# DerryHub/BEVFormer_tensorrt

Hardware: AMD Instinct MI355X
Metric: frames/sec BEVFormer-base bs=1 fp16 end-to-end on MI355X (re-hosted model, random weights, synthetic 6-camera frames) (higher is better)
Workload: dtype f16

## Files before the change

### bevformer_tensorrt_amd/bevformer.py

```python
import math
import os
import time

import torch
import torch.nn as nn
import torch.nn.functional as F

from . import functions as _hip_ops
from . import geometry as G
from .functions.dispatch import OWN_KERNELS, own_kernel_choice, using as _dispatch_using
from .functions.linear import tsgemm_weight_stationary
from .utils import lib as _lib

CONFIGS = {
    "tiny": dict(depth=50, dcn=(False, False, False, False), fpn_in=[2048], out_indices=(3,), levels=1,
                 image=(480, 800), bev=(50, 50), enc_layers=3, style="pytorch"),
    "small": dict(depth=101, dcn=(False, False, True, True), fpn_in=[2048], out_indices=(3,), levels=1,
                  image=(736, 1280), bev=(150, 150), enc_layers=3, style="caffe"),
    "base": dict(depth=101, dcn=(False, False, True, True), fpn_in=[512, 1024, 2048], out_indices=(1, 2, 3),
                 levels=4, image=(928, 1600), bev=(200, 200), enc_layers=6, style="caffe"),
}
PC_RANGE = [-51.2, -51.2, -5.0, 51.2, 51.2, 3.0]
POST_CENTER_RANGE = [-61.2, -61.2, -10.0, 61.2, 61.2, 10.0]
MAX_DETECTIONS = 300
EMBED, HEADS, NUM_QUERY, NUM_CAMS = 256, 8, 900, 6


inverse_sigmoid = G.inverse_sigmoid


_CAM_IDX = {}


def _take_cams(t, cams):
    cams = tuple(cams)
    if cams == tuple(range(t.shape[0])):
        return t
    key = (cams, str(t.device))
    idx = _CAM_IDX.get(key)
    if idx is None:
        idx = _CAM_IDX[key] = torch.tensor(cams, dtype=torch.long, device=t.device)
    return t.index_select(0, idx)


def _rows(x):
    return x.permute(0, 2, 3, 1).reshape(-1, x.shape[1])


def _from_rows(y, n, h, w):
    return y.view(n, h, w, y.shape[-1]).permute(0, 3, 1, 2)


_FUSED_LINEAR = {"enabled": os.environ.get("BEVOPS_FUSED_LINEAR", "1") != "0"}
_R3 = {"enabled": os.environ.get("BEVOPS_R3_FUSIONS", "1") != "0"}
_TSA_LOCAL = {"enabled": os.environ.get("BEVOPS_TSA_LOCAL", "1") == "1"}
_TSA_GLUE = {"enabled": os.environ.get("BEVOPS_TSA_GLUE", "1") == "1"}


def _or_none(fn, *args, **kwargs):
    try:
        return fn(*args, **kwargs)
    except _lib.BevopsError as exc:
        if exc.status != _lib.NOT_SUPPORTED:
            raise
        return None


def _fused_linear(ops, x, weight, bias, residual, relu):
    fn = getattr(ops, "linear_bias_act", None)
    if fn is None or not _FUSED_LINEAR["enabled"] or x.dtype != torch.float16 or not x.is_cuda:
        return None
    auto = getattr(ops, "dense_auto", None)
    if auto is not None and _R3["enabled"]:
        return _or_none(auto, x, weight, bias, residual, relu)
    return _or_none(fn, x, weight, bias, residual, relu)


def _gemm_entry(ops):
    return getattr(ops, "dense_auto", None) or getattr(ops, "linear_bias_act", None)


def _dense(ops, lin, x, residual=None, relu=False):
    if hasattr(lin, "fake_quant_reference"):
        return lin(x, residual, relu)
    y = _fused_linear(ops, x, lin.weight, lin.bias, residual, relu)
    if y is not None:
        return y
    y = lin(x)
    if residual is not None:
        y = y + residual
    return F.relu(y, inplace=True) if relu else y


def _mlp(ops, seq, x):
    mods = list(seq)
    if not _R3["enabled"] or not all(isinstance(m, (nn.Linear, nn.ReLU)) for m in mods):
        return seq(x)
    i = 0
    while i < len(mods):
        if isinstance(mods[i], nn.ReLU):
            x = F.relu(x)
            i += 1
            continue
        relu = i + 1 < len(mods) and isinstance(mods[i + 1], nn.ReLU)
        x = _dense(ops, mods[i], x, None, relu)
        i += 2 if relu else 1
    return x


def _layer_norm(ops, norm, x):
    fn = getattr(ops, "layer_norm", None)
    if fn is None or not _FUSED_LINEAR["enabled"] or x.dtype != torch.float16 or not x.is_cuda or \
            x.shape[-1] not in (64, 128, 256, 512):
        return norm(x)
    return fn(x, norm.weight, norm.bias, norm.eps)


_FUSED_REFINE = {"enabled": os.environ.get("BEVOPS_FUSED_REFINE", "1") == "1"}
_OWN_ATTN = {"enabled": os.environ.get("BEVOPS_OWN_ATTN", "1") == "1"}
_LN_FUSED = {"enabled": os.environ.get("BEVOPS_LN_FUSED", "1") == "1"}
_INT8_LN_FUSED = {"enabled": os.environ.get("BEVOPS_INT8_LN_FUSED", "0") == "1"}
_OWN_ENCODER = {"enabled": os.environ.get("BEVOPS_OWN_ENCODER", "1") == "1"}
_SHARDED_TABLE_BACKBONE = {"enabled": _OWN_ENCODER["enabled"] and os.environ.get("BEVOPS_SHARDED_RULE_DISPATCH", "0") != "1"}


def _dense_norm(ops, lin, x, residual, norm):
    fn = getattr(ops, "tsgemm_ln", None)
    if fn is not None and _LN_FUSED["enabled"] and _R3["enabled"] and _FUSED_LINEAR["enabled"] and type(lin) is nn.Linear \
            and x.dtype == torch.float16 and x.is_cuda and lin.out_features == EMBED and lin.in_features % 64 == 0 \
            and isinstance(norm, nn.LayerNorm) and norm.elementwise_affine and norm.normalized_shape == (EMBED,) \
            and x.numel() // x.shape[-1] >= 32:
        out = _or_none(fn, x, lin.weight, lin.bias, residual, norm.weight, norm.bias, norm.eps)
        if out is not None:
            return out
    if _int8_ln_on(ops) and _int8_norm_ok(lin, x, norm):
        return lin.forward_norm_from_q(_hip_ops.quantize_rows(x, lin.scale_in), residual, norm)
    return _layer_norm(ops, norm, _dense(ops, lin, x, residual, False))


def _int8_ln_on(ops):
    on = getattr(ops, "int8_ln_fused", None)
    return _INT8_LN_FUSED["enabled"] if on is None else on


def _int8_norm_ok(lin, x, norm):
    return hasattr(lin, "fake_quant_reference") and lin.mode == "int8" \
        and lin.in_features % 128 == 0 and lin.out_features == EMBED and x.dtype == torch.float16 and x.is_cuda \
        and isinstance(norm, nn.LayerNorm) and norm.elementwise_affine and norm.normalized_shape == (EMBED,)


def _int8_ffn_chain_ok(fc1, fc2, x, norm):
    return hasattr(fc1, "fake_quant_reference") and fc1.mode == "int8" and fc1.in_features % 16 == 0 \
        and _int8_norm_ok(fc2, x, norm)


def _conv1x1_nhwc(ops, x, conv, relu, residual=None):
    s = conv.stride[0]
    if s > 1:
        strided = getattr(ops, "conv_nhwc", None)
        if strided is not None and _R3["enabled"] and _FUSED_LINEAR["enabled"] and x.dtype == torch.float16 and x.is_cuda \
                and not hasattr(conv, "lin") and conv.in_channels % 32 == 0 and x.is_contiguous(memory_format=torch.channels_last):
            return strided(x, conv.weight, conv.bias, relu, residual, s)
        lin = getattr(conv, "lin", None)
        int8_conv = getattr(ops, "conv_int8_nhwc", None)
        if lin is not None and getattr(lin, "mode", None) == "int8" and int8_conv is not None and _R3["enabled"] \
                and x.dtype == torch.float16 and x.is_cuda and conv.in_channels % 64 == 0 \
                and x.is_contiguous(memory_format=torch.channels_last):
            return int8_conv(x, lin.scale_in, lin.weight_q.view(conv.out_channels, 1, 1, conv.in_channels), lin.scale_w,
                             lin.bias_f32, relu, residual, s)
        x = x[:, :, ::s, ::s].contiguous(memory_format=torch.channels_last)
    n, c, h, w = x.shape
    if hasattr(conv, "lin"):
        y = conv.lin(_rows(x), None if residual is None else _rows(residual), relu)
        return _from_rows(y, n, h, w)
    wt = conv.weight.view(conv.out_channels, c).t()
    if residual is not None:
        y = _fused_linear(ops, _rows(x), conv.weight.view(conv.out_channels, c), conv.bias, _rows(residual), relu)
        if y is None:
            y = torch.mm(_rows(x), wt)
            ops.bias_act_nhwc_(y, conv.bias, _rows(residual), relu)
    else:
        y = _fused_linear(ops, _rows(x), conv.weight.view(conv.out_channels, c), conv.bias, None, relu) \
            if _R3["enabled"] else None
        if y is None:
            y = torch._addmm_activation(conv.bias, _rows(x), wt) if relu else torch.addmm(conv.bias, _rows(x), wt)
    return _from_rows(y, n, h, w)


def _conv_nhwc(ops, x, conv, relu, residual=None):
    qmode = getattr(conv, "qmode", None)
    if qmode == "calibrate":
        conv.collect(x)
    elif qmode == "int8" and x.is_contiguous(memory_format=torch.channels_last):
        return conv.int8_nhwc(x, residual, relu)
    auto = getattr(ops, "conv3x3_auto", None)
    if auto is not None and _R3["enabled"] and _FUSED_LINEAR["enabled"] and x.dtype == torch.float16 and x.is_cuda \
            and conv.kernel_size == (3, 3) and conv.stride[0] == conv.stride[1] and conv.padding == (1, 1) \
            and conv.groups == 1 and conv.dilation == (1, 1) and conv.in_channels % 32 == 0 \
            and x.is_contiguous(memory_format=torch.channels_last):
        return auto(x, conv.weight, conv.bias, relu, residual, conv.stride[0])
    y = F.conv2d(x, conv.weight, None, conv.stride, conv.padding)
    if not y.is_contiguous(memory_format=torch.channels_last):
        y = y.contiguous(memory_format=torch.channels_last)
    return ops.bias_act_nhwc_(y, conv.bias, residual, relu)


class DCNv2Pack(nn.Module):

    def __init__(self, cin, cout, ops, stride=1):
        super().__init__()
        self.ops, self.stride = ops, stride
        self._c32_ok = True
        self.weight = nn.Parameter(torch.randn(cout, cin, 3, 3) / math.sqrt(cin * 9))
        self.bias = nn.Parameter(torch.zeros(cout))
        self.conv_offset = nn.Conv2d(cin, 27, 3, stride, 1)
        nn.init.normal_(self.conv_offset.weight, std=0.01)
        nn.init.zeros_(self.conv_offset.bias)

    def forward(self, x):
        out = self.conv_offset(x)
        o1, o2, mask = torch.chunk(out, 3, dim=1)
        offset = torch.cat((o1, o2), dim=1)
        return self.ops.modulated_deformable_conv2d(x, offset, torch.sigmoid(mask), self.weight,
                                                    self.bias, self.stride, 1, 1, 1, 1)

    def _chain_collect(self, om):
        cal = getattr(self, "chain_cal", None)
        if cal is not None:
            cal.collect(self.chain_site + ".offset", om[:, :18])
            cal.collect(self.chain_site + ".mask", torch.sigmoid(om[:, 18:27]))

    def forward_nhwc(self, x, relu):
        fn = getattr(self.ops, "conv_offset_nhwc", None)
        if fn is not None and self.stride == 1 and _FUSED_LINEAR["enabled"] and self._c32_ok:
            try:
                out = fn(x, self.conv_offset.weight, self.conv_offset.bias)
                self._chain_collect(out)
                return self.ops.modulated_deformable_conv2d_nhwc(x, None, None, self.weight, self.bias, self.stride,
                                                                 1, 1, 1, 1, relu=relu, offset_mask_nhwc=out)
            except _lib.BevopsError as exc:
                if exc.status != _lib.NOT_SUPPORTED:
                    raise
                self._c32_ok = False
        w = self.conv_offset.weight
        if getattr(self, "_w32", None) is None or self._w32[2] != (w._version, w.dtype, w.device):
            w32 = torch.zeros(32, *w.shape[1:], dtype=w.dtype, device=w.device)
            w32[:27] = w.detach()
            b32 = torch.zeros(32, dtype=w.dtype, device=w.device)
            b32[:27] = self.conv_offset.bias.detach()
            self._w32 = (w32.contiguous(memory_format=torch.channels_last), b32, (w._version, w.dtype, w.device))
        out = F.conv2d(x, self._w32[0], None, self.stride, 1)
        if not out.is_contiguous(memory_format=torch.channels_last):
            out = out.contiguous(memory_format=torch.channels_last)
        out = self.ops.bias_act_nhwc_(out, self._w32[1], None, False)
        self._chain_collect(out)
        return self.ops.modulated_deformable_conv2d_nhwc(x, None, None, self.weight, self.bias, self.stride, 1, 1,
                                                         1, 1, relu=relu, offset_mask_nhwc=out)


_FUSED_DOWNSAMPLE = {"enabled": os.environ.get("BEVOPS_FUSED_DOWNSAMPLE", "1") != "0"}
_FUSED_DOWNSAMPLE_SHAPES = {(64, 64, 1), (128, 256, 2), (256, 512, 2), (512, 1024, 2)}


def _two_source_ok(ops, blk, x):
    ds, c3 = blk.downsample, blk.conv3
    if ds is None or not (_FUSED_DOWNSAMPLE["enabled"] and _R3["enabled"] and _FUSED_LINEAR["enabled"]) \
            or getattr(ops, "gemm2", None) is None or getattr(blk, "chain_cal", None) is not None:
        return False
    if type(ds) is not nn.Conv2d or type(c3) is not nn.Conv2d or hasattr(ds, "lin") or hasattr(c3, "lin") \
            or ds.bias is None or c3.bias is None or ds.weight.dtype != torch.float16 or c3.weight.dtype != torch.float16 \
            or ds.kernel_size != (1, 1) or c3.kernel_size != (1, 1) or c3.stride != (1, 1) or ds.stride[0] != ds.stride[1]:
        return False
    if x.dtype != torch.float16 or not x.is_cuda or x.dim() != 4 or not x.is_contiguous(memory_format=torch.channels_last):
        return False
    return (c3.in_channels, ds.in_channels, ds.stride[0]) in _FUSED_DOWNSAMPLE_SHAPES


def _stacked_pair(blk):
    ds, c3 = blk.downsample, blk.conv3
    key = _versions(c3.weight, ds.weight, c3.bias, ds.bias)
    hit = getattr(blk, "_w3d", None)
    if hit is None or hit[0] != key:
        n = c3.out_channels
        w = torch.cat([c3.weight.detach().reshape(n, -1), ds.weight.detach().reshape(n, -1)], dim=1).contiguous()
        b = (c3.bias.detach().float() + ds.bias.detach().float()).to(c3.bias.dtype).contiguous()
        hit = (key, w, b)
        blk._w3d = hit
    return hit[1], hit[2]


class Bottleneck(nn.Module):

    def __init__(self, cin, planes, stride, dcn, ops, downsample, style="caffe"):
        super().__init__()
        s1, s2 = (stride, 1) if style == "caffe" else (1, stride)
        self.conv1 = nn.Conv2d(cin, planes, 1, s1)
        self.conv2 = DCNv2Pack(planes, planes, ops, s2) if dcn else nn.Conv2d(planes, planes, 3, s2, 1)
        self.conv3 = nn.Conv2d(planes, planes * 4, 1)
        self.downsample = nn.Conv2d(cin, planes * 4, 1, stride) if downsample else None

    def forward(self, x):
        idt = x if self.downsample is None else self.downsample(x)
        out = F.relu(self.conv1(x), inplace=True)
        out = F.relu(self.conv2(out), inplace=True)
        return F.relu(self.conv3(out) + idt, inplace=True)

    def _hidden_nhwc(self, x, ops):
        out = _conv1x1_nhwc(ops, x, self.conv1, True)
        if isinstance(self.conv2, DCNv2Pack):
            return self.conv2.forward_nhwc(out, True)
        return _conv_nhwc(ops, out, self.conv2, True)

    def forward_nhwc(self, x, ops):
        if _two_source_ok(ops, self, x):
            h = self._hidden_nhwc(x, ops)
            w, b = _stacked_pair(self)
            n, _, ho, wo = h.shape
            y = _or_none(ops.gemm2, _rows(h), x, w, b, self.downsample.stride[0], True)
            if y is not None:
                return _from_rows(y, n, ho, wo)
            return _conv1x1_nhwc(ops, h, self.conv3, True, residual=_conv1x1_nhwc(ops, x, self.downsample, False))
        idt = x if self.downsample is None else _conv1x1_nhwc(ops, x, self.downsample, False)
        out = _conv1x1_nhwc(ops, x, self.conv1, True)
        cal = getattr(self, "chain_cal", None)
        if cal is not None:
            cal.collect(self.chain_site + ".t1", out)
            if self.downsample is not None:
                cal.collect(self.chain_site + ".idt", idt)
        if isinstance(self.conv2, DCNv2Pack):
            out = self.conv2.forward_nhwc(out, True)
        else:
            out = _conv_nhwc(ops, out, self.conv2, True)
        return _conv1x1_nhwc(ops, out, self.conv3, True, residual=idt)


class ResNet(nn.Module):
    def __init__(self, depth, dcn, out_indices, ops, style="caffe"):
        super().__init__()
        blocks = {50: (3, 4, 6, 3), 101: (3, 4, 23, 3)}[depth]
        self.out_indices = out_indices
        self.stem = nn.Conv2d(3, 64, 7, 2, 3)
        cin, stages = 64, []
        for i, n in enumerate(blocks):
            planes, layers = 64 * 2 ** i, []
            for j in range(n):
                layers.append(Bottleneck(cin, planes, (2 if i > 0 else 1) if j == 0 else 1, dcn[i], ops, j == 0, style))
                cin = planes * 4
            stages.append(nn.Sequential(*layers))
        self.stages = nn.ModuleList(stages)

    def forward(self, x):
        x = F.max_pool2d(F.relu(self.stem(x), inplace=True), 3, 2, 1)
        outs = []
        for i, st in enumerate(self.stages):
            x = st(x)
            if i in self.out_indices:
                outs.append(x)
        return outs

    def _stem_fused(self, x, ops):
        fused = getattr(ops, "stem_conv_pool", None)
        if fused is None or not (_R3["enabled"] and _FUSED_LINEAR["enabled"]):
            return None
        from .functions.conv import STEM_FUSED
        st = self.stem
        ok = (STEM_FUSED["enabled"] and x.is_cuda and x.dtype == torch.float16 and x.is_contiguous() and x.shape[-1] % 2 == 0
              and tuple(st.weight.shape) == (64, 3, 7, 7) and st.stride == (2, 2) and st.padding == (3, 3))
        return fused(x, st.weight, st.bias) if ok else None

    def forward_nhwc(self, x, ops):
        y = self._stem_fused(x, ops)
        if y is not None:
            return self._stages_nhwc(y, ops)
        x = x.contiguous(memory_format=torch.channels_last)
        pool = getattr(ops, "bias_relu_maxpool_nhwc", None)
        if pool is not None and _R3["enabled"] and _FUSED_LINEAR["enabled"] and x.dtype == torch.float16 and x.is_cuda:
            y = F.conv2d(x, self.stem.weight, None, self.stem.stride, self.stem.padding)
            if not y.is_contiguous(memory_format=torch.channels_last):
                y = y.contiguous(memory_format=torch.channels_last)
            x = pool(y, self.stem.bias)
        else:
            x = F.max_pool2d(_conv_nhwc(ops, x, self.stem, True), 3, 2, 1)
        return self._stages_nhwc(x, ops)

    def _stages_nhwc(self, x, ops):
        outs = []
        for i, st in enumerate(self.stages):
            for blk in st:
                x = blk.forward_nhwc(x, ops)
            if i in self.out_indices:
                outs.append(x)
        return outs


class FPN(nn.Module):

    def __init__(self, cins, cout, num_outs):
        super().__init__()
        self.lateral = nn.ModuleList(nn.Conv2d(c, cout, 1) for c in cins)
        self.fpn = nn.ModuleList(nn.Conv2d(cout, cout, 3, 1, 1) for _ in cins)
        self.extra = nn.ModuleList(nn.Conv2d(cout, cout, 3, 2, 1) for _ in range(num_outs - len(cins)))

    def forward(self, feats):
        lat = [l(f) for l, f in zip(self.lateral, feats)]
        for i in range(len(lat) - 1, 0, -1):
            lat[i - 1] = lat[i - 1] + F.interpolate(lat[i], size=lat[i - 1].shape[2:], mode="nearest")
        outs = [c(x) for c, x in zip(self.fpn, lat)]
        for e in self.extra:
            outs.append(e(F.relu(outs[-1])))
        return outs

    def forward_nhwc(self, feats, ops):
        return self.topdown_nhwc([_conv1x1_nhwc(ops, f, l, False) for l, f in zip(self.lateral, feats)], ops)

    def topdown_nhwc(self, lat, ops):
        up_add = getattr(ops, "upsample_add_nhwc_", None)
        for i in range(len(lat) - 1, 0, -1):
            a, b = lat[i - 1], lat[i]
            if up_add is not None and _FUSED_LINEAR["enabled"] and _R3["enabled"] and a.dtype == torch.float16 and a.is_cuda \
                    and a.is_contiguous(memory_format=torch.channels_last) and b.is_contiguous(memory_format=torch.channels_last):
                up_add(a, b)
            else:
                lat[i - 1] = a + F.interpolate(b, size=a.shape[2:], mode="nearest")
        outs = [_conv_nhwc(ops, x.contiguous(memory_format=torch.channels_last), c, False) for c, x in zip(self.fpn, lat)]
        for e in self.extra:
            outs.append(_conv_nhwc(ops, F.relu(outs[-1]), e, False))
        return outs


class FFN(nn.Module):
    def __init__(self, dim=EMBED, hidden=2 * EMBED):
        super().__init__()
        self.fc1, self.fc2 = nn.Linear(dim, hidden), nn.Linear(hidden, dim)

    def forward(self, x, ops=None, norm=None):
        if norm is not None and _int8_ln_on(ops) and _int8_ffn_chain_ok(self.fc1, self.fc2, x, norm):
            h_q = self.fc1.forward_q(x, self.fc2.scale_in, relu=True)
            return self.fc2.forward_norm_from_q(h_q, x, norm)
        h = _dense(ops, self.fc1, x, None, True)
        return _dense(ops, self.fc2, h, x, False) if norm is None else _dense_norm(ops, self.fc2, h, x, norm)


class TemporalSelfAttention(nn.Module):

    def __init__(self, ops, points=4):
        super().__init__()
        self.ops, self.points = ops, points
        self.sampling_offsets = nn.Linear(EMBED * 2, 2 * HEADS * points * 2)
        self.attention_weights = nn.Linear(EMBED * 2, 2 * HEADS * points)
        self.value_proj, self.output_proj = nn.Linear(EMBED, EMBED), nn.Linear(EMBED, EMBED)
        self._split = self._pos_term = None

    def _split_projection(self, query, prev0, bev_pos, prev_term=None):
        def both_terms():
            terms = self._split_terms(query, bev_pos)
            if terms is None:
                return None
            fn, wa, wb, pos_term = terms
            t = prev_term if prev_term is not None else fn(prev0.reshape(-1, EMBED), wa, None, pos_term, False)
            return fn(query.reshape(-1, EMBED), wb, None, t, False)
        return _or_none(both_terms)

    def _split_terms(self, query, bev_pos):
        fn = _gemm_entry(self.ops)
        so, aw = self.sampling_offsets, self.attention_weights
        if fn is None or not (_R3["enabled"] and _FUSED_LINEAR["enabled"]) or query.dtype != torch.float16 \
                or not query.is_cuda or type(so) is not nn.Linear or type(aw) is not nn.Linear:
            return None
        key = (so.weight._version, aw.weight._version, so.bias._version, aw.bias._version, so.weight.data_ptr())
        if self._split is None or self._split[0] != key:
            w = torch.cat([so.weight, aw.weight]).detach()
            self._split = (key, w[:, :EMBED].contiguous(), w[:, EMBED:].contiguous(),
                           torch.cat([so.bias, aw.bias]).detach().contiguous())
            self._pos_term = None
        _, wa, wb, b = self._split
        pkey = (bev_pos.data_ptr(), bev_pos._version, tuple(bev_pos.shape), bev_pos.dtype)
        if self._pos_term is None or self._pos_term[0] != pkey:
            self._pos_term = (pkey, fn(bev_pos.reshape(-1, EMBED), wb, b, None, False))
        return fn, wa, wb, self._pos_term[1]

    def forward(self, query, value, bev_pos, ref_2d, spatial_shapes, rows=None, norm=None, prev_term=None):
        identity = query
        nq, nk = query.shape[1], value.shape[1]
        mine = value if rows is None else value[:, rows[0]:rows[1]]
        both = self._split_projection(query, mine[0], bev_pos, prev_term if rows is None else None)
        split = getattr(self.ops, "tsa_split", None) if _TSA_GLUE["enabled"] else None
        pre = None
        if both is not None and split is not None and self.points == 4:
            pre = split(both, HEADS, self.points)
        elif both is not None:
            n_off = 2 * HEADS * self.points * 2
            off = both[:, :n_off].view(1, nq, HEADS, 2, 1, self.points, 2)
            w = both[:, n_off:].view(1, nq, HEADS, 2, 1, self.points)
        else:
            query = torch.cat([mine[:1], query + bev_pos], -1)
            off = self.sampling_offsets(query).view(1, nq, HEADS, 2, 1, self.points, 2)
            w = self.attention_weights(query).view(1, nq, HEADS, 2, 1, self.points)
        value = _dense(self.ops, self.value_proj, value).view(2, nk, HEADS, EMBED // HEADS)
        if pre is not None:
            off, w = pre
        else:
            w = w.permute(0, 3, 1, 2, 4, 5).contiguous().view(2, nq, HEADS, -1)
            off = off.permute(0, 3, 1, 2, 4, 5, 6).contiguous().view(2, nq, HEADS, -1)
        msda = (getattr(self.ops, "multi_scale_deformable_attn_local", None) if _TSA_LOCAL["enabled"] else None) \
            or self.ops.multi_scale_deformable_attn
        out = msda(value, spatial_shapes, ref_2d, off, w).flatten(2)
        mean2 = getattr(self.ops, "queue_mean2", None) if _TSA_GLUE["enabled"] else None
        if mean2 is not None and out.is_cuda and out.dtype == torch.float16 and out.numel() % 16 == 0 and _R3["enabled"]:
            out = mean2(out)
        else:
            out = torch.mean(out, keepdim=True, dim=0)
        if norm is not None:
            return _dense_norm(self.ops, self.output_proj, out, identity, norm)
        return _dense(self.ops, self.output_proj, out, identity, False)


class SpatialCrossAttention(nn.Module):

    def __init__(self, ops, levels, points=8):
        super().__init__()
        self.ops = ops
        self._proj_ok = True
        self.sampling_offsets = nn.Linear(EMBED, HEADS * levels * points * 2)
        self.attention_weights = nn.Linear(EMBED, HEADS * levels * points)
        self.value_proj, self.output_proj = nn.Linear(EMBED, EMBED), nn.Linear(EMBED, EMBED)

    def _offsets_weights(self, query, nq, merged):
        pair = _merged_pair(self.ops, self, "_so_aw", self.sampling_offsets, self.attention_weights, query) if merged else None
        if pair is None:
            pair = (_dense(self.ops, self.sampling_offsets, query), _dense(self.ops, self.attention_weights, query))
        return pair[0].view(1, nq, HEADS, -1), pair[1].view(1, nq, HEADS, -1)

    def forward(self, query, value, reference_points_cam, bev_mask, spatial_shapes, cams=None, gather=None, plan=None,
                residual=None, norm=None, merged=False):
        inp_residual = query if residual is None else residual
        ncam, nk, nq = value.shape[0], value.shape[1], query.shape[1]
        mode = getattr(gather, "mode", None)
        if cams is None and gather is not None and hasattr(gather, "cams"):
            cams = gather.cams
        ref = reference_points_cam.reshape(reference_points_cam.shape[0], nq, 1, -1)
        ref_l, mask_l = (ref, bev_mask) if cams is None else (_take_cams(ref, cams), _take_cams(bev_mask, cams))
        local_sum = gather is None or mode in ("reduce", "scatter")
        projected = getattr(self.ops, "spatial_cross_attention_projected", None)
        fused = getattr(self.ops, "spatial_cross_attention_sample", None)
        fp16_gpu = value.dtype == torch.float16 and value.is_cuda
        slots = None
        if local_sum and ncam == 0:
            slots = torch.zeros((1, nq, EMBED), dtype=value.dtype, device=value.device)
        elif projected is not None and local_sum and _R3["enabled"] and self._proj_ok and fp16_gpu \
                and not hasattr(self.value_proj, "fake_quant_reference"):
            off, w = self._offsets_weights(query, nq, merged)
            try:
                slots = projected(value.reshape(ncam, nk, EMBED), self.value_proj.weight, self.value_proj.bias,
                                  spatial_shapes, ref_l.contiguous(), off, w, mask_l.contiguous(), HEADS,
                                  **({"plan": plan} if plan is not None else {}))
            except _lib.BevopsError as exc:
                if exc.status != _lib.NOT_SUPPORTED:
                    raise
                self._proj_ok = False
        if slots is None:
            value = _dense(self.ops, self.value_proj, value.reshape(ncam, nk, EMBED)).view(ncam, nk, HEADS, EMBED // HEADS)
            off, w = (t.expand(ncam, -1, -1, -1) for t in self._offsets_weights(query, nq, merged))
            msda = self.ops.multi_scale_deformable_attn
            if mode == "gather":
                ref_c = ref_l.contiguous()
                queries = gather.gather(
                    lambda i: msda(value[i:i + 1], spatial_shapes, ref_c[i:i + 1], off[:1], w[:1]).flatten(2),
                    (nq, EMBED), value.dtype, value.device)
                slots = (queries * bev_mask).sum(0, keepdim=True)
            elif local_sum and fused is not None and (fp16_gpu or getattr(fused, "any_device", False)):
                slots = fused(value, spatial_shapes, ref_l, off[:1], w[:1], mask_l)
            elif local_sum:
                queries = msda(value, spatial_shapes, ref_l.contiguous(), off, w).flatten(2)
                slots = (queries * mask_l).sum(0, keepdim=True)
            else:
                queries = gather(msda(value, spatial_shapes, ref_l.contiguous(), off, w).flatten(2))
                slots = (queries * bev_mask).sum(0, keepdim=True)
        if mode == "reduce":
            slots = gather.reduce(slots)
        elif mode == "scatter":
            slots = gather.reduce_scatter_queries(slots, nq)
        if norm is not None:
            return _dense_norm(self.ops, self.output_proj, slots, inp_residual, norm)
        return _dense(self.ops, self.output_proj, slots, inp_residual, False)


class BEVFormerLayer(nn.Module):
    def __init__(self, ops, levels):
        super().__init__()
        self.tsa, self.sca, self.ffn = TemporalSelfAttention(ops), SpatialCrossAttention(ops, levels), FFN()
        self.norms = nn.ModuleList(nn.LayerNorm(EMBED) for _ in range(3))

    def forward(self, query, value, bev_pos, ref_2d, ref_cam, bev_mask, spatial_shapes, bev_shapes, prev_bev,
                use_prev_bev, cams, gather, plan=None, rows=None, tsa_prev_term=None, merged=False):
        ops = self.tsa.ops
        if rows is not None:
            lo, hi = rows
            nq = bev_pos.shape[1]
            if torch.is_tensor(use_prev_bev) or not use_prev_bev:
                full = gather.all_gather_queries(query, nq)
                prev = torch.where(use_prev_bev.to(torch.bool), prev_bev, full.expand(2, -1, -1)) \
                    if torch.is_tensor(use_prev_bev) else full.repeat(2, 1, 1)
            else:
                prev = prev_bev
            query = self.tsa(query, prev, bev_pos[:, lo:hi], ref_2d[:, lo:hi].contiguous(), bev_shapes, rows=rows,
                             norm=self.norms[0])
            full = gather.all_gather_queries(query, nq)
            query = self.sca(full, value, ref_cam, bev_mask, spatial_shapes, cams, gather, plan, residual=query,
                             norm=self.norms[1])
            return self.ffn(query, ops, norm=self.norms[2])
        if torch.is_tensor(use_prev_bev):
            prev = torch.where(use_prev_bev.to(torch.bool), prev_bev, query.expand(2, -1, -1))
        else:
            prev = prev_bev if use_prev_bev else query.repeat(2, 1, 1)
        if prev is not prev_bev:
            tsa_prev_term = None
        query = self.tsa(query, prev, bev_pos, ref_2d, bev_shapes, norm=self.norms[0], prev_term=tsa_prev_term)
        query = self.sca(query, value, ref_cam, bev_mask, spatial_shapes, cams, gather, plan, norm=self.norms[1],
                         merged=merged)
        return self.ffn(query, ops, norm=self.norms[2])


def _static_term(cache, owner, key, pos, fn, weight, bias):
    hit = getattr(owner, cache, None)
    if hit is None or hit[0] != key or hit[1] is not pos:
        hit = (key, pos, fn(pos.reshape(-1, pos.shape[-1]), weight, bias, None, False))
        setattr(owner, cache, hit)
    return hit[2]


def _fast_dense_ok(ops, x, *linears):
    return getattr(ops, "linear_bias_act", None) is not None and _R3["enabled"] and _FUSED_LINEAR["enabled"] \
        and x.dtype == torch.float16 and x.is_cuda \
        and all(isinstance(l, nn.Linear) and not hasattr(l, "fake_quant_reference") for l in linears)


def _versions(*tensors):
    return tuple(t._version for t in tensors) + tuple(t.data_ptr() for t in tensors)


_MERGED_PROJ = {"enabled": os.environ.get("BEVOPS_MERGED_PROJ", "1") != "0"}


def _merge_ok(ops, x, linears, has_res):
    if not (_MERGED_PROJ["enabled"] and _R3["enabled"] and _FUSED_LINEAR["enabled"]) \
            or getattr(ops, "dense_auto", None) is None or x.dtype != torch.float16 or not x.is_cuda \
            or not all(type(l) is nn.Linear and l.bias is not None and l.weight.dtype == torch.float16 for l in linears):
        return False
    if not OWN_KERNELS["enabled"]:
        return False
    K = x.shape[-1]
    return _per_layer_kernels(x.device, x.numel() // K, [l.weight.shape[0] for l in linears], K, not has_res, has_res) == "tiled"


def _per_layer_kernels(device, M, widths, K, has_bias, has_res):
    if M <= 0:
        return None
    names = {own_kernel_choice(device, M, n, K, False, has_bias, has_res) for n in widths}
    if names == {"small"}:
        return "small"
    if names <= {"tile", "tsgemm"} and ("tsgemm" not in names or tsgemm_weight_stationary(K)):
        return "tiled"
    return None


def _merged_pair(ops, owner, cache, lin_a, lin_b, x):
    fn = getattr(ops, "tile_gemm_dst", None)
    widths = [lin_a.weight.shape[0], lin_b.weight.shape[0]]
    if fn is None or not _merge_ok(ops, x, (lin_a, lin_b), False) or any(n % 64 for n in widths):
        return None
    key = _versions(lin_a.weight, lin_b.weight, lin_a.bias, lin_b.bias)
    hit = getattr(owner, cache, None)
    if hit is None or hit[0] != key:
        hit = (key, torch.cat([lin_a.weight, lin_b.weight]).detach().contiguous(),
               torch.cat([lin_a.bias, lin_b.bias]).detach().contiguous())
        setattr(owner, cache, hit)
    return _or_none(fn, x.reshape(-1, x.shape[-1]), hit[1], hit[2], widths)


def _merged_prev_terms(ops, owner, cache, tsas, query, prev0, bev_pos):
    fn = getattr(ops, "tile_gemm_dst", None)
    if fn is None or not (_MERGED_PROJ["enabled"] and _R3["enabled"] and _FUSED_LINEAR["enabled"]) \
            or prev0.dtype != torch.float16 or not prev0.is_cuda:
        return None
    if not OWN_KERNELS["enabled"]:
        return None

    def all_layers():
        terms = [t._split_terms(query, bev_pos) for t in tsas]
        if any(t is None for t in terms):
            return None
        widths = [t[1].shape[0] for t in terms]
        M = prev0.numel() // EMBED
# ... 566 lines not shown
```

### bevformer_tensorrt_amd/csrc/capi.hip

```cpp
#include <string.h>

#include "common.h"

extern "C" const char *bevops_version(void) { return "bevops-hip 0.1 (gfx950)"; }

extern "C" const char *bevops_status_string(int status) {
  switch (status) {
    case BEVOPS_SUCCESS: return "success";
    case BEVOPS_FAILURE: return "failure (kernel launch error)";
    case BEVOPS_BAD_PARAM: return "bad parameter";
    case BEVOPS_NOT_SUPPORTED: return "dtype/shape combination not supported";
    case BEVOPS_NOT_INITIALIZED: return "not initialized";
    default: return "unknown status";
  }
}

namespace {
struct Entry {
  const char *name;
  void *fn;
};
const Entry kTable[] = {
    {"bevops_msda_forward", (void *)&bevops_msda_forward},
    {"bevops_msda_forward_ws", (void *)&bevops_msda_forward_ws},
    {"bevops_msda_workspace_size", (void *)&bevops_msda_workspace_size},
    {"MultiScaleDeformableAttnTRT", (void *)&bevops_msda_forward},
    {"MultiScaleDeformableAttnTRT2", (void *)&bevops_msda_forward},
    {"bevops_rotate_forward", (void *)&bevops_rotate_forward},
    {"RotateTRT", (void *)&bevops_rotate_forward},
    {"RotateTRT2", (void *)&bevops_rotate_forward},
    {"bevops_grid_sampler_2d_forward", (void *)&bevops_grid_sampler_2d_forward},
    {"GridSampler2DTRT", (void *)&bevops_grid_sampler_2d_forward},
    {"GridSampler2DTRT2", (void *)&bevops_grid_sampler_2d_forward},
    {"bevops_grid_sampler_3d_forward", (void *)&bevops_grid_sampler_3d_forward},
    {"GridSampler3DTRT", (void *)&bevops_grid_sampler_3d_forward},
    {"GridSampler3DTRT2", (void *)&bevops_grid_sampler_3d_forward},
    {"bevops_bev_pool_v2_forward", (void *)&bevops_bev_pool_v2_forward},
    {"BEVPoolV2TRT", (void *)&bevops_bev_pool_v2_forward},
    {"BEVPoolV2TRT2", (void *)&bevops_bev_pool_v2_forward},
    {"bevops_mdconv_forward", (void *)&bevops_mdconv_forward},
    {"bevops_mdconv_workspace_size", (void *)&bevops_mdconv_workspace_size},
    {"bevops_mdconv_forward_int8", (void *)&bevops_mdconv_forward_int8},
    {"bevops_mdconv_forward_int8_packed", (void *)&bevops_mdconv_forward_int8_packed},
    {"ModulatedDeformableConv2dTRT", (void *)&bevops_mdconv_forward},
    {"ModulatedDeformableConv2dTRT2", (void *)&bevops_mdconv_forward},
    {"bevops_qkv_forward", (void *)&bevops_qkv_forward},
    {"bevops_qkv_workspace_size", (void *)&bevops_qkv_workspace_size},
    {"QKVTRT", (void *)&bevops_qkv_forward},
    {"QKVTRT2", (void *)&bevops_qkv_forward},
    {"bevops_inverse_forward", (void *)&bevops_inverse_forward},
    {"InverseTRT", (void *)&bevops_inverse_forward},
    {"bevops_nms_free_decode", (void *)&bevops_nms_free_decode},
    {"bevops_centerpoint_decode", (void *)&bevops_centerpoint_decode},
    {"bevops_centerpoint_decode_ex", (void *)&bevops_centerpoint_decode_ex},
    {"bevops_centerpoint_decode_workspace_size", (void *)&bevops_centerpoint_decode_workspace_size},
    {"bevops_bev_nms", (void *)&bevops_bev_nms},
    {"bevops_bev_nms_workspace_size", (void *)&bevops_bev_nms_workspace_size},
    {"bevops_bev_iou", (void *)&bevops_bev_iou},
    {"bevops_centernet_decode", (void *)&bevops_centernet_decode},
    {"bevops_centernet_decode_workspace_size", (void *)&bevops_centernet_decode_workspace_size},
    {"bevops_yolox_decode", (void *)&bevops_yolox_decode},
    {"bevops_box_nms", (void *)&bevops_box_nms},
    {"bevops_box_nms_workspace_size", (void *)&bevops_box_nms_workspace_size},
    {"bevops_lss_voxel_prepare", (void *)&bevops_lss_voxel_prepare},
    {"bevops_lss_voxel_prepare_workspace_size", (void *)&bevops_lss_voxel_prepare_workspace_size},
    {"bevops_lss_voxel_prepare_batched", (void *)&bevops_lss_voxel_prepare_batched},
    {"bevops_lss_voxel_prepare_batched_workspace_size", (void *)&bevops_lss_voxel_prepare_batched_workspace_size},
    {"bevops_bev_pool_v2_forward_indirect", (void *)&bevops_bev_pool_v2_forward_indirect},
    {"bevops_grid_sampler_2d_forward_ws", (void *)&bevops_grid_sampler_2d_forward_ws},
    {"bevops_grid_sampler_2d_workspace_size", (void *)&bevops_grid_sampler_2d_workspace_size},
    {"bevops_rotate_forward_hwc", (void *)&bevops_rotate_forward_hwc},
    {"bevops_sca_forward", (void *)&bevops_sca_forward},
    {"bevops_mdconv_forward_nhwc", (void *)&bevops_mdconv_forward_nhwc},
    {"bevops_conv3x3_c32_forward_nhwc", (void *)&bevops_conv3x3_c32_forward_nhwc},
    {"bevops_bias_act_nhwc", (void *)&bevops_bias_act_nhwc},
    {"bevops_bias_relu_maxpool_nhwc", (void *)&bevops_bias_relu_maxpool_nhwc},
    {"bevops_stem_packed_size", (void *)&bevops_stem_packed_size},
    {"bevops_stem_pack", (void *)&bevops_stem_pack},
    {"bevops_stem_conv_pool", (void *)&bevops_stem_conv_pool},
    {"bevops_stem_set_variant", (void *)&bevops_stem_set_variant},
    {"bevops_upsample_add_nhwc", (void *)&bevops_upsample_add_nhwc},
    {"bevops_lss_depth_split", (void *)&bevops_lss_depth_split},
    {"bevops_upsample_bilinear_concat_nhwc", (void *)&bevops_upsample_bilinear_concat_nhwc},
    {"bevops_lss_depth_split_s8", (void *)&bevops_lss_depth_split_s8},
    {"bevops_upsample_bilinear_s8", (void *)&bevops_upsample_bilinear_s8},
    {"bevops_tsa_split", (void *)&bevops_tsa_split},
    {"bevops_queue_mean2", (void *)&bevops_queue_mean2},
    {"bevops_tsgemm_f16", (void *)&bevops_tsgemm_f16},
    {"bevops_tsgemm_s8", (void *)&bevops_tsgemm_s8},
    {"bevops_tsgemm_s8_ln", (void *)&bevops_tsgemm_s8_ln},
    {"bevops_tsgemm_tile_rows", (void *)&bevops_tsgemm_tile_rows},
    {"bevops_tsgemm_f16_ln", (void *)&bevops_tsgemm_f16_ln},
    {"bevops_tsgemm_f16_grouped", (void *)&bevops_tsgemm_f16_grouped},
    {"bevops_mha_selfattn_f16", (void *)&bevops_mha_selfattn_f16},
    {"bevops_mha_selfattn_max_queries", (void *)&bevops_mha_selfattn_max_queries},
    {"bevops_value_proj_packed_size", (void *)&bevops_value_proj_packed_size},
    {"bevops_value_proj_packed", (void *)&bevops_value_proj_packed},
    {"bevops_value_pack_planes", (void *)&bevops_value_pack_planes},
    {"bevops_sca_prepacked_workspace_size", (void *)&bevops_sca_prepacked_workspace_size},
    {"bevops_sca_forward_prepacked", (void *)&bevops_sca_forward_prepacked},
    {"bevops_sca_plan_size", (void *)&bevops_sca_plan_size},
    {"bevops_sca_plan_build", (void *)&bevops_sca_plan_build},
    {"bevops_sca_forward_planned", (void *)&bevops_sca_forward_planned},
    {"bevops_point_sampling", (void *)&bevops_point_sampling},
    {"bevops_feat_embed_nhwc", (void *)&bevops_feat_embed_nhwc},
    {"bevops_linear_bias_act", (void *)&bevops_linear_bias_act},
    {"bevops_linear_tune", (void *)&bevops_linear_tune},
    {"bevops_quantize_rows", (void *)&bevops_quantize_rows},
    {"bevops_dequantize_rows", (void *)&bevops_dequantize_rows},
    {"bevops_linear_int8", (void *)&bevops_linear_int8},
    {"bevops_linear_int8_fused", (void *)&bevops_linear_int8_fused},
    {"bevops_tile_gemm_f16", (void *)&bevops_tile_gemm_f16},
    {"bevops_tile_gemm_f16_dst", (void *)&bevops_tile_gemm_f16_dst},
    {"bevops_gemm2_f16", (void *)&bevops_gemm2_f16},
    {"bevops_small_gemm_f16_dst", (void *)&bevops_small_gemm_f16_dst},
    {"bevops_small_gemm_f16", (void *)&bevops_small_gemm_f16},
    {"bevops_conv_tile_f16", (void *)&bevops_conv_tile_f16},
    {"bevops_conv3x3_c64_f16", (void *)&bevops_conv3x3_c64_f16},
    {"bevops_deconv4x4s2_packed_weight_size", (void *)&bevops_deconv4x4s2_packed_weight_size},
    {"bevops_deconv4x4s2_pack_weight", (void *)&bevops_deconv4x4s2_pack_weight},
    {"bevops_deconv4x4s2_f16", (void *)&bevops_deconv4x4s2_f16},
    {"bevops_conv_slice_f16", (void *)&bevops_conv_slice_f16},
    {"bevops_conv_slice_f16_ex", (void *)&bevops_conv_slice_f16_ex},
    {"bevops_lss_camera_gate_packed_size", (void *)&bevops_lss_camera_gate_packed_size},
    {"bevops_lss_camera_gate", (void *)&bevops_lss_camera_gate},
    {"bevops_se_gate2_nhwc", (void *)&bevops_se_gate2_nhwc},
    {"bevops_global_avgpool_nhwc", (void *)&bevops_global_avgpool_nhwc},
    {"bevops_focus_nhwc", (void *)&bevops_focus_nhwc},
    {"bevops_spp_maxpool_nhwc", (void *)&bevops_spp_maxpool_nhwc},
    {"bevops_upsample_nearest2x_nhwc", (void *)&bevops_upsample_nearest2x_nhwc},
    {"bevops_conv_slice_s8", (void *)&bevops_conv_slice_s8},
    {"bevops_conv_slice_s8_ex", (void *)&bevops_conv_slice_s8_ex},
    {"bevops_conv_slice_s8_ex2", (void *)&bevops_conv_slice_s8_ex2},
    {"bevops_se_gate2_nhwc_s8", (void *)&bevops_se_gate2_nhwc_s8},
    {"bevops_global_avgpool_nhwc_s8", (void *)&bevops_global_avgpool_nhwc_s8},
    {"bevops_deconv4x4s2_s8", (void *)&bevops_deconv4x4s2_s8},
    {"bevops_focus_nhwc_q", (void *)&bevops_focus_nhwc_q},
    {"bevops_spp_maxpool_nhwc_s8", (void *)&bevops_spp_maxpool_nhwc_s8},
    {"bevops_upsample_nearest2x_nhwc_s8", (void *)&bevops_upsample_nearest2x_nhwc_s8},
    {"bevops_refine_reference_points", (void *)&bevops_refine_reference_points},
    {"bevops_decode_boxes", (void *)&bevops_decode_boxes},
    {"bevops_conv_tile_int8_fused", (void *)&bevops_conv_tile_int8_fused},
    {"bevops_linear_int8_chain", (void *)&bevops_linear_int8_chain},
    {"bevops_conv_tile_int8", (void *)&bevops_conv_tile_int8},
    {"bevops_bias_relu_maxpool_nhwc_int8", (void *)&bevops_bias_relu_maxpool_nhwc_int8},
    {"bevops_mdconv_int8_nhwc_workspace_size", (void *)&bevops_mdconv_int8_nhwc_workspace_size},
    {"bevops_mdconv_forward_int8_nhwc", (void *)&bevops_mdconv_forward_int8_nhwc},
    {"bevops_image_normalize_pad", (void *)&bevops_image_normalize_pad},
    {"bevops_image_normalize_resize_pad", (void *)&bevops_image_normalize_resize_pad},
    {"bevops_image_letterbox", (void *)&bevops_image_letterbox},
    {"bevops_image_resize_plan_size", (void *)&bevops_image_resize_plan_size},
    {"bevops_image_resize_plan_build", (void *)&bevops_image_resize_plan_build},
    {"bevops_image_resize_crop_normalize", (void *)&bevops_image_resize_crop_normalize},
    {"bevops_msda_packed_size", (void *)&bevops_msda_packed_size},
    {"bevops_msda_pack_value", (void *)&bevops_msda_pack_value},
    {"bevops_msda_forward_prepacked", (void *)&bevops_msda_forward_prepacked},
    {"bevops_linear_workspace_size", (void *)&bevops_linear_workspace_size},
    {"bevops_msda_workspace_size_shapes", (void *)&bevops_msda_workspace_size_shapes},
    {"bevops_sca_workspace_size", (void *)&bevops_sca_workspace_size},
    {"bevops_mdconv_forward_packed", (void *)&bevops_mdconv_forward_packed},
    {"bevops_mdconv_pack_weight", (void *)&bevops_mdconv_pack_weight},
    {"bevops_mdconv_packed_weight_size", (void *)&bevops_mdconv_packed_weight_size},
    {"bevops_conv3x3_c32_pack_weight", (void *)&bevops_conv3x3_c32_pack_weight},
    {"bevops_conv3x3_c32_packed_weight_size", (void *)&bevops_conv3x3_c32_packed_weight_size},
    {"bevops_layer_norm", (void *)&bevops_layer_norm},
    {"bevops_calib_state_size", (void *)&bevops_calib_state_size},
    {"bevops_calib_collect", (void *)&bevops_calib_collect},
    {"bevops_calib_threshold_workspace_size", (void *)&bevops_calib_threshold_workspace_size},
    {"bevops_calib_threshold", (void *)&bevops_calib_threshold},
    {"bevops_deform_conv3x3_nhwc_f16", (void *)&bevops_deform_conv3x3_nhwc_f16},
};
}

extern "C" void *bevops_query(const char *name) {
  if (!name) return nullptr;
  for (const Entry &e : kTable)
    if (strcmp(e.name, name) == 0) return e.fn;
  return nullptr;
}
```

### bevformer_tensorrt_amd/csrc/tsgemm.hip

```cpp
#include <stdlib.h>

#include <type_traits>

#include "gemm_host.h"
#include "mdconv.h"
#include "msda_pad.h"

namespace bevops {
namespace {

constexpr int kTsBN = 256;
constexpr int kTsG = 5;
constexpr int kTsThreads = 512;
constexpr int kTsW = kTsBN * 128;
constexpr int kTsX = kTsG * 32 * 128;
constexpr int kTsStage = kTsW + kTsX;
constexpr int kTsEpiStride = 128 * 4 + 16;
constexpr int kTsStages = 3;
constexpr int kTsLds = kTsStages * kTsStage;
constexpr int kTsS8LnLds = kTsLds + 2 * kTsBN * 2;

struct TsPacked {
  char *gset, *sset;
  Hm3Tab t;
// ... 161 lines not shown
    w_off[j] = (unsigned)(((size_t)(n0 + row) * K) * 2) + ((pchunk ^ swz8(row)) << 4);
  }
  const unsigned hi = (unsigned)(lane >> 5);
  const unsigned fa = (unsigned)(wave * 32 + (lane & 31));
  const int nk = K / 64;

  float bcol[16];
#pragma unroll
  for (int rq = 0; rq < 4; ++rq)
#pragma unroll
    for (int e = 0; e < 4; ++e)
      bcol[4 * rq + e] = bias ? __half2float(bias[n0 + wave * 32 + 8 * rq + 4 * (int)hi + e]) : 0.f;

  for (int u0 = u_begin; u0 < u_end; u0 += kTsG) {
    const int G = min(kTsG, u_end - u0);
    const int r0 = u0 * 32;
    const int pieces_x = G * 4;
    unsigned x_off[3];
#pragma unroll
    for (int j = 0; j < 3; ++j) {
      const unsigned row = (unsigned)((wave + 8 * j) * 8) + prow;
      x_off[j] = (unsigned)(((size_t)(r0 + row) * K) * 2) + ((pchunk ^ swz8(row)) << 4);
    }
    const int k_rot = bi % nk;
    auto dma = [&](int step, int buf) {
      char *wd = smem + buf * kTsStage + wave * 4096;
      int kstep = step + k_rot;
      if (kstep >= nk) kstep -= nk;
      const int soff = kstep * 128;
#pragma unroll
      for (int j = 0; j < 4; ++j)
        __builtin_amdgcn_raw_ptr_buffer_load_lds(rs_w, (lds_void_t *)(wd + j * 1024), 16, (int)w_off[j], soff, 0, 0);
      char *xd = smem + buf * kTsStage + kTsW;
#pragma unroll
      for (int j = 0; j < 3; ++j)
        if (wave + 8 * j < pieces_x)
          __builtin_amdgcn_raw_ptr_buffer_load_lds(rs_x, (lds_void_t *)(xd + (wave + 8 * j) * 1024), 16,
                                                   (int)x_off[j], soff, 0, 0);
    };
    f32x16 acc[kTsG];
#pragma unroll
    for (int g = 0; g < kTsG; ++g)
#pragma unroll
      for (int r = 0; r < 16; ++r) acc[g][r] = 0.f;

    const int my_dma = 4 + (wave < pieces_x ? 1 : 0) + (wave + 8 < pieces_x ? 1 : 0) + (wave + 16 < pieces_x ? 1 : 0);
    auto wait_keep_one_step = [&]() {
      switch (my_dma) {
        case 4: asm volatile("s_waitcnt vmcnt(4)" ::: "memory"); break;
        case 5: asm volatile("s_waitcnt vmcnt(5)" ::: "memory"); break;
        case 6: asm volatile("s_waitcnt vmcnt(6)" ::: "memory"); break;
        default: asm volatile("s_waitcnt vmcnt(7)" ::: "memory"); break;
      }
    };
    auto kloop = [&](auto gc) __attribute__((always_inline)) {
      constexpr int GG = decltype(gc)::value;
      dma(0, 0);
      if (nk > 1) dma(1, 1);
      for (int s = 0; s < nk; ++s) {
        const int buf = s % kTsStages;
        if (s + 1 < nk) wait_keep_one_step();
        else asm volatile("s_waitcnt vmcnt(0)" ::: "memory");
        __builtin_amdgcn_s_barrier();
        if (s + 2 < nk) dma(s + 2, (s + 2) % kTsStages);
        const char *Wb = smem + buf * kTsStage;
        const char *Xb = Wb + kTsW;
#pragma unroll
        for (int ks = 0; ks < 4; ++ks) {
          const unsigned c = 2u * ks + hi;
          const f16x8 a = *reinterpret_cast<const f16x8 *>(Wb + fa * 128 + ((c ^ swz8(fa)) << 4));
          f16x8 b[GG];
#pragma unroll
          for (int g = 0; g < GG; ++g) {
            const unsigned xr = (unsigned)(g * 32 + (lane & 31));
            b[g] = *reinterpret_cast<const f16x8 *>(Xb + xr * 128 + ((c ^ swz8(xr)) << 4));
          }
#pragma unroll
          for (int g = 0; g < GG; ++g) acc[g] = __builtin_amdgcn_mfma_f32_32x32x16_f16(a, b[g], acc[g], 0, 0, 0);
        }
      }
    };
    switch (G) {
      case 1: kloop(std::integral_constant<int, 1>{}); break;
      case 2: kloop(std::integral_constant<int, 2>{}); break;
      case 3: kloop(std::integral_constant<int, 3>{}); break;
      case 4: kloop(std::integral_constant<int, 4>{}); break;
      default: kloop(std::integral_constant<int, 5>{}); break;
    }
    __builtin_amdgcn_s_barrier();
    const int rows = min(G * 32, M - r0);
    uint4 keep[2][kTsG];
    float rsum[kTsG];
    if constexpr (EPI == 2) {
#pragma unroll
      for (int i = 0; i < kTsG; ++i) rsum[i] = 0.f;
    }
#pragma unroll
    for (int half = 0; half < 2; ++half) {
      if ((wave >> 2) == half) {
        const int cw = (wave & 3) * 32;
#pragma unroll
        for (int g = 0; g < kTsG; ++g) {
          if (g < G) {
            char *rowp = smem + (g * 32 + (lane & 31)) * kTsEpiStride;
#pragma unroll
            for (int rq = 0; rq < 4; ++rq) {
              float4 v = make_float4(acc[g][4 * rq] + bcol[4 * rq], acc[g][4 * rq + 1] + bcol[4 * rq + 1],
                                     acc[g][4 * rq + 2] + bcol[4 * rq + 2], acc[g][4 * rq + 3] + bcol[4 * rq + 3]);
              *reinterpret_cast<float4 *>(rowp + (cw + 8 * rq + 4 * (int)hi) * 4) = v;
            }
          }
        }
      }
      __builtin_amdgcn_s_barrier();
      auto row_pass = [&](int r, auto itc) __attribute__((always_inline)) {
        constexpr int it = decltype(itc)::value;
        (void)it;
        const int c8 = tid & 15;
        const float4 lo = *reinterpret_cast<const float4 *>(smem + r * kTsEpiStride + c8 * 32);
        const float4 hi4 = *reinterpret_cast<const float4 *>(smem + r * kTsEpiStride + c8 * 32 + 16);
        float v[8] = {lo.x, lo.y, lo.z, lo.w, hi4.x, hi4.y, hi4.z, hi4.w};
        const int col = n0 + half * 128 + c8 * 8;
        const size_t m = (size_t)(r0 + r);
        if constexpr (EPI == 2) {
          if (res) {
            const uint4 q = *reinterpret_cast<const uint4 *>(res + m * N + col);
            v[0] += h2f_lo(q.x); v[1] += h2f_hi(q.x); v[2] += h2f_lo(q.y); v[3] += h2f_hi(q.y);
            v[4] += h2f_lo(q.z); v[5] += h2f_hi(q.z); v[6] += h2f_lo(q.w); v[7] += h2f_hi(q.w);
          }
          uint4 o;
          o.x = pack_h2(v[0], v[1]); o.y = pack_h2(v[2], v[3]); o.z = pack_h2(v[4], v[5]); o.w = pack_h2(v[6], v[7]);
          keep[half][it] = o;
          rsum[it] += (h2f_lo(o.x) + h2f_hi(o.x)) + (h2f_lo(o.y) + h2f_hi(o.y)) + (h2f_lo(o.z) + h2f_hi(o.z)) +
                      (h2f_lo(o.w) + h2f_hi(o.w));
        } else if constexpr (EPI == 0) {
          if (res) {
            const uint4 q = *reinterpret_cast<const uint4 *>(res + m * N + col);
            v[0] += h2f_lo(q.x); v[1] += h2f_hi(q.x); v[2] += h2f_lo(q.y); v[3] += h2f_hi(q.y);
            v[4] += h2f_lo(q.z); v[5] += h2f_hi(q.z); v[6] += h2f_lo(q.w); v[7] += h2f_hi(q.w);
          }
          if (relu) {
#pragma unroll
            for (int k = 0; k < 8; ++k) v[k] = fmaxf(v[k], 0.f);
          }
          uint4 o;
          o.x = pack_h2(v[0], v[1]); o.y = pack_h2(v[2], v[3]); o.z = pack_h2(v[4], v[5]); o.w = pack_h2(v[6], v[7]);
          *reinterpret_cast<uint4 *>(out + m * N + col) = o;
        } else {
          const int cam = (int)(m / (size_t)pk.nk), s = (int)(m - (size_t)cam * pk.nk);
          const int head = col >> 5, q8 = (col & 31) >> 3;
          int l = 0;
#pragma unroll
          for (int k = 1; k < kHm3MaxLevels; ++k)
            if (k < pk.t.L && s >= pk.t.src0[k]) l = k;
          const int rel = s - pk.t.src0[l];
          const int y = rel / pk.t.W[l], xx = rel - y * pk.t.W[l];
          const int wp = pk.t.W[l] + 1;
          const int f = pk.t.ent0[l] + (y + 1) * wp + xx;
          const size_t plane = (size_t)cam * pk.heads + head;
          const unsigned h0 = pack_h2(v[0], v[1]), h1 = pack_h2(v[2], v[3]), h2 = pack_h2(v[4], v[5]), h3 = pack_h2(v[6], v[7]);
          if (l >= pk.t.ls) {
            *reinterpret_cast<uint4 *>(pk.sset + (plane * pk.t.s_entries + f) * kLdsPixBytes + q8 * 16) =
                make_uint4(h0, h1, h2, h3);
          } else {
            float nb[8];
            const bool has_r = xx + 1 < pk.t.W[l] && r + 1 < rows;
            const bool own_r = xx + 1 < pk.t.W[l];
            if (has_r) {
              const float4 a4 = *reinterpret_cast<const float4 *>(smem + (r + 1) * kTsEpiStride + c8 * 32);
              const float4 b4 = *reinterpret_cast<const float4 *>(smem + (r + 1) * kTsEpiStride + c8 * 32 + 16);
              nb[0] = a4.x; nb[1] = a4.y; nb[2] = a4.z; nb[3] = a4.w; nb[4] = b4.x; nb[5] = b4.y; nb[6] = b4.z; nb[7] = b4.w;
            } else {
#pragma unroll
              for (int k = 0; k < 8; ++k) nb[k] = 0.f;
            }
            char *e = pk.gset + (plane * pk.t.g_entries + f) * kEntBytes + q8 * 32;
            if (has_r || !own_r) {
              uint4 o0, o1;
              o0.x = pack_h2(v[0], nb[0]); o0.y = pack_h2(v[1], nb[1]); o0.z = pack_h2(v[2], nb[2]); o0.w = pack_h2(v[3], nb[3]);
              o1.x = pack_h2(v[4], nb[4]); o1.y = pack_h2(v[5], nb[5]); o1.z = pack_h2(v[6], nb[6]); o1.w = pack_h2(v[7], nb[7]);
              *reinterpret_cast<uint4 *>(e) = o0;
              *reinterpret_cast<uint4 *>(e + 16) = o1;
            } else {
              unsigned short *e16 = reinterpret_cast<unsigned short *>(e);
              const unsigned hv[4] = {h0, h1, h2, h3};
#pragma unroll
              for (int k = 0; k < 4; ++k) { e16[4 * k] = (unsigned short)(hv[k] & 0xffffu); e16[4 * k + 2] = (unsigned short)(hv[k] >> 16); }
            }
            if (xx == 0) {
              uint4 o0, o1;
              o0.x = h0 << 16; o0.y = h0 & 0xffff0000u; o0.z = h1 << 16; o0.w = h1 & 0xffff0000u;
              o1.x = h2 << 16; o1.y = h2 & 0xffff0000u; o1.z = h3 << 16; o1.w = h3 & 0xffff0000u;
              *reinterpret_cast<uint4 *>(e - kEntBytes) = o0;
              *reinterpret_cast<uint4 *>(e - kEntBytes + 16) = o1;
            } else if (r == 0) {
              unsigned short *e16 = reinterpret_cast<unsigned short *>(e - kEntBytes);
              const unsigned hv[4] = {h0, h1, h2, h3};
#pragma unroll
              for (int k = 0; k < 4; ++k) { e16[4 * k + 1] = (unsigned short)(hv[k] & 0xffffu); e16[4 * k + 3] = (unsigned short)(hv[k] >> 16); }
            }
          }
        }
      };
      if constexpr (EPI == 2) {
        const int rb = tid >> 4;
        if (rb < rows) row_pass(rb, std::integral_constant<int, 0>{});
        if (rb + 32 < rows) row_pass(rb + 32, std::integral_constant<int, 1>{});
        if (rb + 64 < rows) row_pass(rb + 64, std::integral_constant<int, 2>{});
        if (rb + 96 < rows) row_pass(rb + 96, std::integral_constant<int, 3>{});
        if (rb + 128 < rows) row_pass(rb + 128, std::integral_constant<int, 4>{});
      } else {
        for (int r = tid >> 4; r < rows; r += kTsThreads / 16) row_pass(r, std::integral_constant<int, 0>{});
      }
      __builtin_amdgcn_s_barrier();
    }
    if constexpr (EPI == 2) {
      const int c8 = tid & 15;
      const __half *gam = reinterpret_cast<const __half *>(pk.gset), *bet = reinterpret_cast<const __half *>(pk.sset);
      int it = 0;
#pragma unroll
      for (int r = tid >> 4; r < kTsG * 32; r += kTsThreads / 16, ++it) {
        if (r >= rows) break;
        const float mean = row16_sum(rsum[it]) * (1.f / 256.f);
        float f[16];
#pragma unroll
        for (int h = 0; h < 2; ++h) {
          const uint4 o = keep[h][it];
          f[8 * h + 0] = h2f_lo(o.x) - mean; f[8 * h + 1] = h2f_hi(o.x) - mean;
          f[8 * h + 2] = h2f_lo(o.y) - mean; f[8 * h + 3] = h2f_hi(o.y) - mean;
          f[8 * h + 4] = h2f_lo(o.z) - mean; f[8 * h + 5] = h2f_hi(o.z) - mean;
          f[8 * h + 6] = h2f_lo(o.w) - mean; f[8 * h + 7] = h2f_hi(o.w) - mean;
        }
        float sq = 0.f;
#pragma unroll
        for (int k = 0; k < 16; ++k) sq = fmaf(f[k], f[k], sq);
        const float rstd = rsqrtf(row16_sum(sq) * (1.f / 256.f) + pk.eps);
        const size_t m = (size_t)(r0 + r);
#pragma unroll
        for (int h = 0; h < 2; ++h) {
          const int col = h * 128 + c8 * 8;
          const uint4 g4 = *reinterpret_cast<const uint4 *>(gam + col), b4 = *reinterpret_cast<const uint4 *>(bet + col);
          const float gg[8] = {h2f_lo(g4.x), h2f_hi(g4.x), h2f_lo(g4.y), h2f_hi(g4.y),
                               h2f_lo(g4.z), h2f_hi(g4.z), h2f_lo(g4.w), h2f_hi(g4.w)};
          const float bb[8] = {h2f_lo(b4.x), h2f_hi(b4.x), h2f_lo(b4.y), h2f_hi(b4.y),
                               h2f_lo(b4.z), h2f_hi(b4.z), h2f_lo(b4.w), h2f_hi(b4.w)};
          float y[8];
#pragma unroll
          for (int k = 0; k < 8; ++k) y[k] = fmaf(f[8 * h + k] * rstd, gg[k], bb[k]);
          uint4 o;
          o.x = pack_h2(y[0], y[1]); o.y = pack_h2(y[2], y[3]); o.z = pack_h2(y[4], y[5]); o.w = pack_h2(y[6], y[7]);
          *reinterpret_cast<uint4 *>(out + m * N + col) = o;
        }
      }
    }
  }
}

__global__ __launch_bounds__(256) void tsgemm_pad_zero_kernel(TsPacked pk, int planes) {
  const Hm3Tab &t = pk.t;
  const int plane = blockIdx.y;
  if (plane >= planes) return;
  for (int l = 0; l < t.L; ++l) {
    const bool staged = l >= t.ls;
    const int wp = t.W[l] + 1, H = t.H[l];
    const int ebytes = staged ? kLdsPixBytes : kEntBytes;
    const int chunks = ebytes / 16;
    char *base = (staged ? pk.sset + (size_t)plane * t.s_entries * kLdsPixBytes
                         : pk.gset + (size_t)plane * t.g_entries * kEntBytes);
    const int total = 2 * wp + H;
    for (int i = blockIdx.x * 256 + threadIdx.x; i < total * chunks; i += gridDim.x * 256) {
      const int e = i / chunks, c = i - e * chunks;
      int yp, xx;
      if (e < wp) { yp = 0; xx = e; }
      else if (e < 2 * wp) { yp = H + 1; xx = e - wp; }
      else { yp = e - 2 * wp + 1; xx = t.W[l]; }
      if (!staged && xx == t.W[l] && yp < H) continue;
      *reinterpret_cast<uint4 *>(base + (size_t)(t.ent0[l] + yp * wp + xx) * ebytes + c * 16) = make_uint4(0, 0, 0, 0);
    }
  }
  if (blockIdx.x == 0 && threadIdx.x < 16) {
    const int c = threadIdx.x & 7, which = threadIdx.x >> 3;
    char *g = pk.gset + (size_t)plane * t.g_entries * kEntBytes;
    *reinterpret_cast<uint4 *>(g + (which ? (size_t)(t.g_entries - 1) * kEntBytes : 0) + c * 16) = make_uint4(0, 0, 0, 0);
    if (t.s_entries && c < 4) {
      char *s = pk.sset + (size_t)plane * t.s_entries * kLdsPixBytes;
      *reinterpret_cast<uint4 *>(s + (which ? (size_t)(t.s_entries - 1) * kLdsPixBytes : 0) + c * 16) = make_uint4(0, 0, 0, 0);
    }
  }
}

constexpr int kWsG = 2;
constexpr int kWsRows = kWsG * 32;
constexpr int kWsBufs = 3;
constexpr int kWsStep = kWsRows * 128;
constexpr int kWsEpi = kWsRows * kTsEpiStride;
constexpr int ws_lds(int ks) { return kWsEpi + kWsBufs * ks * kWsStep; }

struct TsSrc2 {
  const __half *x2;
  unsigned bytes;
  int hin, win, hout, wout, stride;
};

template <int EPI, int KS, bool GRP, int KS2 = 0>
__device__ __forceinline__ void tsgemm_ws_body(const __half *__restrict__ x, const __half *__restrict__ w,
                                               const __half *__restrict__ bias, const __half *__restrict__ res,
                                               __half *__restrict__ out, int M, int N, int relu, int units_total, int parts,
                                               int chunks, const TsPacked &pk, const TsSrc2 &src2 = TsSrc2{}) {
  extern __shared__ __attribute__((aligned(16))) char smem[];
  constexpr int K = KS * 64;
  constexpr int KS1 = KS - KS2, K1 = KS1 * 64, K2 = KS2 * 64;
  const int tid = threadIdx.x, lane = tid & 63, wave = tid >> 6;
  int part, chunk;
  if (gridDim.x % (8u * (unsigned)chunks) == 0) {
    const int i = (int)(blockIdx.x >> 3);
    chunk = i % chunks;
    part = (i / chunks) * 8 + (int)(blockIdx.x & 7);
  } else {
    chunk = (int)blockIdx.x % chunks;
    part = (int)blockIdx.x / chunks;
  }
  const int n0 = chunk * kTsBN;
  const int per = units_total / parts, extra = units_total % parts;
  const int u_begin = part * per + min(part, extra);
  const int u_end = u_begin + per + (part < extra ? 1 : 0);
  if (u_begin >= u_end) return;
  const int ntiles = (u_end - u_begin + kWsG - 1) / kWsG;

  const __amdgpu_buffer_rsrc_t rs_x =
      __builtin_amdgcn_make_buffer_rsrc(const_cast<__half *>(x), 0, (unsigned)((size_t)M * K1 * 2), 0x00020000);
  const __amdgpu_buffer_rsrc_t rs_x2 =
      __builtin_amdgcn_make_buffer_rsrc(const_cast<__half *>(src2.x2), 0, KS2 > 0 ? src2.bytes : 0u, 0x00020000);
  const unsigned hi = (unsigned)(lane >> 5);
  const unsigned fa = (unsigned)(wave * 32 + (lane & 31));
  f16x8 wr[KS * 4];
  {
    const __half *wrow = w + (size_t)(n0 + (int)fa) * K + hi * 8;
#pragma unroll
    for (int kk = 0; kk < KS * 4; ++kk) wr[kk] = *reinterpret_cast<const f16x8 *>(wrow + kk * 16);
  }
  float bcol[16];
  if (bias) {
    uint2 bq[4];
#pragma unroll
    for (int rq = 0; rq < 4; ++rq)
      bq[rq] = *reinterpret_cast<const uint2 *>(bias + n0 + wave * 32 + 8 * rq + 4 * (int)hi);
#pragma unroll
    for (int rq = 0; rq < 4; ++rq) {
      bcol[4 * rq] = h2f_lo(bq[rq].x); bcol[4 * rq + 1] = h2f_hi(bq[rq].x);
      bcol[4 * rq + 2] = h2f_lo(bq[rq].y); bcol[4 * rq + 3] = h2f_hi(bq[rq].y);
    }
  } else {
#pragma unroll
    for (int i = 0; i < 16; ++i) bcol[i] = 0.f;
  }

  const unsigned trow = (unsigned)(wave * 8 + (lane >> 3));
  const unsigned tchunk = (((unsigned)(lane & 7)) ^ swz8(trow)) << 4;
  auto dma = [&](int t, int buf) {
    const int row = (u_begin + t * kWsG) * 32 + (int)trow;
    const bool valid = t < ntiles && u_begin + t * kWsG + (wave >> 2) < u_end && row < M;
    const unsigned voff = valid ? (unsigned)((size_t)row * K1 * 2) + tchunk : 0xFFFFFF00u;
    char *d = smem + kWsEpi + buf * (KS * kWsStep) + wave * 1024;
#pragma unroll
    for (int ks = 0; ks < KS1; ++ks)
      __builtin_amdgcn_raw_ptr_buffer_load_lds(rs_x, (lds_void_t *)(d + ks * kWsStep), 16, (int)voff, ks * 128, 0, 0);
    if constexpr (KS2 > 0) {
      unsigned voff2 = 0xFFFFFF00u;
      if (valid) {
        size_t pix = (size_t)row;
        if (src2.stride != 1) {
          const int per = src2.hout * src2.wout;
          const int b = row / per, q = row - b * per;
          const int yo = q / src2.wout, xo = q - yo * src2.wout;
          pix = ((size_t)b * src2.hin + (size_t)(yo * src2.stride)) * src2.win + (size_t)(xo * src2.stride);
        }
        voff2 = (unsigned)(pix * K2 * 2) + tchunk;
      }
#pragma unroll
      for (int ks = 0; ks < KS2; ++ks)
        __builtin_amdgcn_raw_ptr_buffer_load_lds(rs_x2, (lds_void_t *)(d + (KS1 + ks) * kWsStep), 16, (int)voff2, ks * 128,
                                                 0, 0);
    }
  };
  auto wait_keep_one_tile = [&]() { asm volatile("s_waitcnt vmcnt(%0)" ::"n"(KS) : "memory"); };
  auto wait_for_next_tile = [&](int younger) {
    switch (younger) {
      case 0: asm volatile("s_waitcnt vmcnt(%0)" ::"n"(KS) : "memory"); break;
      case 2: asm volatile("s_waitcnt vmcnt(%0)" ::"n"(KS + 2) : "memory"); break;
      case 4: asm volatile("s_waitcnt vmcnt(%0)" ::"n"(KS + 4) : "memory"); break;
      case 6: asm volatile("s_waitcnt vmcnt(%0)" ::"n"(KS + 6) : "memory"); break;
      default: asm volatile("s_waitcnt vmcnt(%0)" ::"n"(KS + 8) : "memory"); break;
    }
  };
  const int rb = tid >> 4, c8 = tid & 15;
  uint4 rq[2][kWsG];
  auto load_res = [&](int t, uint4(&q)[2][kWsG]) {
#pragma unroll
    for (int half = 0; half < 2; ++half)
#pragma unroll
      for (int i = 0; i < kWsG; ++i) {
        const size_t m = (size_t)min((u_begin + t * kWsG) * 32 + rb + 32 * i, M - 1);
        q[half][i] = *reinterpret_cast<const uint4 *>(res + m * N + n0 + half * 128 + c8 * 8);
      }
  };
  uint4 gb[4];
  if constexpr (EPI == 2) ts_ln_params(pk, c8, gb);
  if constexpr (EPI != 1) {
    if (res) load_res(0, rq);
  }

  dma(0, 0);
  dma(1, 1);
#pragma unroll
  for (int kk = 0; kk < KS * 4; ++kk) asm volatile("" ::"v"(wr[kk]));
  wait_keep_one_tile();
  __builtin_amdgcn_s_barrier();

  int buf = 0;
  int stores_prev = 0;
  for (int t = 0; t < ntiles; ++t) {
    const int u0 = u_begin + t * kWsG;
    const int r0 = u0 * 32;
    const int rows = min(min(kWsRows, (u_end - u0) * 32), M - r0);
    uint4 rqn[2][kWsG];
    if constexpr (EPI != 1) {
      if (res) load_res(t + 1, rqn);
    }
    {
      int b2 = buf + 2;
      if (b2 >= kWsBufs) b2 -= kWsBufs;
      dma(t + 2, b2);
    }
    f32x16 acc[kWsG];
#pragma unroll
    for (int g = 0; g < kWsG; ++g)
#pragma unroll
      for (int r = 0; r < 16; ++r) acc[g][r] = 0.f;
    const char *Xt = smem + kWsEpi + buf * (KS * kWsStep);
#pragma unroll
    for (int kk = 0; kk < KS * 4; ++kk) {
      const unsigned c = 2u * (kk & 3) + hi;
      f16x8 b[kWsG];
#pragma unroll
      for (int g = 0; g < kWsG; ++g) {
        const unsigned xr = (unsigned)(g * 32 + (lane & 31));
        b[g] = *reinterpret_cast<const f16x8 *>(Xt + (kk >> 2) * kWsStep + xr * 128 + ((c ^ swz8(xr)) << 4));
      }
#pragma unroll
      for (int g = 0; g < kWsG; ++g) acc[g] = __builtin_amdgcn_mfma_f32_32x32x16_f16(wr[kk], b[g], acc[g], 0, 0, 0);
    }
    uint4 keep[2][kWsG];
    float rsum[kWsG];
    if constexpr (EPI == 2) {
#pragma unroll
      for (int i = 0; i < kWsG; ++i) rsum[i] = 0.f;
    }
#pragma unroll
    for (int half = 0; half < 2; ++half) {
      if ((wave >> 2) == half) {
        const int cw = (wave & 3) * 32;
#pragma unroll
        for (int g = 0; g < kWsG; ++g) {
          const unsigned rowa = lds_addr(smem + (lane & 31) * kTsEpiStride + (cw + 4 * (int)hi) * 4);
          auto put = [&](auto qc) __attribute__((always_inline)) {
            constexpr int q = decltype(qc)::value;
            const f32x4 v = {acc[g][4 * q] + bcol[4 * q], acc[g][4 * q + 1] + bcol[4 * q + 1],
                             acc[g][4 * q + 2] + bcol[4 * q + 2], acc[g][4 * q + 3] + bcol[4 * q + 3]};
            if (g == 0) lds_write16<q * 32>(rowa, v);
            else lds_write16<32 * kTsEpiStride + q * 32>(rowa, v);
          };
          put(std::integral_constant<int, 0>{}); put(std::integral_constant<int, 1>{});
          put(std::integral_constant<int, 2>{}); put(std::integral_constant<int, 3>{});
        }
        asm volatile("s_waitcnt lgkmcnt(0)" ::: "memory");
      }
      __builtin_amdgcn_s_barrier();
      if (half == 0) wait_for_next_tile(stores_prev + ((EPI != 1 && res) ? 4 : 0));
#pragma unroll
      for (int i = 0; i < kWsG; ++i) {
        const int r = rb + 32 * i;
        if (r < rows) {
          float v[8];
          lds_read32(lds_addr(smem + r * kTsEpiStride + c8 * 32), v);
          const int col = n0 + half * 128 + c8 * 8;
          const size_t m = (size_t)(r0 + r);
          if constexpr (EPI == 1) {
            ts_store_planes(v, pk, m, col, r, rows, c8, smem);
          } else {
            if (res) ts_add_res(v, rq[half][i]);
            if constexpr (EPI == 2) {
              const uint4 o = ts_pack8(v);
              keep[half][i] = o;
              rsum[i] += ts_sum8(o);
            } else {
              if (relu) {
#pragma unroll
                for (int k = 0; k < 8; ++k) v[k] = fmaxf(v[k], 0.f);
              }
              if constexpr (GRP)
                *reinterpret_cast<uint4 *>(out + (size_t)chunk * (size_t)pk.gstride + m * kTsBN + (col - n0)) = ts_pack8(v);
              else
                *reinterpret_cast<uint4 *>(out + m * N + col) = ts_pack8(v);
            }
          }
        }
      }
      __builtin_amdgcn_s_barrier();
    }
    if constexpr (EPI == 2) {
#pragma unroll
      for (int i = 0; i < kWsG; ++i) {
        const int r = rb + 32 * i;
        if (r < rows) ts_ln_row(keep[0][i], keep[1][i], rsum[i], pk.eps, gb, out + (size_t)(r0 + r) * N, c8);
      }
    }
    if constexpr (EPI != 1) {
      if (res) {
#pragma unroll
        for (int half = 0; half < 2; ++half)
#pragma unroll
          for (int i = 0; i < kWsG; ++i) rq[half][i] = rqn[half][i];
      }
    }
    stores_prev = __builtin_amdgcn_readfirstlane(2 * ((wave * 4 < rows ? 1 : 0) + (wave * 4 + 32 < rows ? 1 : 0)));
    if (++buf == kWsBufs) buf = 0;
  }
}

template <int EPI, int KS>
__global__ __launch_bounds__(kTsThreads) void tsgemm_ws_kernel(const __half *__restrict__ x, const __half *__restrict__ w,
                                                               const __half *__restrict__ bias,
                                                               const __half *__restrict__ res, __half *__restrict__ out,
                                                               int M, int N, int relu, int units_total, int parts,
                                                               int chunks, TsPacked pk) {
  tsgemm_ws_body<EPI, KS, false>(x, w, bias, res, out, M, N, relu, units_total, parts, chunks, pk);
}

template <int KS>
__global__ __launch_bounds__(kTsThreads) void tsgemm_ws_grouped_kernel(const __half *__restrict__ x, const __half *__restrict__ w,
                                                                       const __half *__restrict__ bias, __half *__restrict__ out,
                                                                       int M, int N, int units_total, int parts, int chunks,
                                                                       TsPacked pk) {
  tsgemm_ws_body<0, KS, true>(x, w, bias, nullptr, out, M, N, 0, units_total, parts, chunks, pk);
}

template <int KS, int KS2>
__global__ __launch_bounds__(kTsThreads) void tsgemm_ws2_kernel(const __half *__restrict__ x, const __half *__restrict__ w,
                                                                const __half *__restrict__ bias, __half *__restrict__ out,
                                                                int M, int N, int relu, int units_total, int parts, int chunks,
                                                                TsSrc2 src2) {
  tsgemm_ws_body<0, KS, false, KS2>(x, w, bias, nullptr, out, M, N, relu, units_total, parts, chunks, TsPacked{}, src2);
}

typedef int i32x4v __attribute__((ext_vector_type(4)));
typedef int i32x16v __attribute__((ext_vector_type(16)));

struct TsS8Args {
  const int8_t *a, *w;
  const float *bias, *wscale;
  const void *res;
  void *out;
  float s_aw, s_res, inv_s_out;
  int M, N, K, relu, units_total, res_i8, out_i8;
};

struct TsS8LnArgs : TsS8Args {
  TsPacked pk;
};

template <int EPI>
__global__ __launch_bounds__(kTsThreads) void tsgemm_s8_kernel(
    const std::conditional_t<EPI == 2, TsS8LnArgs, TsS8Args> p) {
  extern __shared__ __attribute__((aligned(16))) char smem[];
  const int tid = threadIdx.x, lane = tid & 63, wave = tid >> 6;
  const int M = p.M, N = p.N, K = p.K;
  const int n0 = blockIdx.y * kTsBN;
  const int nb = gridDim.x, bi = blockIdx.x;
  const int per = p.units_total / nb, extra = p.units_total % nb;
  const int u_begin = bi * per + min(bi, extra);
  const int u_end = u_begin + per + (bi < extra ? 1 : 0);
  if (u_begin >= u_end) return;
  const __amdgpu_buffer_rsrc_t rs_x =
      __builtin_amdgcn_make_buffer_rsrc(const_cast<int8_t *>(p.a), 0, (unsigned)((size_t)M * K), 0x00020000);
  const __amdgpu_buffer_rsrc_t rs_w =
      __builtin_amdgcn_make_buffer_rsrc(const_cast<int8_t *>(p.w), 0, (unsigned)((size_t)N * K), 0x00020000);
  const unsigned prow = (unsigned)(lane >> 3), pchunk = (unsigned)(lane & 7);
  unsigned w_off[4];
#pragma unroll
  for (int j = 0; j < 4; ++j) {
    const unsigned row = (unsigned)((wave * 4 + j) * 8) + prow;
    w_off[j] = (unsigned)((size_t)(n0 + row) * K) + ((pchunk ^ swz8(row)) << 4);
  }
  const unsigned hi = (unsigned)(lane >> 5);
  const unsigned fa = (unsigned)(wave * 32 + (lane & 31));
  const int nk = K / 128;
  float scol[16], bcol[16];
#pragma unroll
  for (int rq = 0; rq < 4; ++rq)
#pragma unroll
    for (int e = 0; e < 4; ++e) {
      const int col = n0 + wave * 32 + 8 * rq + 4 * (int)hi + e;
      scol[4 * rq + e] = p.wscale ? p.s_aw * p.wscale[col] : p.s_aw;
      bcol[4 * rq + e] = p.bias ? p.bias[col] : 0.f;
    }
  TsPacked ln_lds;
  if constexpr (EPI == 2) {
    ln_lds.gset = smem + kTsLds;
    ln_lds.sset = smem + kTsLds + kTsBN * 2;
    if (tid < 64) {
      const char *src = (tid < 32 ? p.pk.gset : p.pk.sset) + (tid & 31) * 16;
      *reinterpret_cast<uint4 *>(smem + kTsLds + tid * 16) = *reinterpret_cast<const uint4 *>(src);
      asm volatile("s_waitcnt lgkmcnt(0)" ::: "memory");
    }
  }
  for (int u0 = u_begin; u0 < u_end; u0 += kTsG) {
    const int G = min(kTsG, u_end - u0);
    const int r0 = u0 * 32;
    const int pieces_x = G * 4;
    unsigned x_off[3];
#pragma unroll
    for (int j = 0; j < 3; ++j) {
      const unsigned row = (unsigned)((wave + 8 * j) * 8) + prow;
      x_off[j] = (unsigned)((size_t)(r0 + row) * K) + ((pchunk ^ swz8(row)) << 4);
    }
    const int k_rot = bi % nk;
    auto dma = [&](int step, int buf) {
      char *wd = smem + buf * kTsStage + wave * 4096;
      int kstep = step + k_rot;
      if (kstep >= nk) kstep -= nk;
      const int soff = kstep * 128;
#pragma unroll
      for (int j = 0; j < 4; ++j)
        __builtin_amdgcn_raw_ptr_buffer_load_lds(rs_w, (lds_void_t *)(wd + j * 1024), 16, (int)w_off[j], soff, 0, 0);
      char *xd = smem + buf * kTsStage + kTsW;
#pragma unroll
      for (int j = 0; j < 3; ++j)
        if (wave + 8 * j < pieces_x)
          __builtin_amdgcn_raw_ptr_buffer_load_lds(rs_x, (lds_void_t *)(xd + (wave + 8 * j) * 1024), 16,
                                                   (int)x_off[j], soff, 0, 0);
    };
    i32x16v acc[kTsG];
#pragma unroll
    for (int g = 0; g < kTsG; ++g)
#pragma unroll
      for (int r = 0; r < 16; ++r) acc[g][r] = 0;
    const int my_dma = 4 + (wave < pieces_x ? 1 : 0) + (wave + 8 < pieces_x ? 1 : 0) + (wave + 16 < pieces_x ? 1 : 0);
    auto wait_keep_one_step = [&]() {
      switch (my_dma) {
        case 4: asm volatile("s_waitcnt vmcnt(4)" ::: "memory"); break;
        case 5: asm volatile("s_waitcnt vmcnt(5)" ::: "memory"); break;
        case 6: asm volatile("s_waitcnt vmcnt(6)" ::: "memory"); break;
        default: asm volatile("s_waitcnt vmcnt(7)" ::: "memory"); break;
      }
    };
    auto kloop = [&](auto gc) __attribute__((always_inline)) {
      constexpr int GG = decltype(gc)::value;
      dma(0, 0);
      if (nk > 1) dma(1, 1);
      for (int s = 0; s < nk; ++s) {
        const int buf = s % kTsStages;
        if (s + 1 < nk) wait_keep_one_step();
        else asm volatile("s_waitcnt vmcnt(0)" ::: "memory");
        __builtin_amdgcn_s_barrier();
        if (s + 2 < nk) dma(s + 2, (s + 2) % kTsStages);
        const char *Wb = smem + buf * kTsStage;
        const char *Xb = Wb + kTsW;
#pragma unroll
        for (int ks = 0; ks < 4; ++ks) {
          const unsigned c = 2u * ks + hi;
          const i32x4v a = *reinterpret_cast<const i32x4v *>(Wb + fa * 128 + ((c ^ swz8(fa)) << 4));
          i32x4v b[GG];
#pragma unroll
          for (int g = 0; g < GG; ++g) {
            const unsigned xr = (unsigned)(g * 32 + (lane & 31));
            b[g] = *reinterpret_cast<const i32x4v *>(Xb + xr * 128 + ((c ^ swz8(xr)) << 4));
          }
#pragma unroll
          for (int g = 0; g < GG; ++g) acc[g] = __builtin_amdgcn_mfma_i32_32x32x32_i8(a, b[g], acc[g], 0, 0, 0);
        }
      }
    };
    switch (G) {
      case 1: kloop(std::integral_constant<int, 1>{}); break;
      case 2: kloop(std::integral_constant<int, 2>{}); break;
      case 3: kloop(std::integral_constant<int, 3>{}); break;
      case 4: kloop(std::integral_constant<int, 4>{}); break;
      default: kloop(std::integral_constant<int, 5>{}); break;
    }
    __builtin_amdgcn_s_barrier();
    const int rows = min(G * 32, M - r0);
    uint4 keep[kTsG];
#pragma unroll
    for (int half = 0; half < 2; ++half) {
      if ((wave >> 2) == half) {
        const int cw = (wave & 3) * 32;
#pragma unroll
        for (int g = 0; g < kTsG; ++g) {
          if (g < G) {
            char *rowp = smem + (g * 32 + (lane & 31)) * kTsEpiStride;
#pragma unroll
            for (int rq = 0; rq < 4; ++rq) {
              float4 v = make_float4((float)acc[g][4 * rq] * scol[4 * rq] + bcol[4 * rq],
                                     (float)acc[g][4 * rq + 1] * scol[4 * rq + 1] + bcol[4 * rq + 1],
                                     (float)acc[g][4 * rq + 2] * scol[4 * rq + 2] + bcol[4 * rq + 2],
                                     (float)acc[g][4 * rq + 3] * scol[4 * rq + 3] + bcol[4 * rq + 3]);
              *reinterpret_cast<float4 *>(rowp + (cw + 8 * rq + 4 * (int)hi) * 4) = v;
            }
          }
        }
      }
      __builtin_amdgcn_s_barrier();
      if constexpr (EPI == 2) {
        auto ln_pass = [&](auto itc) __attribute__((always_inline)) {
          constexpr int it = decltype(itc)::value;
          const int r = (tid >> 4) + 32 * it;
          if (r >= rows) return;
          const int c8 = tid & 15;
          const float4 lo = *reinterpret_cast<const float4 *>(smem + r * kTsEpiStride + c8 * 32);
          const float4 hi4 = *reinterpret_cast<const float4 *>(smem + r * kTsEpiStride + c8 * 32 + 16);
          float v[8] = {lo.x, lo.y, lo.z, lo.w, hi4.x, hi4.y, hi4.z, hi4.w};
          const int col = half * 128 + c8 * 8;
          const size_t m = (size_t)(r0 + r);
          if (p.res) {
            if (p.res_i8) {
              const uint2 q = *reinterpret_cast<const uint2 *>(static_cast<const int8_t *>(p.res) + m * kTsBN + col);
#pragma unroll
              for (int c = 0; c < 4; ++c) {
                v[c] += (float)(int)(signed char)((q.x >> (8 * c)) & 0xffu) * p.s_res;
                v[4 + c] += (float)(int)(signed char)((q.y >> (8 * c)) & 0xffu) * p.s_res;
              }
            } else {
              ts_add_res(v, *reinterpret_cast<const uint4 *>(static_cast<const __half *>(p.res) + m * kTsBN + col));
            }
          }
          const uint4 o = ts_pack8(v);
          if (half == 0) {
            keep[it] = o;
          } else {
            uint4 gb[4];
            ts_ln_params(ln_lds, c8, gb);
            ts_ln_row(keep[it], o, ts_sum8(keep[it]) + ts_sum8(o), p.pk.eps, gb, static_cast<__half *>(p.out) + m * kTsBN, c8);
          }
        };
        ln_pass(std::integral_constant<int, 0>{}); ln_pass(std::integral_constant<int, 1>{});
        ln_pass(std::integral_constant<int, 2>{}); ln_pass(std::integral_constant<int, 3>{});
        ln_pass(std::integral_constant<int, 4>{});
        __builtin_amdgcn_s_barrier();
        continue;
      }
      for (int r = tid >> 4; r < rows; r += kTsThreads / 16) {
        const int c8 = tid & 15;
        const float4 lo = *reinterpret_cast<const float4 *>(smem + r * kTsEpiStride + c8 * 32);
        const float4 hi4 = *reinterpret_cast<const float4 *>(smem + r * kTsEpiStride + c8 * 32 + 16);
        float v[8] = {lo.x, lo.y, lo.z, lo.w, hi4.x, hi4.y, hi4.z, hi4.w};
        const int col = n0 + half * 128 + c8 * 8;
        const size_t m = (size_t)(r0 + r);
        if (p.res) {
          if (p.res_i8) {
            const uint2 q = *reinterpret_cast<const uint2 *>(static_cast<const int8_t *>(p.res) + m * N + col);
#pragma unroll
            for (int c = 0; c < 4; ++c) {
              v[c] += (float)(int)(signed char)((q.x >> (8 * c)) & 0xffu) * p.s_res;
              v[4 + c] += (float)(int)(signed char)((q.y >> (8 * c)) & 0xffu) * p.s_res;
            }
          } else {
            const uint4 q = *reinterpret_cast<const uint4 *>(static_cast<const __half *>(p.res) + m * N + col);
            v[0] += h2f_lo(q.x); v[1] += h2f_hi(q.x); v[2] += h2f_lo(q.y); v[3] += h2f_hi(q.y);
            v[4] += h2f_lo(q.z); v[5] += h2f_hi(q.z); v[6] += h2f_lo(q.w); v[7] += h2f_hi(q.w);
          }
        }
        if (p.relu) {
#pragma unroll
          for (int k = 0; k < 8; ++k) v[k] = fmaxf(v[k], 0.f);
        }
        if (p.out_i8) {
          unsigned pk[2] = {0, 0};
#pragma unroll
          for (int c = 0; c < 8; ++c)
            pk[c >> 2] |= ((unsigned)(int)fminf(fmaxf(rintf(v[c] * p.inv_s_out), -127.f), 127.f) & 0xffu) << (8 * (c & 3));
          *reinterpret_cast<uint2 *>(static_cast<int8_t *>(p.out) + m * N + col) = make_uint2(pk[0], pk[1]);
        } else {
          uint4 o;
          o.x = pack_h2(v[0], v[1]); o.y = pack_h2(v[2], v[3]); o.z = pack_h2(v[4], v[5]); o.w = pack_h2(v[6], v[7]);
          *reinterpret_cast<uint4 *>(static_cast<__half *>(p.out) + m * N + col) = o;
        }
      }
      __builtin_amdgcn_s_barrier();
    }
  }
}

inline int ts_grid_x(int units, int chunks_n) {
  int dev = 0, cus = 256;
  if (hipGetDevice(&dev) == hipSuccess) {
    hipDeviceProp_t p;
    static int cached[16] = {0};
    if (cached[dev & 15] == 0 && hipGetDeviceProperties(&p, dev) == hipSuccess) cached[dev & 15] = p.multiProcessorCount;
    if (cached[dev & 15] > 0) cus = cached[dev & 15];
  }
  (void)chunks_n;
  return units < cus ? units : cus;
}

thread_local int g_ts_variant = 0;
const bool g_ts_env_old = [] {
  const char *e = getenv("BEVOPS_TSGEMM_WS");
  return e && e[0] == '0' && e[1] == 0;
}();

inline bool ts_use_ws(int k) { return k <= 256 && g_ts_variant != 1 && !g_ts_env_old; }

template <int EPI, int KS, bool GRP = false>
int ws_launch_ks(const GemmCall &c, const TsPacked &pk) {
  if constexpr (GRP) {
    if (!ensure_dynamic_lds<tsgemm_ws_grouped_kernel<KS>>(ws_lds(KS))) return BEVOPS_FAILURE;
  } else {
    if (!ensure_dynamic_lds<tsgemm_ws_kernel<EPI, KS>>(ws_lds(KS))) return BEVOPS_FAILURE;
  }
  const int units = (int)((c.m + 31) / 32), chunks = c.n / kTsBN;
  const int cus = ts_grid_x(1 << 30, chunks);
  int parts = cus / chunks;
  if (parts < 1) parts = 1;
  if (GRP && parts >= 8) parts -= parts % 8;
  if (parts > units) parts = units;
  if constexpr (GRP)
    hipLaunchKernelGGL((tsgemm_ws_grouped_kernel<KS>), dim3((unsigned)(parts * chunks)), dim3(kTsThreads), ws_lds(KS), c.st,
                       (const __half *)c.x, (const __half *)c.w, (const __half *)c.bias, (__half *)c.out, (int)c.m, c.n,
                       units, parts, chunks, pk);
  else
    hipLaunchKernelGGL((tsgemm_ws_kernel<EPI, KS>), dim3((unsigned)(parts * chunks)), dim3(kTsThreads), ws_lds(KS), c.st,
                       (const __half *)c.x, (const __half *)c.w, (const __half *)c.bias, (const __half *)c.res,
                       (__half *)c.out, (int)c.m, c.n, c.relu, units, parts, chunks, pk);
  return launch_status();
}

template <int EPI>
int ts_launch_f16(const GemmCall &c, const TsPacked &pk) {
  if (ts_use_ws(c.k)) {
    if constexpr (EPI == 1) return ws_launch_ks<1, 4>(c, pk);
    else return gemm_k64<4>(c.k / 64, [&](auto ks) { return ws_launch_ks<EPI, decltype(ks)::value>(c, pk); });
  }
  if (!ensure_dynamic_lds<tsgemm_f16_kernel<EPI>>(kTsLds)) return BEVOPS_FAILURE;
  const int units = (int)((c.m + 31) / 32);
  const dim3 grid((unsigned)ts_grid_x(units, c.n / kTsBN), (unsigned)(c.n / kTsBN));
  hipLaunchKernelGGL(tsgemm_f16_kernel<EPI>, grid, dim3(kTsThreads), kTsLds, c.st, (const __half *)c.x, (const __half *)c.w,
                     (const __half *)c.bias, (const __half *)c.res, (__half *)c.out, (int)c.m, c.n, c.k, c.relu, units, pk);
  return launch_status();
}

int ts_f16_check(const GemmCall &c, bool w_limit) {
  if (c.m > 0x7fffffff || gemm_over_limit(c.m, c.k, 2) || (w_limit && gemm_over_limit(c.n, c.k, 2))) return BEVOPS_NOT_SUPPORTED;
  if (misaligned(c.x, 15u) || misaligned(c.w, 15u) || misaligned(c.out, 15u) || (c.bias && misaligned(c.bias, 15u)) ||
      (c.res && misaligned(c.res, 15u)))
    return BEVOPS_BAD_PARAM;
  return BEVOPS_SUCCESS;
}

int ts_s8_check(const GemmCallS8 &c, bool one_chunk) {
  const bool res8 = c.res && c.res_dtype == BEVOPS_I8, out8 = c.out_dtype == BEVOPS_I8;
  if (!(c.scale_a > 0.f) || (!c.w_scales && !(c.scale_w > 0.f))) return BEVOPS_BAD_PARAM;
  if (c.k % 128 != 0 || (one_chunk ? c.n != kTsBN : c.n % kTsBN != 0)) return BEVOPS_NOT_SUPPORTED;
  if (!out8 && c.out_dtype != BEVOPS_F16) return BEVOPS_NOT_SUPPORTED;
  if (c.res && !res8 && c.res_dtype != BEVOPS_F16) return BEVOPS_NOT_SUPPORTED;
  if (out8 && !(c.scale_out > 0.f)) return BEVOPS_BAD_PARAM;
  if (res8 && !(c.scale_res > 0.f)) return BEVOPS_BAD_PARAM;
  if (c.m > 0x7fffffff || gemm_over_limit(c.m, c.k, 1) || (!one_chunk && gemm_over_limit(c.n, c.k, 1))) return BEVOPS_NOT_SUPPORTED;
  if (misaligned(c.x, 15u) || misaligned(c.w, 15u) || misaligned(c.out, out8 ? 7u : 15u) ||
      (c.res && misaligned(c.res, res8 ? 7u : 15u)) || (c.bias && misaligned(c.bias, 3u)) ||
      (c.w_scales && misaligned(c.w_scales, 3u)))
    return BEVOPS_BAD_PARAM;
  return BEVOPS_SUCCESS;
}

void ts_s8_fill(TsS8Args &p, const GemmCallS8 &c) {
  p.a = static_cast<const int8_t *>(c.x); p.w = static_cast<const int8_t *>(c.w);
  p.bias = static_cast<const float *>(c.bias); p.wscale = c.w_scales; p.res = c.res; p.out = c.out;
  p.s_aw = c.w_scales ? c.scale_a : c.scale_a * c.scale_w;
  p.s_res = c.scale_res;
  p.inv_s_out = c.out_dtype == BEVOPS_I8 ? 1.0f / c.scale_out : 0.f;
  p.M = (int)c.m; p.N = c.n; p.K = c.k; p.relu = c.relu; p.units_total = (int)((c.m + 31) / 32);
  p.res_i8 = c.res && c.res_dtype == BEVOPS_I8 ? 1 : 0;
  p.out_i8 = c.out_dtype == BEVOPS_I8 ? 1 : 0;
}

TsPacked ts_ln_params(const void *ln_weight, const void *ln_bias, float eps) {
  TsPacked pk{};
  pk.gset = const_cast<char *>(static_cast<const char *>(ln_weight));
  pk.sset = const_cast<char *>(static_cast<const char *>(ln_bias));
  pk.eps = eps;
  return pk;
}

template <int KS, int KS2>
int ws2_launch_ks(const Gemm2Call &g) {
  if (!ensure_dynamic_lds<tsgemm_ws2_kernel<KS, KS2>>(ws_lds(KS))) return BEVOPS_FAILURE;
  const int units = (int)((g.m + 31) / 32), chunks = g.n / kTsBN;
  int parts = ts_grid_x(1 << 30, chunks) / chunks;
  if (parts < 1) parts = 1;
  if (parts > units) parts = units;
  const TsSrc2 src2{(const __half *)g.a2, (unsigned)((unsigned long long)g.B * g.H * g.W * g.k2 * 2), g.H, g.W, g.ho, g.wo,
                    g.stride};
  hipLaunchKernelGGL((tsgemm_ws2_kernel<KS, KS2>), dim3((unsigned)(parts * chunks)), dim3(kTsThreads), ws_lds(KS), g.st,
                     (const __half *)g.a1, (const __half *)g.w, (const __half *)g.bias, (__half *)g.out, (int)g.m, g.n, g.relu,
                     units, parts, chunks, src2);
  return launch_status();
}

}

bool tsgemm_ws2_in_domain(const Gemm2Call &g) { return g.n % kTsBN == 0 && g.k1 + g.k2 <= 256 && ts_use_ws(g.k1 + g.k2); }

int tsgemm_ws2_launch(const Gemm2Call &g) {
  return gemm_k64<4>((g.k1 + g.k2) / 64, [&](auto ks) {
    constexpr int KS = decltype(ks)::value;
    return gemm_k64<KS - 1>(g.k2 / 64, [&](auto ks2) { return ws2_launch_ks<KS, decltype(ks2)::value>(g); });
  });
}

}

using namespace bevops;

extern "C" int bevops_tsgemm_set_variant(int variant) {
  const int prev = g_ts_variant;
  g_ts_variant = variant;
  return prev;
}

extern "C" int bevops_tsgemm_tile_rows(int k) {
  if (k <= 0 || k % 64 != 0) return 0;
  return ts_use_ws(k) ? kWsRows : kTsG * 32;
}

extern "C" int bevops_tsgemm_f16(const void *x, const void *weight, const void *bias, const void *residual,
                                 void *out, long long m, int n, int k, int relu, void *stream) {
  const GemmCall c{x, weight, bias, residual, out, m, n, k, relu, static_cast<hipStream_t>(stream)};
  if (!x || !weight || !out || m <= 0 || n <= 0 || k <= 0) return BEVOPS_BAD_PARAM;
  if (k % 64 != 0 || n % kTsBN != 0) return BEVOPS_NOT_SUPPORTED;
  const int rc = ts_f16_check(c, true);
  return rc != BEVOPS_SUCCESS ? rc : ts_launch_f16<0>(c, TsPacked{});
}

extern "C" int bevops_tsgemm_f16_grouped(const void *x, const void *weight, const void *bias, void *out,
                                         long long group_stride, long long m, int groups, int k, void *stream) {
  if (!x || !weight || !out || m <= 0 || groups <= 0 || k <= 0) return BEVOPS_BAD_PARAM;
  if (k % 64 != 0 || k > 256 || groups > 64) return BEVOPS_NOT_SUPPORTED;
  const GemmCall c{x, weight, bias, nullptr, out, m, groups * kTsBN, k, 0, static_cast<hipStream_t>(stream)};
  const int rc = ts_f16_check(c, false);
  if (rc != BEVOPS_SUCCESS) return rc;
  if (group_stride < m * kTsBN || group_stride % 8 != 0) return BEVOPS_BAD_PARAM;
  if (!ts_use_ws(k)) {
    for (int g = 0; g < groups; ++g) {
      const int rc_g = bevops_tsgemm_f16(x, static_cast<const __half *>(weight) + (size_t)g * kTsBN * k,
                                         bias ? static_cast<const __half *>(bias) + (size_t)g * kTsBN : nullptr, nullptr,
                                         static_cast<__half *>(out) + (size_t)g * (size_t)group_stride, m, kTsBN, k, 0, stream);
      if (rc_g != BEVOPS_SUCCESS) return rc_g;
    }
    return BEVOPS_SUCCESS;
  }
  TsPacked pk{};
  pk.gstride = group_stride;
  return gemm_k64<4>(k / 64, [&](auto ks) { return ws_launch_ks<0, decltype(ks)::value, true>(c, pk); });
}

extern "C" int bevops_tsgemm_f16_ln(const void *x, const void *weight, const void *bias, const void *residual,
                                    const void *ln_weight, const void *ln_bias, float eps, void *out, long long m, int n,
                                    int k, void *stream) {
  const GemmCall c{x, weight, bias, residual, out, m, n, k, 0, static_cast<hipStream_t>(stream)};
  if (!x || !weight || !out || !ln_weight || !ln_bias || m <= 0 || n <= 0 || k <= 0 || !(eps >= 0.f)) return BEVOPS_BAD_PARAM;
  if (k % 64 != 0 || n != kTsBN) return BEVOPS_NOT_SUPPORTED;
  const int rc = ts_f16_check(c, false);
  if (rc != BEVOPS_SUCCESS) return rc;
  if (misaligned(ln_weight, 15u) || misaligned(ln_bias, 15u)) return BEVOPS_BAD_PARAM;
  return ts_launch_f16<2>(c, ts_ln_params(ln_weight, ln_bias, eps));
}

extern "C" int bevops_tsgemm_s8(const void *a_q, float scale_a, const void *w_q, const float *w_scales, float scale_w,
                                const float *bias, const void *residual, int res_dtype, float scale_res, int out_dtype,
                                void *out, float scale_out, long long m, int n, int k, int relu, void *stream) {
  const GemmCallS8 c{{a_q, w_q, bias, residual, out, m, n, k, relu, static_cast<hipStream_t>(stream)},
                     w_scales, scale_a, scale_w, scale_res, scale_out, res_dtype, out_dtype};
  if (!a_q || !w_q || !out || m <= 0 || n <= 0 || k <= 0) return BEVOPS_BAD_PARAM;
  const int rc = ts_s8_check(c, false);
  if (rc != BEVOPS_SUCCESS) return rc;
  if (!ensure_dynamic_lds<tsgemm_s8_kernel<0>>(kTsLds)) return BEVOPS_FAILURE;
  TsS8Args p;
  ts_s8_fill(p, c);
  const dim3 grid((unsigned)ts_grid_x(p.units_total, n / kTsBN), (unsigned)(n / kTsBN));
  hipLaunchKernelGGL(tsgemm_s8_kernel<0>, grid, dim3(kTsThreads), kTsLds, c.st, p);
  return launch_status();
}

extern "C" int bevops_tsgemm_s8_ln(const void *a_q, float scale_a, const void *w_q, const float *w_scales, float scale_w,
                                   const float *bias, const void *residual, int res_dtype, float scale_res,
                                   const void *ln_weight, const void *ln_bias, float eps, void *out, long long m, int n,
                                   int k, void *stream) {
  const GemmCallS8 c{{a_q, w_q, bias, residual, out, m, n, k, 0, static_cast<hipStream_t>(stream)},
                     w_scales, scale_a, scale_w, scale_res, 1.f, res_dtype, BEVOPS_F16};
  if (!a_q || !w_q || !out || !ln_weight || !ln_bias || m <= 0 || n <= 0 || k <= 0 || !(eps >= 0.f)) return BEVOPS_BAD_PARAM;
  const int rc = ts_s8_check(c, true);
  if (rc != BEVOPS_SUCCESS) return rc;
  if (misaligned(ln_weight, 15u) || misaligned(ln_bias, 15u)) return BEVOPS_BAD_PARAM;
  if (!ensure_dynamic_lds<tsgemm_s8_kernel<2>>(kTsS8LnLds)) return BEVOPS_FAILURE;
  TsS8LnArgs p{};
  ts_s8_fill(p, c);
  p.pk = ts_ln_params(ln_weight, ln_bias, eps);
  hipLaunchKernelGGL(tsgemm_s8_kernel<2>, dim3((unsigned)ts_grid_x(p.units_total, 1)), dim3(kTsThreads), kTsS8LnLds, c.st, p);
  return launch_status();
}

extern "C" size_t bevops_value_proj_packed_size(const int32_t *spatial_shapes_host, int num_cams, int nk, int heads,
                                                int channels, int num_levels, int num_query, int num_point) {
  if (!spatial_shapes_host || num_cams <= 0 || nk <= 0) return 0;
  if (heads <= 0 || channels != 32 || (heads * channels) % kTsBN != 0) return 0;
  const MsdaDims d{num_cams, nk, heads, channels, num_levels, num_query, num_point, 4, 1};
  Hm3Tab tab;
  size_t g_room = 0, s_bytes = 0;
  if (!msda_hm5_layout(d, spatial_shapes_host, &tab, &g_room, &s_bytes)) return 0;
  if (gemm_over_limit((unsigned long long)num_cams * nk, heads * channels, 2)) return 0;
  return msda_hm5_workspace_bytes(d, spatial_shapes_host);
}

extern "C" int bevops_value_proj_packed(const void *x, const void *weight, const void *bias,
                                        const int32_t *spatial_shapes_host, void *packed, size_t packed_bytes,
                                        int num_cams, int nk, int heads, int channels, int num_levels,
                                        int num_query, int num_point, void *stream) {
  if (!x || !weight || !spatial_shapes_host || !packed) return BEVOPS_BAD_PARAM;
  if (num_cams <= 0 || nk <= 0 || heads <= 0 || channels != 32 || (heads * channels) % kTsBN != 0) return BEVOPS_NOT_SUPPORTED;
  long total = 0;
  for (int l = 0; l < num_levels; ++l) total += (long)spatial_shapes_host[2 * l] * spatial_shapes_host[2 * l + 1];
  if (total != nk) return BEVOPS_BAD_PARAM;
  TsPacked pk{};
  size_t g_room = 0, s_bytes = 0;
  const MsdaDims d{num_cams, nk, heads, channels, num_levels, num_query, num_point, 4, 1};
  if (!msda_hm5_layout(d, spatial_shapes_host, &pk.t, &g_room, &s_bytes))
    return BEVOPS_NOT_SUPPORTED;
  if (packed_bytes < g_room + s_bytes || misaligned(packed, 127u)) return BEVOPS_BAD_PARAM;
  const int n = heads * channels;
  const GemmCall c{x, weight, bias, nullptr, nullptr, (long long)num_cams * nk, n, n, 0, static_cast<hipStream_t>(stream)};
  const int rc = ts_f16_check(c, false);
  if (rc != BEVOPS_SUCCESS) return rc;
  pk.gset = static_cast<char *>(packed);
  pk.sset = pk.gset + g_room;
  pk.nk = nk;
  pk.heads = heads;
  hipLaunchKernelGGL(tsgemm_pad_zero_kernel, dim3(4, (unsigned)(num_cams * heads)), dim3(256), 0, c.st, pk, num_cams * heads);
  return ts_launch_f16<1>(c, pk);
}

extern "C" int bevops_value_pack_planes(const void *value, const int32_t *spatial_shapes_host, void *packed,
                                        size_t packed_bytes, int num_cams, int nk, int heads, int channels,
                                        int num_levels, int num_query, int num_point, void *stream) {
  if (!value || !spatial_shapes_host || !packed) return BEVOPS_BAD_PARAM;
  TsPacked pk{};
  size_t g_room = 0, s_bytes = 0;
  const MsdaDims d{num_cams, nk, heads, channels, num_levels, num_query, num_point, 4, 1};
  if (!msda_hm5_layout(d, spatial_shapes_host, &pk.t, &g_room, &s_bytes))
    return BEVOPS_NOT_SUPPORTED;
  if (packed_bytes < g_room + s_bytes || misaligned(packed, 127u)) return BEVOPS_BAD_PARAM;
  msda_hm3_repack_launch(value, static_cast<char *>(packed), static_cast<char *>(packed) + g_room, pk.t, num_cams, nk,
                         heads, static_cast<hipStream_t>(stream));
  return launch_status();
}
```

### bevformer_tensorrt_amd/functions/__init__.py

```python
from .multi_scale_deformable_attn import (
    multi_scale_deformable_attn,
    multi_scale_deformable_attn2,
    multi_scale_deformable_attn_int8,
    multi_scale_deformable_attn_local,
    msda_pack_value,
    multi_scale_deformable_attn_prepacked,
)
from .rotate import rotate, rotate2, rotate_int8, rotate_hwc
from .grid_sampler import grid_sampler, grid_sampler2, grid_sampler_int8
from .bev_pool_v2 import bev_pool_v2, bev_pool_v2_2, bev_pool_v2_int8
from .modulated_deformable_conv2d import (modulated_deformable_conv2d, modulated_deformable_conv2d2,
                                          modulated_deformable_conv2d_int8, modulated_deformable_conv2d_nhwc,
                                          bias_act_nhwc_, bias_relu_maxpool_nhwc, conv_offset_nhwc, upsample_add_nhwc_,
                                          feat_embed_nhwc)
from .spatial_cross_attention import (spatial_cross_attention_sample, spatial_cross_attention_projected,
                                      spatial_cross_attention_plan)
from .linear import (linear_bias_act, layer_norm, quantize_rows, dequantize_rows, linear_int8, tsgemm, tsgemm_ln, tsgemm_grouped, tile_gemm, tile_gemm_dst, gemm2, small_gemm, small_gemm_dst,
                     dense_auto, tsa_split, queue_mean2)
from .int8_chain import linear_int8_chain, linear_int8_ln, conv_int8_chain_nhwc, modulated_deformable_conv2d_int8_nhwc
from .conv import conv_nhwc, conv3x3_nhwc, conv3x3_auto, conv3x3_c64, conv_int8_nhwc, stem_conv_pool
from .image import (image_normalize_pad, padded_size, bevdet_test_augmentation, bevdet_post_transform, image_resize_plan,
                    image_resize_crop_normalize, BEVFORMER_IMAGE_PIPELINES, scaled_size, scale_lidar2img,
                    image_normalize_resize_pad, DETECT2D_IMAGE_PIPELINES, keep_ratio_size, yolox_test_geometry,
                    centernet_test_geometry, image_letterbox)
from .point_sampling import point_sampling
from .attention import self_attention_qkv
from .refine import refine_reference_points, decode_boxes
from .multi_head_attn import qkv, qkv2
from .inverse import inverse
from .decode import nms_free_decode, centerpoint_decode
from .nms import bev_nms, nms_bev, circle_nms, bev_iou
from .decode2d import centernet_decode, yolox_decode, box_nms
from .lss_prepare import (lss_voxel_prepare, lss_lidar_coor, bev_pool_v2_indirect, lss_voxel_prepare_batched,
                          lss_lidar_coor_batched)
from .calibrate import calib_state_size, calib_collect, calib_threshold
from .bev_half import lss_depth_split, upsample_bilinear_concat_nhwc, lss_depth_split_q, upsample_bilinear_nhwc_q
from .deconv import conv_transpose2d_nhwc, pack_deconv4x4s2, deconv_packed_weight, conv_transpose2d_q_nhwc, quantize_deconv_weight
from .yolox_ops import (conv_slice_nhwc, conv_slice_taps, conv_slice_packed_weight, focus_nhwc, spp_maxpool_nhwc,
                        upsample_nearest2x_nhwc, pad_channels, unpad_channels, conv_slice_q_taps, focus_nhwc_q,
                        quantize_weight_taps)
from .lss_depthnet import (lss_camera_gate, se_gate2_nhwc, global_avgpool_nhwc, pack_camera_gate, camera_gate_packed,
                           se_gate2_nhwc_q, global_avgpool_nhwc_q)
from .deform_conv import deform_conv2d, deform_conv2d_nhwc, deform_conv_packed_weight
from ..utils.register import TRT_FUNCTIONS

TRT_FUNCTIONS.register_module(module=multi_scale_deformable_attn)
TRT_FUNCTIONS.register_module(module=multi_scale_deformable_attn2)
TRT_FUNCTIONS.register_module(module=multi_scale_deformable_attn_int8)
for _f in (rotate, rotate2, rotate_int8, grid_sampler, grid_sampler2, grid_sampler_int8,
           bev_pool_v2, bev_pool_v2_2, bev_pool_v2_int8, modulated_deformable_conv2d,
           modulated_deformable_conv2d2, modulated_deformable_conv2d_int8,
           spatial_cross_attention_sample, inverse, qkv, qkv2):
    TRT_FUNCTIONS.register_module(module=_f)

__all__ = [
    "multi_scale_deformable_attn",
    "multi_scale_deformable_attn2",
    "multi_scale_deformable_attn_int8",
    "rotate", "rotate2", "rotate_int8",
    "grid_sampler", "grid_sampler2", "grid_sampler_int8",
    "bev_pool_v2", "bev_pool_v2_2", "bev_pool_v2_int8",
    "modulated_deformable_conv2d", "modulated_deformable_conv2d2", "modulated_deformable_conv2d_int8",
    "inverse", "qkv", "qkv2",
    "nms_free_decode", "centerpoint_decode",
    "bev_nms", "nms_bev", "circle_nms", "bev_iou",
    "centernet_decode", "yolox_decode", "box_nms",
    "lss_voxel_prepare", "lss_lidar_coor", "bev_pool_v2_indirect", "lss_voxel_prepare_batched", "lss_lidar_coor_batched",
    "calib_state_size", "calib_collect", "calib_threshold",
    "bevdet_test_augmentation", "bevdet_post_transform", "image_resize_plan", "image_resize_crop_normalize",
    "BEVFORMER_IMAGE_PIPELINES", "scaled_size", "scale_lidar2img", "image_normalize_resize_pad",
    "DETECT2D_IMAGE_PIPELINES", "keep_ratio_size", "yolox_test_geometry", "centernet_test_geometry", "image_letterbox",
    "spatial_cross_attention_sample", "spatial_cross_attention_projected", "spatial_cross_attention_plan", "modulated_deformable_conv2d_nhwc", "bias_act_nhwc_", "linear_bias_act", "layer_norm", "rotate_hwc", "conv_offset_nhwc", "upsample_add_nhwc_", "feat_embed_nhwc",
    "msda_pack_value", "multi_scale_deformable_attn_prepacked", "multi_scale_deformable_attn_local", "image_normalize_pad", "padded_size", "quantize_rows", "dequantize_rows", "linear_int8", "tsgemm", "tsgemm_ln", "tsgemm_grouped", "tile_gemm", "tile_gemm_dst", "gemm2", "small_gemm_dst", "small_gemm", "dense_auto", "tsa_split", "queue_mean2", "conv_nhwc", "conv3x3_nhwc", "conv3x3_auto", "conv3x3_c64", "conv_int8_nhwc", "bias_relu_maxpool_nhwc", "stem_conv_pool", "point_sampling", "self_attention_qkv", "refine_reference_points", "decode_boxes",
    "linear_int8_chain", "linear_int8_ln", "conv_int8_chain_nhwc", "modulated_deformable_conv2d_int8_nhwc",
    "lss_depth_split", "upsample_bilinear_concat_nhwc", "lss_depth_split_q", "upsample_bilinear_nhwc_q",
    "conv_transpose2d_nhwc", "pack_deconv4x4s2", "deconv_packed_weight", "conv_transpose2d_q_nhwc", "quantize_deconv_weight",
    "conv_slice_nhwc", "conv_slice_taps", "conv_slice_packed_weight", "focus_nhwc", "spp_maxpool_nhwc",
    "upsample_nearest2x_nhwc", "pad_channels", "unpad_channels",
    "conv_slice_q_taps", "focus_nhwc_q", "quantize_weight_taps",
    "lss_camera_gate", "se_gate2_nhwc", "global_avgpool_nhwc", "pack_camera_gate", "camera_gate_packed",
    "se_gate2_nhwc_q", "global_avgpool_nhwc_q",
    "deform_conv2d", "deform_conv2d_nhwc", "deform_conv_packed_weight",
]
```

### bevformer_tensorrt_amd/functions/linear.py

```python
import ctypes
import os

import torch

from ..utils import lib as _lib
from ..utils import workspace as _ws
from . import dispatch as _dispatch
from .dispatch import (DENSE_LOG, DENSE_MISSES, DETERMINISTIC, OWN_KERNELS, _DENSE_CHOICE, _TABLE,
                       _dense_default, _dense_deterministic, _dense_own, _problem, _small_pays, _table, graph_time_us,
                       own_kernel_choice)


_TUNED = set()


def _tune_once(handle, key, args, x2, out_shape):
    _TUNED.add(key)
    if os.environ.get("BEVOPS_LINEAR_TUNE", "1") == "0":
        return
    scratch = torch.empty(out_shape, dtype=x2.dtype, device=x2.device)
    a = list(args)
    a[5] = scratch.data_ptr()
    handle.bevops_linear_tune(*a)


def _operands(x, weight, bias, residual, out, bias_dtype=torch.float16, res_dtypes=None, out_dtype=None):
    K, N = x.shape[-1], weight.shape[0]
    if weight.shape[1] != K:
        raise ValueError(f"weight {tuple(weight.shape)} does not match x [..., {K}]")
    x2 = x.reshape(-1, K)
    if not x2.is_contiguous():
        x2 = x2.contiguous()
    if not weight.is_contiguous():
        weight = weight.contiguous()
    M = x2.shape[0]
    r2 = None
    if residual is not None:
        if residual.dtype not in (res_dtypes or (x.dtype,)) or residual.numel() != M * N:
            raise ValueError(f"residual must be {res_dtypes or x.dtype} with M*N elements")
        r2 = residual.reshape(M, N)
        if not r2.is_contiguous():
            r2 = r2.contiguous()
    if bias is not None and (bias.dtype != bias_dtype or not bias.is_contiguous()):
        bias = bias.to(bias_dtype).contiguous()
    if out is None:
        out = torch.empty((M, N), dtype=out_dtype or x.dtype, device=x.device)
    elif out is not False:
        assert out.is_contiguous() and out.numel() == M * N and out.dtype == (out_dtype or x.dtype)
    return x2, weight, bias, r2, out, M, N, K


def _like_rows(out, x, N):
    return out.view(*x.shape[:-1], N)


def _ptr(t):
    return t.data_ptr() if t is not None else None


def _call(entry, device, *args):
    handle = _lib.load_library()
    with torch.cuda.device(device):
        st = getattr(handle, entry)(*args, _lib.current_stream_ptr(device))
    _lib.check(st, entry)


def _gemm_f16(entry, x, weight, bias, residual, relu, out, max_rows=None, launch=None):
    assert x.is_cuda and x.dtype == torch.float16 and weight.dtype == torch.float16
    x2, weight, bias, r2, out, M, N, K = _operands(x, weight, bias, residual, out)
    if max_rows is not None and M > max_rows:
        raise _lib.BevopsError(f"{entry}: more than {max_rows} rows (the tiled GEMMs' domain)", _lib.NOT_SUPPORTED)
    if M == 0:
        return _like_rows(out, x, N)
    handle = _lib.load_library()
    stream = _lib.current_stream_ptr(x.device)
    args = (x2.data_ptr(), weight.data_ptr(), _ptr(bias), _ptr(r2), out.data_ptr(), M, N, K, int(bool(relu)))
    with torch.cuda.device(x.device):
        st = getattr(handle, entry)(*args, stream) if launch is None else launch(handle, args, stream)
    _lib.check(st, entry)
    return _like_rows(out, x, N)


def linear_bias_act(x, weight, bias=None, residual=None, relu=False, out=None):
    def launch(handle, args, stream):
        nbytes = handle.bevops_linear_workspace_size() if os.environ.get("BEVOPS_LINEAR_WS", "1") != "0" else 0
        ws = _ws.lend("linear", nbytes, x.device, stream) if nbytes else None
        full = (_lib.F16,) + args + (_ptr(ws), nbytes, stream)
        key = (str(x.device),) + args[5:8] + (bool(relu), args[2] is not None, args[3] is not None)
        if key not in _TUNED and not torch.cuda.is_current_stream_capturing():
            _tune_once(handle, key, full, x, args[5:7])
        return handle.bevops_linear_bias_act(*full)
    return _gemm_f16("bevops_linear_bias_act", x, weight, bias, residual, relu, out, launch=launch)


def layer_norm(x, weight=None, bias=None, eps=1e-5, out=None):
    assert x.is_cuda and x.dtype == torch.float16
    C = x.shape[-1]
    x2 = x.reshape(-1, C)
    if not x2.is_contiguous():
        x2 = x2.contiguous()
    if out is None:
        out = torch.empty_like(x2)
    else:
        assert out.is_contiguous() and out.numel() == x2.numel() and out.dtype == x.dtype
    w = weight.to(torch.float16).contiguous() if weight is not None else None
    b = bias.to(torch.float16).contiguous() if bias is not None else None
    if x2.shape[0] == 0:
        return out.view(x.shape)
    _call("bevops_layer_norm", x.device, _lib.F16, x2.data_ptr(), _ptr(w), _ptr(b), out.data_ptr(), x2.shape[0], C, float(eps))
    return out.view(x.shape)


def _scaled_rows(entry, x, scale, out_dtype, out=None):
    x = x.contiguous()
    if x.numel() % 8:
        raise ValueError("element count must be a multiple of 8")
    if out is None:
        out = torch.empty(x.shape, dtype=out_dtype, device=x.device)
    if x.numel() == 0:
        return out
    _call(entry, x.device, _lib.F16, x.data_ptr(), out.data_ptr(), x.numel(), float(scale))
    return out


def quantize_rows(x, scale, out=None):
    assert x.is_cuda and x.dtype == torch.float16
    return _scaled_rows("bevops_quantize_rows", x, scale, torch.int8, out)


def dequantize_rows(q, scale):
    assert q.is_cuda and q.dtype == torch.int8
    return _scaled_rows("bevops_dequantize_rows", q, scale, torch.float16)


def linear_int8(a_q, scale_a, w_q, scale_w, bias=None, residual=None, relu=False, out_dtype=torch.float16,
                scale_out=1.0):
    assert a_q.is_cuda and a_q.dtype in (torch.int8, torch.float16) and w_q.dtype == torch.int8
    fused = a_q.dtype == torch.float16
    a2, w_q, b, r, out, M, N, K = _operands(a_q, w_q, bias, residual, None, bias_dtype=torch.float32,
                                            res_dtypes=(torch.float16,), out_dtype=out_dtype)
    per_channel = torch.is_tensor(scale_w)
    ws = scale_w.float().contiguous() if per_channel else None
    if M == 0:
        return _like_rows(out, a_q, N)
    _call("bevops_linear_int8_fused" if fused else "bevops_linear_int8", a_q.device,
          a2.data_ptr(), float(scale_a), w_q.data_ptr(), _ptr(ws), 1.0 if per_channel else float(scale_w), _ptr(b),
          _ptr(r), _lib.torch_dtype_code(out), out.data_ptr(), float(scale_out), M, N, K, int(bool(relu)))
    return _like_rows(out, a_q, N)


def tsgemm(x, weight, bias=None, residual=None, relu=False, out=None):
    return _gemm_f16("bevops_tsgemm_f16", x, weight, bias, residual, relu, out)


def tsgemm_grouped(x, weight, bias=None, out=None):
    assert x.is_cuda and x.dtype == torch.float16 and weight.dtype == torch.float16
    x2, weight, bias, _, _, M, N, K = _operands(x, weight, bias, None, False)
    if N % 256 != 0 or N == 0:
        raise ValueError(f"weight {tuple(weight.shape)} must be [G * 256, {K}]")
    G = N // 256
    if out is None:
        out = torch.empty((G, M, 256), dtype=x.dtype, device=x.device)
    else:
        assert out.is_contiguous() and tuple(out.shape) == (G, M, 256) and out.dtype == x.dtype
    if M == 0:
        return out
    _call("bevops_tsgemm_f16_grouped", x.device, x2.data_ptr(), weight.data_ptr(), _ptr(bias), out.data_ptr(), M * 256, M, G, K)
    return out


def tsgemm_ln(x, weight, bias, residual, ln_weight, ln_bias, eps=1e-5):
    g, b = ln_weight.to(torch.float16).contiguous(), ln_bias.to(torch.float16).contiguous()
    return _gemm_f16("bevops_tsgemm_f16_ln", x, weight, bias, residual, False, None, launch=lambda handle, a, stream:
                     handle.bevops_tsgemm_f16_ln(*a[:4], g.data_ptr(), b.data_ptr(), float(eps), *a[4:8], stream))


def tile_gemm(x, weight, bias=None, residual=None, relu=False, out=None):
    return _gemm_f16("bevops_tile_gemm_f16", x, weight, bias, residual, relu, out)


class _GemmDst(ctypes.Structure):
    _fields_ = [("col_begin", ctypes.c_int), ("col_end", ctypes.c_int), ("out", ctypes.c_void_p),
                ("out_pitch", ctypes.c_longlong), ("res", ctypes.c_void_p), ("res_pitch", ctypes.c_longlong)]


def tile_gemm_dst(x, weight, bias, widths, residuals=None, relu=False, outs=None, _entry="bevops_tile_gemm_f16_dst"):
    assert x.is_cuda and x.dtype == torch.float16 and weight.dtype == torch.float16
    x2, weight, bias, _, _, M, N, K = _operands(x, weight, bias, None, False)
    if sum(widths) != N:
        raise ValueError(f"weight {tuple(weight.shape)} does not match widths {list(widths)}")
    if outs is None:
        outs = [torch.empty((M, n), dtype=x.dtype, device=x.device) for n in widths]
    residuals = residuals if residuals is not None else [None] * len(widths)
    if M == 0:
        return outs
    tab = (_GemmDst * len(widths))()
    col = 0
    for i, n in enumerate(widths):
        o, r = outs[i], residuals[i]
        assert o.dtype == x.dtype and tuple(o.shape) == (M, n) and (n == 1 or o.stride(1) == 1)
        tab[i].col_begin, tab[i].col_end, tab[i].out, tab[i].out_pitch = col, col + n, o.data_ptr(), o.stride(0) if M > 1 else n
        if r is not None:
            if r.dtype != x.dtype or tuple(r.shape) != (M, n) or r.stride(1) != 1:
                raise ValueError("residual must be fp16 [M, width] with unit column stride")
            tab[i].res, tab[i].res_pitch = r.data_ptr(), r.stride(0) if M > 1 else n
        col += n
    _call(_entry, x.device, x2.data_ptr(), weight.data_ptr(), _ptr(bias), ctypes.addressof(tab), len(widths), M, N, K,
          int(bool(relu)))
    return outs


def gemm2(a1, a2, weight, bias=None, stride=1, relu=False, out=None):
    assert a1.is_cuda and a1.dtype == torch.float16 and a2.dtype == torch.float16 and weight.dtype == torch.float16
    if a2.dim() != 4 or not a2.is_contiguous(memory_format=torch.channels_last):
        raise ValueError("a2 must be a 4-d tensor in channels-last memory")
    B, K2, H, W = a2.shape
    K1, N = a1.shape[-1], weight.shape[0]
    if weight.shape[1] != K1 + K2:
        raise ValueError(f"weight {tuple(weight.shape)} does not match [N, {K1} + {K2}]")
    x1 = a1.reshape(-1, K1)
    if not x1.is_contiguous():
        x1 = x1.contiguous()
    if not weight.is_contiguous():
        weight = weight.contiguous()
    if bias is not None and (bias.dtype != torch.float16 or not bias.is_contiguous()):
        bias = bias.to(torch.float16).contiguous()
    M = x1.shape[0]
    if out is None:
        out = torch.empty((M, N), dtype=a1.dtype, device=a1.device)
    else:
        assert out.is_contiguous() and out.numel() == M * N and out.dtype == a1.dtype
    if M == 0:
        return out
    _call("bevops_gemm2_f16", a1.device, x1.data_ptr(), a2.data_ptr(), weight.data_ptr(), _ptr(bias), out.data_ptr(), M, N,
          K1, K2, B, H, W, int(stride), int(bool(relu)))
    return out


def small_gemm_dst(x, weight, bias, widths, residuals=None, relu=False, outs=None):
    if x.numel() // x.shape[-1] > 8192:
        raise _lib.BevopsError("small_gemm_dst: more than 8192 rows (the tiled GEMMs' domain)", _lib.NOT_SUPPORTED)
    return tile_gemm_dst(x, weight, bias, widths, residuals, relu, outs, _entry="bevops_small_gemm_f16_dst")


def tsgemm_weight_stationary(K):
    return _lib.load_library().bevops_tsgemm_tile_rows(int(K)) == 64


def small_gemm(x, weight, bias=None, residual=None, relu=False, out=None):
    return _gemm_f16("bevops_small_gemm_f16", x, weight, bias, residual, relu, out, max_rows=8192)


def _torch_dense(x, weight, bias, residual, relu):
    if residual is not None or bias is None:
        raise _lib.BevopsError("torch addmm path: bias required, no identity term", _lib.NOT_SUPPORTED)
    x2 = x.reshape(-1, x.shape[-1])
    y = torch._addmm_activation(bias, x2, weight.t()) if relu else torch.addmm(bias, x2, weight.t())
    return y.view(*x.shape[:-1], weight.shape[0])


_DENSE = {"tsgemm": tsgemm, "tile": tile_gemm, "small": small_gemm, "blaslt": linear_bias_act, "torch": _torch_dense}


def dense_auto(x, weight, bias=None, residual=None, relu=False):
    K, N = x.shape[-1], weight.shape[0]
    M = x.numel() // K
    if M == 0:
        return x.new_empty((*x.shape[:-1], N))
    key = (str(x.device), M, N, K, bool(relu), bias is not None, residual is not None)
    name, keep, miss = _dispatch.dense_choice(key, DETERMINISTIC["enabled"], OWN_KERNELS["enabled"],
                                              torch.cuda.is_current_stream_capturing, _dispatch._tune, _table(_TABLE),
                                              _DENSE_CHOICE.get(key))
    if miss and _problem(key) not in DENSE_MISSES:
        DENSE_MISSES.append(_problem(key))
    if name == "measure":
        name = _dense_measure(key, x, weight, bias, residual, relu)
    if keep:
        _DENSE_CHOICE[key] = name
    try:
        return _DENSE[name](x, weight, bias, residual, relu)
    except _lib.BevopsError as exc:
        if exc.status != _lib.NOT_SUPPORTED or name == "blaslt":
            raise
        return linear_bias_act(x, weight, bias, residual, relu)


def _dense_measure(key, x, weight, bias, residual, relu, rounds=3, iters=8):
    with torch.cuda.device(x.device):
        times = _dispatch.measure(_DENSE, lambda name: _DENSE[name](x, weight, bias, residual, relu), iters, rounds)
    DENSE_LOG.append((key, {k: round(v, 1) for k, v in times.items()}))
    return min(times, key=times.get) if times else "blaslt"


def tsa_split(both, heads, points):
    assert both.is_cuda and both.dtype == torch.float16 and both.dim() == 2 and both.is_contiguous()
    nq = both.shape[0]
    assert both.shape[1] == heads * 2 * points * 3
    off = torch.empty((2, nq, heads, points * 2), dtype=both.dtype, device=both.device)
    w = torch.empty((2, nq, heads, points), dtype=both.dtype, device=both.device)
    _call("bevops_tsa_split", both.device, _lib.F16, both.data_ptr(), off.data_ptr(), w.data_ptr(), nq, heads, points)
    return off, w


def queue_mean2(x):
    assert x.is_cuda and x.dtype == torch.float16 and x.shape[0] == 2 and x.is_contiguous()
    out = torch.empty((1,) + tuple(x.shape[1:]), dtype=x.dtype, device=x.device)
    if out.numel() == 0:
        return out
    _call("bevops_queue_mean2", x.device, _lib.F16, x.data_ptr(), out.data_ptr(), out.numel())
    return out
```

### bevformer_tensorrt_amd/utils/lib.py

```python
import ctypes
import os

_PKG = os.path.dirname(os.path.dirname(os.path.abspath(__file__)))
_LIB = None

c_int, c_float, c_void_p, c_size_t = ctypes.c_int, ctypes.c_float, ctypes.c_void_p, ctypes.c_size_t

SIGNATURES = {
    "bevops_version": (ctypes.c_char_p, []),
    "bevops_status_string": (ctypes.c_char_p, [c_int]),
    "bevops_query": (c_void_p, [ctypes.c_char_p]),
    "bevops_msda_set_variant": (c_int, [c_int]),
    "bevops_msda_forward": (c_int, [c_int, c_void_p, c_void_p, c_void_p, c_void_p, c_int,
                                    c_void_p, c_void_p, c_void_p] + [c_int] * 8 +
                            [c_float] * 4 + [c_void_p]),
    "bevops_msda_workspace_size": (c_size_t, [c_int] * 8),
    "bevops_msda_workspace_size_shapes": (c_size_t, [c_int, c_void_p] + [c_int] * 7),
    "bevops_msda_forward_ws": (c_int, [c_int, c_void_p, c_void_p, c_void_p, c_void_p, c_int,
                                       c_void_p, c_void_p, c_void_p] + [c_int] * 8 +
                               [c_float] * 4 + [c_int, c_void_p, c_size_t, c_void_p]),
    "bevops_msda_packed_size": (c_size_t, [c_int, c_void_p] + [c_int] * 7),
    "bevops_msda_pack_value": (c_int, [c_int, c_int, c_void_p, c_void_p, c_void_p, c_size_t] + [c_int] * 7 + [c_void_p]),
    "bevops_msda_forward_prepacked": (c_int, [c_int, c_void_p, c_size_t, c_void_p, c_void_p, c_int, c_void_p, c_void_p,
                                              c_void_p] + [c_int] * 8 + [c_float] * 4 + [c_int, c_void_p]),
    "bevops_sca_workspace_size": (c_size_t, [c_int, c_void_p] + [c_int] * 7),
    "bevops_sca_forward": (c_int, [c_int] + [c_void_p] * 7 + [c_int] * 8 + [c_void_p, c_size_t, c_void_p]),
    "bevops_rotate_forward": (c_int, [c_int, c_void_p, c_void_p, c_void_p, c_int, c_void_p,
                                      c_int, c_int, c_int, c_int, c_float, c_float, c_void_p]),
    "bevops_grid_sampler_2d_forward": (c_int, [c_int, c_void_p, c_void_p, c_void_p] + [c_int] * 9 +
                                       [c_float] * 3 + [c_void_p]),
    "bevops_grid_sampler_2d_workspace_size": (c_size_t, [c_int] * 5),
    "bevops_grid_sampler_2d_forward_ws": (c_int, [c_int, c_void_p, c_void_p, c_void_p] + [c_int] * 9 +
                                          [c_float] * 3 + [c_void_p, c_size_t, c_void_p]),
    "bevops_bev_pool_v2_forward": (c_int, [c_int] + [c_void_p] * 8 + [c_int] * 4 + [c_float] * 3 +
                                   [c_void_p]),
    "bevops_mdconv_set_variant": (c_int, [c_int]),
    "bevops_mdconv_workspace_size": (c_size_t, [c_int] * 16),
    "bevops_mdconv_forward_int8": (c_int, [c_void_p, c_float, c_void_p, c_float, c_void_p, c_float,
                                           c_void_p, c_float, c_void_p, c_void_p, c_float, c_void_p,
                                           c_size_t] + [c_int] * 15 + [c_void_p]),
    "bevops_mdconv_forward_int8_packed": (c_int, [c_void_p, c_float, c_void_p, c_float, c_void_p, c_float,
                                           c_void_p, c_float, c_void_p, c_void_p, c_float, c_void_p,
                                           c_size_t] + [c_int] * 15 + [c_void_p]),
    "bevops_mdconv_forward": (c_int, [c_int] + [c_void_p] * 7 + [c_size_t] + [c_int] * 15 +
                              [c_void_p]),
    "bevops_mdconv_forward_packed": (c_int, [c_int] + [c_void_p] * 7 + [c_size_t] + [c_int] * 15 +
                                     [c_void_p]),
    "bevops_mdconv_forward_nhwc": (c_int, [c_int] + [c_void_p] * 6 + [c_int, c_int, c_void_p, c_size_t] + [c_int] * 15 +
                                   [c_void_p]),
    "bevops_bias_act_nhwc": (c_int, [c_int, c_void_p, c_void_p, c_void_p, c_size_t, c_int, c_int, c_void_p]),
    "bevops_value_proj_packed_size": (c_size_t, [c_void_p] + [c_int] * 7),
    "bevops_value_proj_packed": (c_int, [c_void_p] * 5 + [c_size_t] + [c_int] * 7 + [c_void_p]),
    "bevops_value_pack_planes": (c_int, [c_void_p, c_void_p, c_void_p, c_size_t] + [c_int] * 7 + [c_void_p]),
    "bevops_sca_prepacked_workspace_size": (c_size_t, [c_int] * 4),
    "bevops_sca_forward_prepacked": (c_int, [c_int, c_void_p, c_size_t] + [c_void_p] * 6 + [c_int] * 8 +
                                     [c_void_p, c_size_t, c_void_p]),
    "bevops_sca_plan_size": (c_size_t, [c_int, c_int]),
    "bevops_sca_plan_build": (c_int, [c_int, c_void_p, c_int, c_int, c_void_p, c_size_t, c_void_p]),
    "bevops_sca_forward_planned": (c_int, [c_int, c_void_p, c_size_t] + [c_void_p] * 6 + [c_size_t, c_void_p] + [c_int] * 8 +
                                   [c_void_p, c_size_t, c_void_p]),
    "bevops_point_sampling": (c_int, [c_int, c_void_p, c_void_p, c_void_p, c_void_p, c_int, c_int, c_int, c_float, c_float,
                                      c_void_p]),
    "bevops_tsgemm_f16": (c_int, [c_void_p] * 5 + [ctypes.c_longlong, c_int, c_int, c_int, c_void_p]),
    "bevops_tsgemm_f16_grouped": (c_int, [c_void_p] * 4 + [ctypes.c_longlong, ctypes.c_longlong, c_int, c_int, c_void_p]),
    "bevops_tsgemm_set_variant": (c_int, [c_int]),
    "bevops_tsgemm_tile_rows": (c_int, [c_int]),
    "bevops_tsgemm_f16_ln": (c_int, [c_void_p] * 6 + [c_float, c_void_p, ctypes.c_longlong, c_int, c_int, c_void_p]),
    "bevops_mha_selfattn_max_queries": (c_size_t, []),
    "bevops_mha_selfattn_f16": (c_int, [c_void_p, c_void_p, c_int, c_int, c_int, c_float, c_void_p]),
    "bevops_tsgemm_s8": (c_int, [c_void_p, c_float, c_void_p, c_void_p, c_float, c_void_p, c_void_p, c_int, c_float, c_int,
                                 c_void_p, c_float, ctypes.c_longlong, c_int, c_int, c_int, c_void_p]),
    "bevops_tsgemm_s8_ln": (c_int, [c_void_p, c_float, c_void_p, c_void_p, c_float, c_void_p, c_void_p, c_int, c_float,
                                    c_void_p, c_void_p, c_float, c_void_p, ctypes.c_longlong, c_int, c_int, c_void_p]),
    "bevops_tsa_split": (c_int, [c_int, c_void_p, c_void_p, c_void_p, c_int, c_int, c_int, c_void_p]),
    "bevops_queue_mean2": (c_int, [c_int, c_void_p, c_void_p, c_size_t, c_void_p]),
    "bevops_upsample_add_nhwc": (c_int, [c_int, c_void_p, c_void_p] + [c_int] * 6 + [c_void_p]),
    "bevops_lss_depth_split": (c_int, [c_int, c_void_p, c_void_p, c_void_p] + [c_int] * 7 + [c_void_p]),
    "bevops_upsample_bilinear_concat_nhwc": (c_int, [c_int, c_void_p, c_void_p, c_void_p] + [c_int] * 7 + [c_void_p]),
    "bevops_lss_depth_split_s8": (c_int, [c_void_p, c_void_p, c_void_p] + [c_int] * 7 + [c_float, c_float, c_void_p]),
    "bevops_upsample_bilinear_s8": (c_int, [c_void_p, c_int, c_float, c_void_p, c_int, c_float] + [c_int] * 6 +
                                    [c_void_p]),
    "bevops_feat_embed_nhwc": (c_int, [c_int, c_void_p, c_void_p, c_void_p, c_void_p, c_int, c_size_t, c_int, c_size_t,
                                       c_void_p]),
    "bevops_conv3x3_c32_set_variant": (c_int, [c_int]),
    "bevops_conv3x3_c32_packed_weight_size": (c_size_t, [c_int, c_int]),
    "bevops_conv3x3_c32_pack_weight": (c_int, [c_int, c_void_p, c_void_p, c_int, c_int, c_void_p]),
    "bevops_conv3x3_c32_forward_nhwc": (c_int, [c_int, c_void_p, c_void_p, c_void_p, c_void_p, c_int, c_int, c_int,
                                                c_int, c_void_p]),
    "bevops_rotate_set_variant": (c_int, [c_int]),
    "bevops_rotate_forward_hwc": (c_int, [c_int, c_void_p, c_void_p, c_void_p, c_int, c_void_p,
                                          c_int, c_int, c_int, c_int, c_void_p]),
    "bevops_layer_norm": (c_int, [c_int, c_void_p, c_void_p, c_void_p, c_void_p, c_size_t, c_int, c_float, c_void_p]),
    "bevops_linear_workspace_size": (c_size_t, []),
    "bevops_linear_bias_act": (c_int, [c_int] + [c_void_p] * 5 + [ctypes.c_longlong, c_int, c_int, c_int,
                                                                  c_void_p, c_size_t, c_void_p]),
    "bevops_image_normalize_pad": (c_int, [c_int, c_void_p, c_int, c_void_p] + [c_int] * 5 +
                                   [ctypes.POINTER(ctypes.c_double), ctypes.POINTER(ctypes.c_double), c_int, c_int, c_void_p]),
    "bevops_image_normalize_resize_pad": (c_int, [c_int, c_void_p, c_int, c_void_p] + [c_int] * 7 +
                                          [ctypes.POINTER(ctypes.c_double), ctypes.POINTER(ctypes.c_double), c_int, c_int,
                                           c_void_p]),
    "bevops_image_letterbox": (c_int, [c_int, c_void_p, c_int, c_void_p] + [c_int] * 9 +
                               [ctypes.POINTER(ctypes.c_double)] * 3 + [c_int, c_int, c_void_p]),
    "bevops_image_resize_plan_size": (c_size_t, [c_int] * 8),
    "bevops_image_resize_plan_build": (c_int, [c_int] * 8 + [c_void_p, c_size_t]),
    "bevops_image_resize_crop_normalize": (c_int, [c_void_p, c_void_p, c_size_t, c_int, c_void_p, c_void_p] + [c_int] * 10 +
                                           [ctypes.POINTER(ctypes.c_double), ctypes.POINTER(ctypes.c_double), c_int, c_int,
                                            c_int, c_void_p]),
    "bevops_quantize_rows": (c_int, [c_int, c_void_p, c_void_p, c_size_t, c_float, c_void_p]),
    "bevops_dequantize_rows": (c_int, [c_int, c_void_p, c_void_p, c_size_t, c_float, c_void_p]),
    "bevops_linear_int8": (c_int, [c_void_p, c_float, c_void_p, c_void_p, c_float, c_void_p, c_void_p, c_int, c_void_p,
                                   c_float, ctypes.c_longlong, c_int, c_int, c_int, c_void_p]),
    "bevops_linear_int8_fused": (c_int, [c_void_p, c_float, c_void_p, c_void_p, c_float, c_void_p, c_void_p, c_int, c_void_p,
                                         c_float, ctypes.c_longlong, c_int, c_int, c_int, c_void_p]),
    "bevops_small_gemm_f16": (c_int, [c_void_p] * 5 + [ctypes.c_longlong, c_int, c_int, c_int, c_void_p]),
    "bevops_tile_gemm_f16": (c_int, [c_void_p] * 5 + [ctypes.c_longlong, c_int, c_int, c_int, c_void_p]),
    "bevops_tile_gemm_f16_dst": (c_int, [c_void_p] * 4 + [c_int, ctypes.c_longlong, c_int, c_int, c_int, c_void_p]),
    "bevops_gemm2_f16": (c_int, [c_void_p] * 5 + [ctypes.c_longlong] + [c_int] * 8 + [c_void_p]),
    "bevops_small_gemm_f16_dst": (c_int, [c_void_p] * 4 + [c_int, ctypes.c_longlong, c_int, c_int, c_int, c_void_p]),
    "bevops_conv_tile_f16": (c_int, [c_void_p] * 5 + [c_int] * 8 + [c_void_p]),
    "bevops_conv3x3_c64_f16": (c_int, [c_void_p] * 4 + [c_int] * 6 + [c_void_p]),
    "bevops_deconv4x4s2_packed_weight_size": (c_size_t, [c_int] * 3),
    "bevops_deconv4x4s2_pack_weight": (c_int, [c_int, c_void_p, c_void_p, c_int, c_int, c_void_p]),
    "bevops_deconv4x4s2_f16": (c_int, [c_int] + [c_void_p] * 4 + [c_int] * 9 + [c_void_p]),
    "bevops_conv_slice_f16": (c_int, [c_void_p, c_int, c_void_p, c_void_p, c_void_p, c_int, c_void_p] + [c_int] * 9 +
                              [c_void_p]),
    "bevops_conv_slice_f16_ex": (c_int, [c_void_p, c_int, c_void_p, c_void_p, c_void_p, c_int, c_void_p] + [c_int] * 11 +
                                 [c_void_p]),
    "bevops_lss_camera_gate_packed_size": (c_size_t, [c_int]),
    "bevops_lss_camera_gate": (c_int, [c_void_p, c_int, c_void_p, c_void_p, c_int, c_int, c_void_p]),
    "bevops_se_gate2_nhwc": (c_int, [c_void_p, c_int, c_void_p, c_void_p, c_int, c_void_p] + [c_int] * 4 + [c_void_p]),
    "bevops_global_avgpool_nhwc": (c_int, [c_void_p, c_int, c_void_p] + [c_int] * 4 + [c_void_p]),
    "bevops_focus_nhwc": (c_int, [c_void_p, c_void_p] + [c_int] * 4 + [c_void_p]),
    "bevops_spp_maxpool_nhwc": (c_int, [c_void_p, c_int, c_void_p] + [c_int] * 8 + [c_void_p]),
    "bevops_upsample_nearest2x_nhwc": (c_int, [c_void_p, c_int, c_void_p] + [c_int] * 5 + [c_void_p]),
    "bevops_conv_slice_s8": (c_int, [c_void_p, c_int, c_float, c_void_p, c_void_p, c_float, c_void_p, c_void_p, c_int,
                                     c_float, c_int, c_void_p, c_int, c_float] + [c_int] * 8 + [c_void_p]),
    "bevops_conv_slice_s8_ex": (c_int, [c_void_p, c_int, c_float, c_void_p, c_void_p, c_float, c_void_p, c_void_p, c_int,
                                        c_float, c_int, c_void_p, c_int, c_float] + [c_int] * 9 + [c_void_p]),
    "bevops_conv_slice_s8_ex2": (c_int, [c_void_p, c_int, c_float, c_void_p, c_void_p, c_float, c_void_p, c_void_p, c_int,
                                         c_float, c_int, c_void_p, c_int, c_float] + [c_int] * 10 + [c_void_p, c_int, c_void_p]),
    "bevops_se_gate2_nhwc_s8": (c_int, [c_void_p, c_int, c_float, c_void_p, c_void_p, c_int, c_float, c_void_p, c_int,
                                        c_float] + [c_int] * 3 + [c_void_p]),
    "bevops_global_avgpool_nhwc_s8": (c_int, [c_void_p, c_int, c_float, c_void_p] + [c_int] * 4 + [c_void_p]),
    "bevops_deconv4x4s2_s8": (c_int, [c_void_p, c_float, c_void_p, c_void_p, c_float, c_void_p, c_int, c_void_p, c_float] +
                              [c_int] * 6 + [c_void_p]),
    "bevops_focus_nhwc_q": (c_int, [c_void_p, c_float, c_void_p] + [c_int] * 4 + [c_void_p]),
    "bevops_spp_maxpool_nhwc_s8": (c_int, [c_void_p, c_int, c_void_p] + [c_int] * 8 + [c_void_p]),
    "bevops_upsample_nearest2x_nhwc_s8": (c_int, [c_void_p, c_int, c_void_p] + [c_int] * 5 + [c_void_p]),
    "bevops_refine_reference_points": (c_int, [c_int] + [c_void_p] * 4 + [c_int] * 2 + [c_void_p] * 3),
    "bevops_decode_boxes": (c_int, [c_int] + [c_void_p] * 3 + [c_int] + [c_float] * 6 + [c_void_p] * 3),
    "bevops_bias_relu_maxpool_nhwc": (c_int, [c_int, c_void_p, c_void_p, c_void_p, c_int, c_int, c_int, c_int, c_void_p]),
    "bevops_stem_packed_size": (c_size_t, []),
    "bevops_stem_pack": (c_int, [c_int, c_void_p, c_void_p, c_void_p, c_void_p]),
    "bevops_stem_conv_pool": (c_int, [c_int, c_int, c_void_p, c_void_p, c_void_p, c_int, c_int, c_int, c_float, c_void_p]),
    "bevops_stem_set_variant": (c_int, [c_int]),
    "bevops_conv_tile_int8_fused": (c_int, [c_void_p, c_float, c_void_p, c_void_p, c_float, c_void_p, c_void_p, c_void_p]
                                    + [c_int] * 8 + [c_void_p]),
    "bevops_linear_int8_chain": (c_int, [c_void_p, c_int, c_float, c_void_p, c_void_p, c_float, c_void_p, c_void_p, c_int,
                                         c_float, c_int, c_void_p, c_float, ctypes.c_longlong, c_int, c_int, c_int, c_void_p]),
    "bevops_conv_tile_int8": (c_int, [c_void_p, c_float, c_void_p, c_void_p, c_float, c_void_p, c_void_p, c_int, c_void_p,
                                      c_float] + [c_int] * 8 + [c_void_p]),
    "bevops_bias_relu_maxpool_nhwc_int8": (c_int, [c_int, c_void_p, c_void_p, c_void_p, c_float, c_int, c_int, c_int, c_int,
                                                   c_void_p]),
    "bevops_mdconv_int8_nhwc_workspace_size": (c_size_t, []),
    "bevops_mdconv_forward_int8_nhwc": (c_int, [c_void_p, c_float, c_void_p, c_int, c_float, c_float, c_void_p, c_float,
                                                c_void_p, c_void_p, c_float, c_int, c_int, c_void_p, c_size_t] + [c_int] * 15 +
                                        [c_void_p]),
    "bevops_linear_tune": (c_int, [c_int] + [c_void_p] * 5 + [ctypes.c_longlong, c_int, c_int, c_int,
                                                              c_void_p, c_size_t, c_void_p]),
    "bevops_mdconv_packed_weight_size": (c_size_t, [c_int] * 5),
    "bevops_mdconv_pack_weight": (c_int, [c_int, c_void_p, c_void_p] + [c_int] * 4 + [c_void_p]),
    "bevops_grid_sampler_3d_forward": (c_int, [c_int, c_void_p, c_void_p, c_void_p] + [c_int] * 11 +
                                       [c_void_p]),
    "bevops_qkv_workspace_size": (c_size_t, [c_int] * 5),
    "bevops_qkv_forward": (c_int, [c_int, c_void_p, c_void_p, c_void_p, c_void_p] + [c_int] * 4 + [c_float] * 4 +
                           [c_void_p, c_size_t, c_void_p]),
    "bevops_inverse_forward": (c_int, [c_int, c_void_p, c_void_p, c_int, c_int, c_void_p]),
    "bevops_nms_free_decode": (c_int, [c_int] + [c_void_p] * 6 + [c_int] * 4 + [c_void_p, c_float, c_int, c_void_p]),
    "bevops_centerpoint_decode_workspace_size": (c_size_t, [c_int] * 5),
    "bevops_centerpoint_decode": (c_int, [c_int] + [c_void_p] * 11 + [c_int] * 5 + [c_float] * 5 +
                                  [c_void_p, c_float, c_int, c_int, c_void_p, c_size_t, c_void_p]),
    "bevops_centerpoint_decode_ex": (c_int, [c_int] + [c_void_p] * 11 + [c_int] * 5 + [c_float] * 5 +
                                     [c_void_p, c_float, c_int, c_int, c_void_p, c_size_t, c_void_p]),
    "bevops_bev_nms_workspace_size": (c_size_t, [c_int, c_int]),
    "bevops_bev_nms": (c_int, [c_int] + [c_void_p] * 9 + [c_int] * 4 + [c_float, c_void_p, c_int, c_int, c_void_p,
                                                                        c_size_t, c_void_p]),
    "bevops_bev_iou": (c_int, [c_void_p, c_int, c_void_p, c_int, c_void_p, c_void_p]),
    "bevops_centernet_decode_workspace_size": (c_size_t, [c_int] * 5),
    "bevops_centernet_decode": (c_int, [c_int] + [c_void_p] * 8 + [c_int] * 8 + [c_void_p, c_void_p, c_float, c_void_p,
                                                                               c_size_t, c_void_p]),
    "bevops_yolox_decode": (c_int, [c_int] + [c_void_p] * 8 + [c_int] * 3 + [c_void_p, c_void_p]),
    "bevops_box_nms_workspace_size": (c_size_t, [c_int, c_int]),
    "bevops_box_nms": (c_int, [c_void_p] * 9 + [c_int, c_int, c_float, c_float, c_int, c_int, c_void_p, c_size_t,
                                                c_void_p]),
    "bevops_lss_voxel_prepare_workspace_size": (c_size_t, [c_int] * 4),
    "bevops_lss_voxel_prepare": (c_int, [c_void_p] * 10 + [c_int] * 5 + [c_void_p, c_size_t, c_void_p]),
    "bevops_lss_voxel_prepare_batched_workspace_size": (c_size_t, [c_int] * 5),
    "bevops_lss_voxel_prepare_batched": (c_int, [c_void_p] * 10 + [c_int] * 5 + [c_void_p, c_size_t, c_void_p]),
    "bevops_bev_pool_v2_forward_indirect": (c_int, [c_int] + [c_void_p] * 9 + [c_int] * 4 + [c_float] * 3 + [c_void_p]),
    "bevops_calib_state_size": (c_size_t, []),
    "bevops_calib_collect": (c_int, [c_int, c_void_p, c_size_t, c_void_p, c_void_p]),
    "bevops_calib_threshold_workspace_size": (c_size_t, [c_int]),
    "bevops_calib_threshold": (c_int, [c_int, ctypes.c_double, c_void_p, c_int, c_size_t, c_void_p, c_void_p, c_void_p,
                                       c_size_t, c_void_p]),
    "bevops_deform_conv3x3_nhwc_f16": (c_int, [c_void_p, c_void_p, c_int, c_void_p, c_void_p, c_void_p] + [c_int] * 7 +
                                       [c_void_p]),
}

F32, F16, I8, U8 = 0, 1, 2, 3


def lib_path():
    return os.environ.get("BEVOPS_LIB", os.path.join(_PKG, "libbevops_hip.so"))


def load_library():
    global _LIB
    if _LIB is not None:
        return _LIB
    path = lib_path()
    if not os.path.exists(path):
        raise RuntimeError(
            f"{path} not found: build the HIP kernels first "
            "(`python -c 'import __graft_entry__ as g; g.build()'` or "
            "`make -C bevformer_tensorrt_amd/csrc`). There is no fallback path.")
    import torch
    handle = ctypes.CDLL(os.path.realpath(path))
    for name, (res, args) in SIGNATURES.items():
        fn = getattr(handle, name)
        fn.restype, fn.argtypes = res, args
    _LIB = handle
    return handle


SUCCESS, FAILURE, BAD_PARAM, NOT_SUPPORTED, NOT_INITIALIZED = range(5)


class BevopsError(RuntimeError):

    def __init__(self, message, status):
        super().__init__(message)
        self.status = status


def check(status, what):
    if status != 0:
        msg = load_library().bevops_status_string(status).decode()
        raise BevopsError(f"{what}: {msg} (status {status})", status)


def torch_dtype_code(t):
    import torch
    code = {torch.float32: F32, torch.float16: F16, torch.int8: I8}.get(t.dtype)
    if code is None:
        raise TypeError(f"unsupported dtype {t.dtype}; expected float32, float16 or int8")
    return code


def current_stream_ptr(device):
    import torch
    return torch.cuda.current_stream(device).cuda_stream
```

### include/bevops.h

```cpp
#ifndef BEVOPS_H_
#define BEVOPS_H_

#include <stddef.h>
#include <stdint.h>

#ifdef __cplusplus
extern "C" {
#endif

typedef enum {
  BEVOPS_SUCCESS = 0,
  BEVOPS_FAILURE = 1,
  BEVOPS_BAD_PARAM = 2,
  BEVOPS_NOT_SUPPORTED = 3,
  BEVOPS_NOT_INITIALIZED = 4
} bevops_status_t;

typedef enum { BEVOPS_F32 = 0, BEVOPS_F16 = 1, BEVOPS_I8 = 2, BEVOPS_U8 = 3  } bevops_dtype_t;

typedef enum { BEVOPS_BILINEAR = 0, BEVOPS_NEAREST = 1, BEVOPS_BICUBIC = 2 } bevops_interp_t;
typedef enum { BEVOPS_PAD_ZEROS = 0, BEVOPS_PAD_BORDER = 1, BEVOPS_PAD_REFLECTION = 2 } bevops_pad_t;

const char *bevops_version(void);
const char *bevops_status_string(int status);
void *bevops_query(const char *name);

int bevops_msda_forward(int dtype, const void *value, const int32_t *spatial_shapes,
                        const int32_t *spatial_shapes_host, const void *reference_points,
                        int ref_dtype, const void *sampling_offsets,
                        const void *attention_weights, void *output, int bs, int nk,
                        int heads, int channels, int num_levels, int num_query,
                        int num_point, int points_per_group, float scale_value,
                        float scale_offset, float scale_weight, float scale_out,
                        void *stream);

size_t bevops_msda_workspace_size(int dtype, int bs, int nk, int heads, int channels,
                                  int num_levels, int num_query, int num_point);
size_t bevops_msda_workspace_size_shapes(int dtype, const int32_t *spatial_shapes_host, int bs,
                                         int nk, int heads, int channels, int num_levels,
                                         int num_query, int num_point);
int bevops_msda_forward_ws(int dtype, const void *value, const int32_t *spatial_shapes,
                           const int32_t *spatial_shapes_host, const void *reference_points,
                           int ref_dtype, const void *sampling_offsets,
                           const void *attention_weights, void *output, int bs, int nk,
                           int heads, int channels, int num_levels, int num_query,
                           int num_point, int points_per_group, float scale_value,
                           float scale_offset, float scale_weight, float scale_out,
                           int shared_offsets, void *workspace, size_t workspace_bytes,
                           void *stream);

int bevops_msda_set_variant(int variant);


int bevops_rotate_forward(int dtype, const void *img, const void *angle, const void *center,
                          int angle_dtype, void *output, int channels, int height, int width,
                          int interpolation, float scale_in, float scale_out, void *stream);

int bevops_grid_sampler_2d_forward(int dtype, const void *input, const void *grid, void *output,
                                   int N, int C, int H_in, int W_in, int H_out, int W_out,
                                   int interpolation, int padding, int align_corners,
                                   float scale_in, float scale_grid, float scale_out,
                                   void *stream);
size_t bevops_grid_sampler_2d_workspace_size(int dtype, int N, int C, int H_in, int W_in);
int bevops_grid_sampler_2d_forward_ws(int dtype, const void *input, const void *grid, void *output,
                                      int N, int C, int H_in, int W_in, int H_out, int W_out,
                                      int interpolation, int padding, int align_corners,
                                      float scale_in, float scale_grid, float scale_out,
                                      void *workspace, size_t workspace_bytes, void *stream);
int bevops_grid_sampler_3d_forward(int dtype, const void *input, const void *grid, void *output,
                                   int N, int C, int D_in, int H_in, int W_in, int D_out,
                                   int H_out, int W_out, int interpolation, int padding,
                                   int align_corners, void *stream);

int bevops_bev_pool_v2_forward(int dtype, const void *depth, const void *feat,
                               const int32_t *ranks_depth, const int32_t *ranks_feat,
                               const int32_t *ranks_bev, const int32_t *interval_starts,
                               const int32_t *interval_lengths, void *output, int channels,
                               int n_intervals, int out_height, int out_width,
                               float scale_depth, float scale_feat, float scale_out,
                               void *stream);

size_t bevops_sca_workspace_size(int dtype, const int32_t *spatial_shapes_host, int num_cams, int nk,
                                 int heads, int channels, int num_levels, int num_query,
                                 int num_point);
int bevops_sca_forward(int dtype, const void *value, const int32_t *spatial_shapes_host,
                       const void *reference_points_cam, const void *sampling_offsets,
                       const void *attention_weights, const void *bev_mask, void *output,
                       int num_cams, int nk, int heads, int channels, int num_levels, int num_query,
                       int num_point, int points_per_group, void *workspace, size_t workspace_bytes,
                       void *stream);

int bevops_mdconv_set_variant(int variant);
size_t bevops_mdconv_workspace_size(int dtype, int B, int Cin, int H, int W, int Cout, int Kh,
                                    int Kw, int stride_h, int stride_w, int pad_h, int pad_w,
                                    int dil_h, int dil_w, int groups, int deform_groups);
int bevops_mdconv_forward_int8(const void *input, float scale_in, const void *offset,
                               float scale_offset, const void *mask, float scale_mask,
                               const void *weight, float scale_weight, const float *bias,
                               void *output, float scale_out, void *workspace,
                               size_t workspace_bytes, int B, int Cin, int H, int W, int Cout, int Kh,
                               int Kw, int stride_h, int stride_w, int pad_h, int pad_w, int dil_h,
                               int dil_w, int groups, int deform_groups, void *stream);
int bevops_mdconv_forward_int8_packed(const void *input, float scale_in, const void *offset,
                                      float scale_offset, const void *mask, float scale_mask,
                                      const void *packed_weight, float scale_weight, const float *bias,
                                      void *output, float scale_out, void *workspace,
                                      size_t workspace_bytes, int B, int Cin, int H, int W, int Cout, int Kh,
                                      int Kw, int stride_h, int stride_w, int pad_h, int pad_w, int dil_h,
                                      int dil_w, int groups, int deform_groups, void *stream);
int bevops_mdconv_forward(int dtype, const void *input, const void *offset, const void *mask,
                          const void *weight, const void *bias, void *output, void *workspace,
                          size_t workspace_bytes, int B, int Cin, int H, int W, int Cout, int Kh,
                          int Kw, int stride_h, int stride_w, int pad_h, int pad_w, int dil_h,
                          int dil_w, int groups, int deform_groups, void *stream);
size_t bevops_mdconv_packed_weight_size(int dtype, int Cout, int Cin_per_group, int Kh, int Kw);
int bevops_mdconv_pack_weight(int dtype, const void *weight, void *packed, int Cout,
                              int Cin_per_group, int Kh, int Kw, void *stream);
int bevops_mdconv_forward_nhwc(int dtype, const void *input_nhwc, const void *offset,
                               const void *mask, const void *packed_weight, const void *bias,
                               void *output_nhwc, int relu, int offset_mask_channels,
                               void *workspace, size_t workspace_bytes,
                               int B, int Cin, int H, int W, int Cout, int Kh, int Kw, int stride_h,
                               int stride_w, int pad_h, int pad_w, int dil_h, int dil_w, int groups,
                               int deform_groups, void *stream);
int bevops_bias_act_nhwc(int dtype, void *x, const void *bias, const void *residual, size_t rows,
                         int channels, int relu, void *stream);
int bevops_bias_relu_maxpool_nhwc(int dtype, const void *x, const void *bias, void *out, int n, int h, int w,
                                  int channels, void *stream);
size_t bevops_stem_packed_size(void);
int bevops_stem_pack(int dtype, const void *weight, const void *bias, void *packed, void *stream);
int bevops_stem_conv_pool(int dtype, int out_dtype, const void *x, const void *packed, void *out, int n, int h, int w,
                          float scale_out, void *stream);
int bevops_stem_set_variant(int variant);

int bevops_upsample_add_nhwc(int dtype, void *a, const void *b, int n, int h, int w, int hb, int wb,
                             int channels, void *stream);

int bevops_lss_depth_split(int dtype, const void *x, void *depth, void *feat, int n, int hw, int row_stride,
                           int depth_offset, int D, int feat_offset, int C, void *stream);

int bevops_upsample_bilinear_concat_nhwc(int dtype, const void *a, const void *b, void *out, int n, int h, int w,
                                         int ca, int hb, int wb, int cb, void *stream);

int bevops_lss_depth_split_s8(const void *x_f16, void *depth_q, void *feat_q, int n, int hw, int row_stride,
                              int depth_offset, int D, int feat_offset, int C, float scale_depth, float scale_feat,
                              void *stream);

int bevops_upsample_bilinear_s8(const void *b_q, int b_pitch, float scale_b, void *out_q, int out_pitch, float scale_out,
                                int n, int h, int w, int hb, int wb, int C, void *stream);

int bevops_feat_embed_nhwc(int dtype, const void *src, const void *cam_embed, const void *level_embed, void *dst,
                           int n, size_t rows, int channels, size_t dst_batch_stride, void *stream);
size_t bevops_conv3x3_c32_packed_weight_size(int dtype, int Cin);
int bevops_conv3x3_c32_pack_weight(int dtype, const void *weight, void *packed, int Cout, int Cin, void *stream);
int bevops_conv3x3_c32_set_variant(int variant);
int bevops_conv3x3_c32_forward_nhwc(int dtype, const void *input_nhwc, const void *packed_weight,
                                    const void *bias32, void *output_nhwc, int B, int H, int W, int Cin,
                                    void *stream);
int bevops_rotate_set_variant(int variant);
int bevops_tsa_split(int dtype, const void *both, void *offsets, void *weights, int num_query, int heads, int points,
                     void *stream);
int bevops_queue_mean2(int dtype, const void *x, void *out, size_t count, void *stream);
int bevops_rotate_forward_hwc(int dtype, const void *img, const void *angle, const void *center,
                              int angle_dtype, void *output, int channels, int height, int width,
                              int interpolation, void *stream);
int bevops_layer_norm(int dtype, const void *x, const void *gamma, const void *beta, void *out,
                      size_t rows, int channels, float eps, void *stream);
int bevops_quantize_rows(int dtype, const void *x, void *q, size_t count, float scale, void *stream);
int bevops_dequantize_rows(int dtype, const void *q, void *out, size_t count, float scale, void *stream);
int bevops_linear_int8(const void *a_q, float scale_a, const void *w_q, const float *w_scales,
                       float scale_w, const float *bias, const void *residual, int out_dtype,
                       void *out, float scale_out, long long M, int N, int K, int relu, void *stream);
int bevops_linear_int8_fused(const void *x_f16, float scale_a, const void *w_q, const float *w_scales,
                             float scale_w, const float *bias, const void *residual, int out_dtype,
                             void *out, float scale_out, long long M, int N, int K, int relu, void *stream);
int bevops_tile_gemm_f16(const void *x, const void *weight, const void *bias, const void *residual,
                         void *out, long long M, int N, int K, int relu, void *stream);
int bevops_gemm2_f16(const void *a1, const void *a2, const void *weight, const void *bias, void *out, long long M, int N,
                     int K1, int K2, int a2_B, int a2_H, int a2_W, int a2_stride, int relu, void *stream);
typedef struct bevops_gemm_dst {
  int col_begin, col_end;
  void *out;
  long long out_pitch;
  const void *res;
  long long res_pitch;
} bevops_gemm_dst;
int bevops_tile_gemm_f16_dst(const void *x, const void *weight, const void *bias, const bevops_gemm_dst *dst, int num_dst,
                             long long M, int N, int K, int relu, void *stream);
int bevops_small_gemm_f16_dst(const void *x, const void *weight, const void *bias, const bevops_gemm_dst *dst, int num_dst,
                              long long M, int N, int K, int relu, void *stream);
int bevops_conv_tile_f16(const void *x, const void *weight_taps, const void *bias, const void *residual,
                         void *out, int B, int H, int W, int Cin, int Cout, int ksize, int stride, int relu,
                         void *stream);
int bevops_conv3x3_c64_f16(const void *x, const void *weight_taps, const void *bias, void *out, int B, int H, int W,
                           int Cin, int Cout, int relu, void *stream);
size_t bevops_deconv4x4s2_packed_weight_size(int dtype, int Cin, int Cout);
int bevops_deconv4x4s2_pack_weight(int dtype, const void *weight, void *packed, int Cin, int Cout, void *stream);
int bevops_deconv4x4s2_f16(int dtype, const void *x, const void *packed_weight, const void *bias, void *out, int B, int H,
                           int W, int Cin, int Cout, int ksize, int stride, int pad, int relu, void *stream);
int bevops_conv_slice_f16(const void *x, int x_pitch, const void *weight_taps, const void *bias, const void *residual,
                          int res_pitch, void *out, int out_pitch, int B, int H, int W, int Cin, int Cout, int ksize,
                          int stride, int act, void *stream);
int bevops_conv_slice_f16_ex(const void *x, int x_pitch, const void *weight_taps, const void *bias, const void *residual,
                             int res_pitch, void *out, int out_pitch, int B, int H, int W, int Cin, int Cout, int ksize,
                             int stride, int act, int dilation, int bias_pitch, void *stream);
size_t bevops_lss_camera_gate_packed_size(int mid);
int bevops_lss_camera_gate(const float *mlp_input, int in_pitch, const void *packed, float *gates, int n, int mid,
                           void *stream);
int bevops_se_gate2_nhwc(const void *x, int x_pitch, const float *gates, void *out_a, int a_pitch, void *out_b,
                         int b_pitch, int n, int hw, int c, void *stream);
int bevops_global_avgpool_nhwc(const void *x, int x_pitch, void *out, int out_pitch, int n, int hw, int c, void *stream);
int bevops_focus_nhwc(const void *image, void *out, int out_pitch, int B, int H, int W, void *stream);
int bevops_spp_maxpool_nhwc(const void *x, int x_pitch, void *out, int out_pitch, int B, int H, int W, int C, int k0,
                            int k1, int k2, void *stream);
int bevops_upsample_nearest2x_nhwc(const void *x, int x_pitch, void *out, int out_pitch, int B, int H, int W, int C,
                                   void *stream);
int bevops_conv_slice_s8(const void *x_q, int x_pitch, float scale_a, const void *w_q_taps, const float *w_scales,
                         float scale_w, const float *bias, const void *residual_q, int res_pitch, float scale_res,
                         int out_dtype, void *out, int out_pitch, float scale_out, int B, int H, int W, int Cin, int Cout,
                         int ksize, int stride, int act, void *stream);
int bevops_conv_slice_s8_ex(const void *x_q, int x_pitch, float scale_a, const void *w_q_taps, const float *w_scales,
                            float scale_w, const float *bias, const void *residual_q, int res_pitch, float scale_res,
                            int out_dtype, void *out, int out_pitch, float scale_out, int B, int H, int W, int Cin, int Cout,
                            int ksize, int stride, int act, int res_first, void *stream);
int bevops_conv_slice_s8_ex2(const void *x_q, int x_pitch, float scale_a, const void *w_q_taps, const float *w_scales,
                             float scale_w, const float *bias, const void *residual_q, int res_pitch, float scale_res,
                             int out_dtype, void *out, int out_pitch, float scale_out, int B, int H, int W, int Cin, int Cout,
                             int ksize, int stride, int act, int res_first, int dilation, const void *image_bias_f16,
                             int image_bias_pitch, void *stream);
int bevops_se_gate2_nhwc_s8(const void *x_q, int x_pitch, float scale_x, const float *gates, void *out_a, int a_pitch,
                            float scale_a, void *out_b, int b_pitch, float scale_b, int n, int hw, int c, void *stream);
int bevops_global_avgpool_nhwc_s8(const void *x_q, int x_pitch, float scale_x, void *out, int out_pitch, int n, int hw,
                                  int c, void *stream);
int bevops_deconv4x4s2_s8(const void *x_q, float scale_a, const void *packed_w_q, const float *w_scales, float scale_w,
                          const float *bias, int out_dtype, void *out, float scale_out, int B, int H, int W, int Cin,
                          int Cout, int relu, void *stream);
int bevops_focus_nhwc_q(const void *image, float scale, void *out, int out_pitch, int B, int H, int W, void *stream);
int bevops_spp_maxpool_nhwc_s8(const void *x, int x_pitch, void *out, int out_pitch, int B, int H, int W, int C, int k0,
                               int k1, int k2, void *stream);
int bevops_upsample_nearest2x_nhwc_s8(const void *x, int x_pitch, void *out, int out_pitch, int B, int H, int W, int C,
                                      void *stream);
int bevops_refine_reference_points(int dtype, const void *tmp, const void *reference_points, void *new_reference_points,
                                   void *reference_xy, int num_query, int tmp_stride, const void *log_table,
                                   const void *sigmoid_table, void *stream);
int bevops_decode_boxes(int dtype, const void *regs, const void *refs, void *out, int count, float scale_x, float offset_x,
                        float scale_y, float offset_y, float scale_z, float offset_z, const void *log_table,
                        const void *sigmoid_table, void *stream);
int bevops_conv_tile_int8_fused(const void *x_f16, float scale_a, const void *w_q_taps, const float *w_scales,
                                float scale_w, const float *bias, const void *residual, void *out, int B, int H,
                                int W, int Cin, int Cout, int ksize, int stride, int relu, void *stream);
int bevops_linear_int8_chain(const void *a, int a_dtype, float scale_a, const void *w_q, const float *w_scales,
                             float scale_w, const float *bias, const void *residual, int res_dtype, float scale_res,
                             int out_dtype, void *out, float scale_out, long long M, int N, int K, int relu,
                             void *stream);
int bevops_conv_tile_int8(const void *x_q, float scale_a, const void *w_q_taps, const float *w_scales, float scale_w,
                          const float *bias, const void *residual, int out_dtype, void *out, float scale_out, int B,
                          int H, int W, int Cin, int Cout, int ksize, int stride, int relu, void *stream);
int bevops_bias_relu_maxpool_nhwc_int8(int dtype, const void *x, const void *bias, void *out_q, float scale_out,
                                       int n, int h, int w, int channels, void *stream);
size_t bevops_mdconv_int8_nhwc_workspace_size(void);
int bevops_mdconv_forward_int8_nhwc(const void *input_nhwc, float scale_in, const void *offset_mask_nhwc,
                                    int offset_mask_channels, float scale_offset, float scale_mask,
                                    const void *packed_weight, float scale_weight, const float *bias,
                                    void *output_nhwc, float scale_out, int relu, int exact, void *workspace,
                                    size_t workspace_bytes, int B, int Cin, int H, int W, int Cout, int Kh, int Kw,
                                    int stride_h, int stride_w, int pad_h, int pad_w, int dil_h, int dil_w,
                                    int groups, int deform_groups, void *stream);
int bevops_image_normalize_pad(int in_dtype, const void *images, int out_dtype, void *output, int N,
                               int H0, int W0, int Hp, int Wp, const double *mean_host,
                               const double *std_host, int to_rgb, int channels_last, void *stream);
size_t bevops_image_resize_plan_size(int H0, int W0, int resize_w, int resize_h, int crop_x0, int crop_y0,
                                     int crop_x1, int crop_y1);
int bevops_image_resize_plan_build(int H0, int W0, int resize_w, int resize_h, int crop_x0, int crop_y0, int crop_x1,
                                   int crop_y1, void *plan_host, size_t plan_bytes);
int bevops_image_resize_crop_normalize(const void *images, const void *plan_dev, size_t plan_bytes, int out_dtype,
                                       void *output, void *canvas_or_null, int N, int H0, int W0, int resize_w,
                                       int resize_h, int crop_x0, int crop_y0, int crop_x1, int crop_y1, int rotate,
                                       const double *mean_host, const double *std_host, int to_rgb, int flip,
                                       int channels_last, void *stream);
int bevops_image_normalize_resize_pad(int in_dtype, const void *images, int out_dtype, void *output, int N,
                                      int H0, int W0, int Hs, int Ws, int Hp, int Wp, const double *mean_host,
                                      const double *std_host, int to_rgb, int channels_last, void *stream);
int bevops_image_letterbox(int arith, const void *images, int out_dtype, void *output, int N, int H0, int W0, int Hs,
                           int Ws, int Hp, int Wp, int oy, int ox, const double *pad_host, const double *mean_host,
                           const double *std_host, int to_rgb, int channels_last, void *stream);
size_t bevops_msda_packed_size(int dtype, const int32_t *spatial_shapes_host, int bs, int nk, int heads,
                               int channels, int num_levels, int num_query, int num_point);
int bevops_msda_pack_value(int dtype, int ref_dtype, const void *value, const int32_t *spatial_shapes_host,
                           void *packed, size_t packed_bytes, int bs, int nk, int heads, int channels,
                           int num_levels, int num_query, int num_point, void *stream);
int bevops_msda_forward_prepacked(int dtype, const void *packed, size_t packed_bytes,
                                  const int32_t *spatial_shapes_host, const void *reference_points,
                                  int ref_dtype, const void *sampling_offsets, const void *attention_weights,
                                  void *output, int bs, int nk, int heads, int channels, int num_levels,
                                  int num_query, int num_point, int points_per_group, float scale_value,
                                  float scale_offset, float scale_weight, float scale_out, int shared_offsets,
                                  void *stream);
size_t bevops_linear_workspace_size(void);
int bevops_linear_bias_act(int dtype, const void *a, const void *weight, const void *bias,
                           const void *residual, void *out, long long M, int N, int K, int relu,
                           void *workspace, size_t workspace_bytes, void *stream);
size_t bevops_value_proj_packed_size(const int32_t *spatial_shapes_host, int num_cams, int nk, int heads, int channels,
                                     int num_levels, int num_query, int num_point);
int bevops_value_proj_packed(const void *x, const void *weight, const void *bias, const int32_t *spatial_shapes_host,
                             void *packed, size_t packed_bytes, int num_cams, int nk, int heads, int channels,
                             int num_levels, int num_query, int num_point, void *stream);
int bevops_value_pack_planes(const void *value, const int32_t *spatial_shapes_host, void *packed, size_t packed_bytes,
                             int num_cams, int nk, int heads, int channels, int num_levels, int num_query,
                             int num_point, void *stream);
size_t bevops_sca_prepacked_workspace_size(int num_cams, int heads, int channels, int num_query);
int bevops_sca_forward_prepacked(int dtype, const void *packed, size_t packed_bytes, const int32_t *spatial_shapes_host,
                                 const void *reference_points_cam, const void *sampling_offsets,
                                 const void *attention_weights, const void *bev_mask, void *output, int num_cams,
                                 int nk, int heads, int channels, int num_levels, int num_query, int num_point,
                                 int points_per_group, void *workspace, size_t workspace_bytes, void *stream);
size_t bevops_sca_plan_size(int num_cams, int num_query);
int bevops_sca_plan_build(int dtype, const void *bev_mask, int num_cams, int num_query, void *plan, size_t plan_bytes,
                          void *stream);
int bevops_sca_forward_planned(int dtype, const void *packed, size_t packed_bytes, const int32_t *spatial_shapes_host,
                               const void *reference_points_cam, const void *sampling_offsets,
                               const void *attention_weights, const void *bev_mask, const void *plan, size_t plan_bytes,
                               void *output, int num_cams, int nk, int heads, int channels, int num_levels,
                               int num_query, int num_point, int points_per_group, void *workspace,
                               size_t workspace_bytes, void *stream);

int bevops_point_sampling(int out_dtype, const float *pillars, const float *lidar2img, void *reference_points_cam,
                          void *bev_mask, int num_cams, int num_query, int num_points_in_pillar, float image_h,
                          float image_w, void *stream);

int bevops_tsgemm_f16(const void *x, const void *weight, const void *bias, const void *residual, void *out,
                      long long m, int n, int k, int relu, void *stream);
int bevops_tsgemm_set_variant(int variant);
int bevops_tsgemm_tile_rows(int k);
int bevops_tsgemm_f16_grouped(const void *x, const void *weight, const void *bias, void *out, long long group_stride,
                              long long m, int groups, int k, void *stream);
int bevops_tsgemm_f16_ln(const void *x, const void *weight, const void *bias, const void *residual, const void *ln_weight,
                         const void *ln_bias, float eps, void *out, long long m, int n, int k, void *stream);
size_t bevops_mha_selfattn_max_queries(void);
int bevops_mha_selfattn_f16(const void *qkv, void *out, int num_query, int heads, int head_dim, float scale, void *stream);
int bevops_tsgemm_s8(const void *a_q, float scale_a, const void *w_q, const float *w_scales, float scale_w,
                     const float *bias, const void *residual, int res_dtype, float scale_res, int out_dtype,
                     void *out, float scale_out, long long m, int n, int k, int relu, void *stream);
int bevops_tsgemm_s8_ln(const void *a_q, float scale_a, const void *w_q, const float *w_scales, float scale_w,
                        const float *bias, const void *residual, int res_dtype, float scale_res,
                        const void *ln_weight, const void *ln_bias, float eps, void *out, long long m, int n, int k,
                        void *stream);

int bevops_small_gemm_f16(const void *x, const void *weight, const void *bias, const void *residual, void *out,
                          long long m, int n, int k, int relu, void *stream);

int bevops_linear_tune(int dtype, const void *a, const void *weight, const void *bias,
                       const void *residual, void *out, long long M, int N, int K, int relu,
                       void *workspace, size_t workspace_bytes, void *stream);
int bevops_mdconv_forward_packed(int dtype, const void *input, const void *offset,
                                 const void *mask, const void *packed_weight, const void *bias,
                                 void *output, void *workspace, size_t workspace_bytes, int B,
                                 int Cin, int H, int W, int Cout, int Kh, int Kw, int stride_h,
                                 int stride_w, int pad_h, int pad_w, int dil_h, int dil_w,
                                 int groups, int deform_groups, void *stream);

size_t bevops_qkv_workspace_size(int dtype, int batch, int q_len, int kv_len, int embed_dim);
int bevops_qkv_forward(int dtype, const void *query, const void *key, const void *value, void *output, int batch,
                       int q_len, int kv_len, int embed_dim, float scale_q, float scale_k, float scale_v,
                       float scale_o, void *workspace, size_t workspace_bytes, void *stream);

int bevops_inverse_forward(int dtype, const void *input, void *output, int batch, int n, void *stream);

int bevops_nms_free_decode(int dtype, const void *cls_logits, const void *bbox_preds, float *boxes, float *scores,
                           int32_t *labels, int32_t *count, int batch, int num_query, int num_classes, int max_num,
                           const float *post_center_range_host, float score_threshold, int bottom_center,
                           void *stream);
size_t bevops_centerpoint_decode_workspace_size(int batch, int num_classes, int height, int width, int max_num);
int bevops_centerpoint_decode(int dtype, const void *reg, const void *height, const void *dim, const void *rot,
                              const void *vel, const void *heatmap, const int32_t *strides_host, float *boxes,
                              float *scores, int32_t *labels, int32_t *count, int batch, int num_classes, int map_h,
                              int map_w, int max_num, float out_size_factor, float voxel_x, float voxel_y, float pc_x,
                              float pc_y, const float *post_center_range_host, float score_threshold, int norm_bbox,
                              int heatmap_is_score, void *workspace, size_t workspace_bytes, void *stream);
int bevops_centerpoint_decode_ex(int dtype, const void *reg, const void *height, const void *dim, const void *rot,
                                 const void *vel, const void *heatmap, const int64_t *strides_host, float *boxes,
                                 float *scores, int32_t *labels, int32_t *count, int batch, int num_classes, int map_h,
                                 int map_w, int max_num, float out_size_factor, float voxel_x, float voxel_y,
                                 float pc_x, float pc_y, const float *post_center_range_host, float score_threshold,
                                 int norm_bbox, int heatmap_is_score, void *workspace, size_t workspace_bytes,
                                 void *stream);

size_t bevops_bev_nms_workspace_size(int batch, int num);
int bevops_bev_nms(int mode, const float *boxes_in, const float *scores_in, const int32_t *labels_in,
                   const int32_t *count_in, float *boxes, float *scores, int32_t *labels, int32_t *count,
                   int32_t *index, int batch, int num, int pre_max_size, int post_max_size, float threshold,
                   const float *rescale_factor_host, int num_factors, int bottom_center, void *workspace,
                   size_t workspace_bytes, void *stream);
int bevops_bev_iou(const float *boxes_a, int num_a, const float *boxes_b, int num_b, float *iou, void *stream);

size_t bevops_centernet_decode_workspace_size(int batch, int num_classes, int height, int width, int k);
int bevops_centernet_decode(int dtype, const void *heatmap, const void *wh, const void *offset,
                            const int32_t *strides_host, float *boxes, float *scores, int32_t *labels, int32_t *count,
                            int batch, int num_classes, int map_h, int map_w, int k, int kernel, int inp_h, int inp_w,
                            const float *border_host, const float *scale_factor_host, float score_threshold,
                            void *workspace, size_t workspace_bytes, void *stream);
int bevops_yolox_decode(int dtype, const void *const *cls_host, const void *const *bbox_host,
                        const void *const *obj_host, const int32_t *level_shapes_host, const int32_t *strides_host,
                        float *boxes, float *scores, int32_t *labels, int batch, int num_levels, int num_classes,
                        const float *scale_factor_host, void *stream);
size_t bevops_box_nms_workspace_size(int batch, int num);
int bevops_box_nms(const float *boxes_in, const float *scores_in, const int32_t *labels_in, const int32_t *count_in,
                   float *boxes, float *scores, int32_t *labels, int32_t *count, int32_t *index, int batch, int num,
                   float score_threshold, float iou_threshold, int class_aware, int max_out, void *workspace,
                   size_t workspace_bytes, void *stream);

size_t bevops_lss_voxel_prepare_workspace_size(int n_cams, int d, int h, int w);
int bevops_lss_voxel_prepare(const float *frustum, const float *calib, const float *grid_host, int32_t *ranks_bev,
                             int32_t *ranks_depth, int32_t *ranks_feat, int32_t *interval_starts,
                             int32_t *interval_lengths, int32_t *counts, float *coor, int batch, int n_cams, int d,
                             int h, int w, void *workspace, size_t workspace_bytes, void *stream);
size_t bevops_lss_voxel_prepare_batched_workspace_size(int batch, int n_cams, int d, int h, int w);
int bevops_lss_voxel_prepare_batched(const float *frustum, const float *calib, const float *grid_host,
                                     int32_t *ranks_bev, int32_t *ranks_depth, int32_t *ranks_feat,
                                     int32_t *interval_starts, int32_t *interval_lengths, int32_t *counts, float *coor,
                                     int batch, int n_cams, int d, int h, int w, void *workspace,
                                     size_t workspace_bytes, void *stream);
int bevops_bev_pool_v2_forward_indirect(int dtype, const void *depth, const void *feat, const int32_t *ranks_depth,
                                        const int32_t *ranks_feat, const int32_t *ranks_bev,
                                        const int32_t *interval_starts, const int32_t *interval_lengths,
                                        const int32_t *n_intervals_dev, void *output, int channels, int max_intervals,
                                        int out_height, int out_width, float scale_depth, float scale_feat,
                                        float scale_out, void *stream);

size_t bevops_calib_state_size(void);
int bevops_calib_collect(int dtype, const void *x, size_t count, void *state, void *stream);
size_t bevops_calib_threshold_workspace_size(int num_states);
int bevops_calib_threshold(int method, double percentile, const void *states, int num_states, size_t state_stride,
                           int32_t *bins, double *kl, void *workspace, size_t workspace_bytes, void *stream);

int bevops_deform_conv3x3_nhwc_f16(const void *input_nhwc, const void *offset_nhwc, int offset_channels,
                                   const void *packed_weight, const void *bias, void *output_nhwc, int relu,
                                   int B, int H, int W, int Cin, int Cout, int groups, void *stream);

#ifdef __cplusplus
}
#endif
#endif
```

Measured before the change: 101.5.

## Chain bottleneck conv3 with next block's conv1 in one weight-stationary GEMM kernel

Adds a chained GEMM kernel in which each tile of one bottleneck's conv3 output (plus residual or downsample source) stays in LDS and immediately feeds a second MFMA GEMM for the next block's conv1, with optional stride-2 subsampling on the second output. The ResNet stage loop now looks one block ahead and passes the precomputed conv1 activation forward. This removes one kernel launch and a re-read of the 256-channel activation per chained block pair, at the cost of more registers and LDS in the kernel and added dispatch complexity. It applies only to the early-stage shapes listed in the whitelist.

New measurement: 102.5, median of 6. No clear change (+0.9%).

```diff
diff --git a/bevformer_tensorrt_amd/bevformer.py b/bevformer_tensorrt_amd/bevformer.py
--- a/bevformer_tensorrt_amd/bevformer.py
+++ b/bevformer_tensorrt_amd/bevformer.py
@@ -8,7 +8,7 @@
 
 from . import functions as _hip_ops
 from . import geometry as G
-from .functions.dispatch import OWN_KERNELS, own_kernel_choice, using as _dispatch_using
+from .functions.dispatch import DETERMINISTIC, OWN_KERNELS, _small_pays, own_kernel_choice, using as _dispatch_using
 from .functions.linear import tsgemm_weight_stationary
 from .utils import lib as _lib
 
@@ -289,6 +289,37 @@
     return hit[1], hit[2]
 
 
+_CONV_CHAIN = {"enabled": os.environ.get("BEVOPS_CONV_CHAIN", "1") != "0"}
+_CONV_CHAIN_SHAPES = {(64, 0, 256, 64, 1), (64, 64, 256, 64, 1), (64, 0, 256, 128, 1), (64, 0, 256, 128, 2)}
+
+
+def _plain_1x1(conv):
+    return type(conv) is nn.Conv2d and not hasattr(conv, "lin") and conv.bias is not None \
+        and conv.weight.dtype == torch.float16 and conv.kernel_size == (1, 1) and conv.stride[0] == conv.stride[1]
+
+
+def _conv_chain_ok(ops, blk, nxt, x):
+    if nxt is None or not (_CONV_CHAIN["enabled"] and _R3["enabled"] and _FUSED_LINEAR["enabled"]) \
+            or getattr(ops, "gemm_chain", None) is None or getattr(blk, "chain_cal", None) is not None \
+            or getattr(nxt, "chain_cal", None) is not None or type(blk) is not Bottleneck or type(nxt) is not Bottleneck:
+        return False
+    c3, c1 = blk.conv3, nxt.conv1
+    if not (_plain_1x1(c3) and _plain_1x1(c1)) or c3.stride != (1, 1) or c1.in_channels != c3.out_channels:
+        return False
+    if x.dtype != torch.float16 or not x.is_cuda or x.dim() != 4 or not x.is_contiguous(memory_format=torch.channels_last):
+        return False
+    if blk.downsample is not None and not _two_source_ok(ops, blk, x):
+        return False
+    k2 = 0 if blk.downsample is None else blk.downsample.in_channels
+    if DETERMINISTIC["enabled"]:
+        sb = 1 if blk.downsample is None else blk.downsample.stride[0]
+        m = x.shape[0] * ((x.shape[2] - 1) // sb + 1) * ((x.shape[3] - 1) // sb + 1)
+        if (k2 == 0 and _small_pays(m, c3.out_channels, c3.in_channels)) \
+                or (c1.stride[0] == 1 and _small_pays(m, c1.out_channels, c1.in_channels)):
+            return False
+    return (c3.in_channels, k2, c3.out_channels, c1.out_channels, c1.stride[0]) in _CONV_CHAIN_SHAPES
+
+
 class Bottleneck(nn.Module):
 
     def __init__(self, cin, planes, stride, dcn, ops, downsample, style="caffe"):
@@ -305,23 +336,42 @@
         out = F.relu(self.conv2(out), inplace=True)
         return F.relu(self.conv3(out) + idt, inplace=True)
 
-    def _hidden_nhwc(self, x, ops):
-        out = _conv1x1_nhwc(ops, x, self.conv1, True)
+    def _hidden_nhwc(self, x, ops, h1=None):
+        out = h1 if h1 is not None else _conv1x1_nhwc(ops, x, self.conv1, True)
         if isinstance(self.conv2, DCNv2Pack):
             return self.conv2.forward_nhwc(out, True)
         return _conv_nhwc(ops, out, self.conv2, True)
 
-    def forward_nhwc(self, x, ops):
+    def _chained(self, ops, nxt, h, w, b, residual=None, a2=None):
+        n, _, ho, wo = h.shape
+        c1 = nxt.conv1
+        s = c1.stride[0]
+        w2 = c1.weight.reshape(c1.out_channels, -1)
+        if a2 is not None:
+            pair = _or_none(ops.gemm2, _rows(h), a2, w, b, self.downsample.stride[0], True, chain=(w2, c1.bias, s))
+        else:
+            pair = _or_none(ops.gemm_chain, _rows(h), w, b, w2, c1.bias, (n, ho, wo), residual=residual, relu=True,
+                            relu2=True, out2_stride=s)
+        if pair is None:
+            return None
+        return _from_rows(pair[0], n, ho, wo), _from_rows(pair[1], n, (ho - 1) // s + 1, (wo - 1) // s + 1)
+
+    def forward_nhwc(self, x, ops, h1=None, chain_next=None):
+        ret = (lambda y: y) if chain_next is None else (lambda y: (y, None))
         if _two_source_ok(ops, self, x):
-            h = self._hidden_nhwc(x, ops)
+            h = self._hidden_nhwc(x, ops, h1)
             w, b = _stacked_pair(self)
             n, _, ho, wo = h.shape
+            if chain_next is not None:
+                pair = self._chained(ops, chain_next, h, w, b, a2=x)
+                if pair is not None:
+                    return pair
             y = _or_none(ops.gemm2, _rows(h), x, w, b, self.downsample.stride[0], True)
             if y is not None:
-                return _from_rows(y, n, ho, wo)
-            return _conv1x1_nhwc(ops, h, self.conv3, True, residual=_conv1x1_nhwc(ops, x, self.downsample, False))
+                return ret(_from_rows(y, n, ho, wo))
+            return ret(_conv1x1_nhwc(ops, h, self.conv3, True, residual=_conv1x1_nhwc(ops, x, self.downsample, False)))
         idt = x if self.downsample is None else _conv1x1_nhwc(ops, x, self.downsample, False)
-        out = _conv1x1_nhwc(ops, x, self.conv1, True)
+        out = h1 if h1 is not None else _conv1x1_nhwc(ops, x, self.conv1, True)
         cal = getattr(self, "chain_cal", None)
         if cal is not None:
             cal.collect(self.chain_site + ".t1", out)
@@ -331,7 +381,12 @@
             out = self.conv2.forward_nhwc(out, True)
         else:
             out = _conv_nhwc(ops, out, self.conv2, True)
-        return _conv1x1_nhwc(ops, out, self.conv3, True, residual=idt)
+        if chain_next is not None and self.downsample is None:
+            c3 = self.conv3
+            pair = self._chained(ops, chain_next, out, c3.weight.reshape(c3.out_channels, -1), c3.bias, residual=_rows(idt))
+            if pair is not None:
+                return pair
+        return ret(_conv1x1_nhwc(ops, out, self.conv3, True, residual=idt))
 
 
 class ResNet(nn.Module):
@@ -384,11 +439,17 @@
         return self._stages_nhwc(x, ops)
 
     def _stages_nhwc(self, x, ops):
-        outs = []
-        for i, st in enumerate(self.stages):
-            for blk in st:
+        outs, h1 = [], None
+        blocks = [(i, j == len(st) - 1, blk) for i, st in enumerate(self.stages) for j, blk in enumerate(st)]
+        for n, (i, last, blk) in enumerate(blocks):
+            nxt = blocks[n + 1][2] if n + 1 < len(blocks) else None
+            if _conv_chain_ok(ops, blk, nxt, x):
+                x, h1 = blk.forward_nhwc(x, ops, h1, nxt)
+            elif h1 is not None:
+                x, h1 = blk.forward_nhwc(x, ops, h1), None
+            else:
                 x = blk.forward_nhwc(x, ops)
-            if i in self.out_indices:
+            if last and i in self.out_indices:
                 outs.append(x)
         return outs
 
diff --git a/bevformer_tensorrt_amd/csrc/capi.hip b/bevformer_tensorrt_amd/csrc/capi.hip
--- a/bevformer_tensorrt_amd/csrc/capi.hip
+++ b/bevformer_tensorrt_amd/csrc/capi.hip
@@ -113,6 +113,7 @@
     {"bevops_tile_gemm_f16", (void *)&bevops_tile_gemm_f16},
     {"bevops_tile_gemm_f16_dst", (void *)&bevops_tile_gemm_f16_dst},
     {"bevops_gemm2_f16", (void *)&bevops_gemm2_f16},
+    {"bevops_gemm_chain_f16", (void *)&bevops_gemm_chain_f16},
     {"bevops_small_gemm_f16_dst", (void *)&bevops_small_gemm_f16_dst},
     {"bevops_small_gemm_f16", (void *)&bevops_small_gemm_f16},
     {"bevops_conv_tile_f16", (void *)&bevops_conv_tile_f16},
diff --git a/bevformer_tensorrt_amd/csrc/tsgemm.hip b/bevformer_tensorrt_amd/csrc/tsgemm.hip
--- a/bevformer_tensorrt_amd/csrc/tsgemm.hip
+++ b/bevformer_tensorrt_amd/csrc/tsgemm.hip
@@ -487,13 +487,31 @@
   int hin, win, hout, wout, stride;
 };
 
-template <int EPI, int KS, bool GRP, int KS2 = 0>
+struct TsChain {
+  const __half *w2, *bias2;
+  __half *out2;
+  int relu2, H, W, Ho, Wo, stride;
+};
+
+template <int OFF>
+__device__ __forceinline__ void lds_read_frag4(const unsigned (&addr)[4], f16x8 (&b)[4]) {
+  asm volatile("ds_read_b128 %0, %4 offset:%8\n\tds_read_b128 %1, %5 offset:%8\n\tds_read_b128 %2, %6 offset:%8\n\t"
+               "ds_read_b128 %3, %7 offset:%8\n\ts_waitcnt lgkmcnt(0)"
+               : "=&v"(b[0]), "=&v"(b[1]), "=&v"(b[2]), "=&v"(b[3])
+               : "v"(addr[0]), "v"(addr[1]), "v"(addr[2]), "v"(addr[3]), "n"(OFF)
+               : "memory");
+}
+
+template <int EPI, int KS, bool GRP, int KS2 = 0, int N2 = 0>
 __device__ __forceinline__ void tsgemm_ws_body(const __half *__restrict__ x, const __half *__restrict__ w,
                                                const __half *__restrict__ bias, const __half *__restrict__ res,
                                                __half *__restrict__ out, int M, int N, int relu, int units_total, int parts,
-                                               int chunks, const TsPacked &pk, const TsSrc2 &src2 = TsSrc2{}) {
+                                               int chunks, const TsPacked &pk, const TsSrc2 &src2 = TsSrc2{},
+                                               const TsChain &ch = TsChain{}) {
   extern __shared__ __attribute__((aligned(16))) char smem[];
   constexpr int K = KS * 64;
+  constexpr bool CH = N2 > 0;
+  static_assert(!CH || (EPI == 0 && !GRP && (N2 == 64 || N2 == 128)), "chain mode: EPI 0, 64 or 128 second columns");
   constexpr int KS1 = KS - KS2, K1 = KS1 * 64, K2 = KS2 * 64;
   const int tid = threadIdx.x, lane = tid & 63, wave = tid >> 6;
   int part, chunk;
@@ -594,16 +612,55 @@
   if constexpr (EPI != 1) {
     if (res) load_res(0, rq);
   }
+  constexpr int CU2 = CH ? N2 / 32 : 1;
+  [[maybe_unused]] const int cu2 = wave % CU2, g2 = wave / CU2;
+  [[maybe_unused]] f16x8 w2r[16];
+  [[maybe_unused]] uint2 b2q[4];
+  [[maybe_unused]] char *const img = smem + kWsEpi + kWsBufs * (KS * kWsStep);
+  constexpr int kStage2 = N2 * 4 + 16;
+  [[maybe_unused]] char *const stage2 = img + kWsRows * kTsBN * 2;
+  if constexpr (CH) {
+    const __half *w2row = ch.w2 + (size_t)(cu2 * 32 + (lane & 31)) * kTsBN + hi * 8;
+#pragma unroll
+    for (int kk = 0; kk < 16; ++kk) w2r[kk] = *reinterpret_cast<const f16x8 *>(w2row + kk * 16);
+#pragma unroll
+    for (int q = 0; q < 4; ++q) {
+      b2q[q] = make_uint2(0u, 0u);
+      if (ch.bias2) b2q[q] = *reinterpret_cast<const uint2 *>(ch.bias2 + cu2 * 32 + 8 * q + 4 * (int)hi);
+    }
+  }
+  [[maybe_unused]] auto wait_for_next_tile_chain = [&](int younger) {
+    switch (younger) {
+      case 0: asm volatile("s_waitcnt vmcnt(%0)" ::"n"(KS) : "memory"); break;
+      case 1: asm volatile("s_waitcnt vmcnt(%0)" ::"n"(KS + 1) : "memory"); break;
+      case 2: asm volatile("s_waitcnt vmcnt(%0)" ::"n"(KS + 2) : "memory"); break;
+      case 3: asm volatile("s_waitcnt vmcnt(%0)" ::"n"(KS + 3) : "memory"); break;
+      case 4: asm volatile("s_waitcnt vmcnt(%0)" ::"n"(KS + 4) : "memory"); break;
+      case 5: asm volatile("s_waitcnt vmcnt(%0)" ::"n"(KS + 5) : "memory"); break;
+      case 6: asm volatile("s_waitcnt vmcnt(%0)" ::"n"(KS + 6) : "memory"); break;
+      case 7: asm volatile("s_waitcnt vmcnt(%0)" ::"n"(KS + 7) : "memory"); break;
+      case 8: asm volatile("s_waitcnt vmcnt(%0)" ::"n"(KS + 8) : "memory"); break;
+      case 9: asm volatile("s_waitcnt vmcnt(%0)" ::"n"(KS + 9) : "memory"); break;
+      default: asm volatile("s_waitcnt vmcnt(%0)" ::"n"(KS + 10) : "memory"); break;
+    }
+  };
 
   dma(0, 0);
   dma(1, 1);
 #pragma unroll
   for (int kk = 0; kk < KS * 4; ++kk) asm volatile("" ::"v"(wr[kk]));
+  if constexpr (CH) {
+#pragma unroll
+    for (int kk = 0; kk < 16; ++kk) asm volatile("" ::"v"(w2r[kk]));
+#pragma unroll
+    for (int q = 0; q < 4; ++q) asm volatile("" ::"v"(b2q[q].x), "v"(b2q[q].y));
+  }
   wait_keep_one_tile();
   __builtin_amdgcn_s_barrier();
 
   int buf = 0;
   int stores_prev = 0;
+  [[maybe_unused]] int stores2_prev = 0;
   for (int t = 0; t < ntiles; ++t) {
     const int u0 = u_begin + t * kWsG;
     const int r0 = u0 * 32;
@@ -661,7 +718,11 @@
         asm volatile("s_waitcnt lgkmcnt(0)" ::: "memory");
       }
       __builtin_amdgcn_s_barrier();
-      if (half == 0) wait_for_next_tile(stores_prev + ((EPI != 1 && res) ? 4 : 0));
+      if constexpr (CH) {
+        if (half == 0) wait_for_next_tile_chain(stores_prev + stores2_prev + (res ? 4 : 0));
+      } else {
+        if (half == 0) wait_for_next_tile(stores_prev + ((EPI != 1 && res) ? 4 : 0));
+      }
 #pragma unroll
       for (int i = 0; i < kWsG; ++i) {
         const int r = rb + 32 * i;
@@ -687,11 +748,79 @@
                 *reinterpret_cast<uint4 *>(out + (size_t)chunk * (size_t)pk.gstride + m * kTsBN + (col - n0)) = ts_pack8(v);
               else
                 *reinterpret_cast<uint4 *>(out + m * N + col) = ts_pack8(v);
+              if constexpr (CH) {
+                const uint4 o = ts_pack8(v);
+                const f32x4 of = {__uint_as_float(o.x), __uint_as_float(o.y), __uint_as_float(o.z), __uint_as_float(o.w)};
+                lds_write16<0>(lds_addr(img + (half * 2 + (c8 >> 3)) * kWsStep + r * 128) +
+                                   ((((unsigned)c8 & 7u) ^ swz8((unsigned)r)) << 4), of);
+              }
             }
           }
         }
       }
+      if constexpr (CH) asm volatile("s_waitcnt lgkmcnt(0)" ::: "memory");
       __builtin_amdgcn_s_barrier();
+    }
+    if constexpr (CH) {
+      if (g2 < kWsG) {
+        f32x16 acc2;
+#pragma unroll
+        for (int r = 0; r < 16; ++r) acc2[r] = 0.f;
+        const unsigned xr = (unsigned)(g2 * 32 + (lane & 31));
+        unsigned fa2[4];
+#pragma unroll
+        for (int ks = 0; ks < 4; ++ks) fa2[ks] = lds_addr(img + xr * 128) + (((2u * ks + hi) ^ swz8(xr)) << 4);
+        auto step = [&](auto jc) __attribute__((always_inline)) {
+          constexpr int j = decltype(jc)::value;
+          f16x8 b[4];
+          lds_read_frag4<j * kWsStep>(fa2, b);
+#pragma unroll
+          for (int ks = 0; ks < 4; ++ks) acc2 = __builtin_amdgcn_mfma_f32_32x32x16_f16(w2r[4 * j + ks], b[ks], acc2, 0, 0, 0);
+        };
+        step(std::integral_constant<int, 0>{}); step(std::integral_constant<int, 1>{});
+        step(std::integral_constant<int, 2>{}); step(std::integral_constant<int, 3>{});
+        const unsigned rowa = lds_addr(stage2 + xr * kStage2 + (cu2 * 32 + 4 * (int)hi) * 4);
+        auto put2 = [&](auto qc) __attribute__((always_inline)) {
+          constexpr int q = decltype(qc)::value;
+          const f32x4 v = {acc2[4 * q] + h2f_lo(b2q[q].x), acc2[4 * q + 1] + h2f_hi(b2q[q].x),
+                           acc2[4 * q + 2] + h2f_lo(b2q[q].y), acc2[4 * q + 3] + h2f_hi(b2q[q].y)};
+          lds_write16<q * 32>(rowa, v);
+        };
+        put2(std::integral_constant<int, 0>{}); put2(std::integral_constant<int, 1>{});
+        put2(std::integral_constant<int, 2>{}); put2(std::integral_constant<int, 3>{});
+        asm volatile("s_waitcnt lgkmcnt(0)" ::: "memory");
+      }
+      __builtin_amdgcn_s_barrier();
+      constexpr int CP = N2 / 8, RP = kTsThreads / CP;
+#pragma unroll
+      for (int i = 0; i < kWsRows / RP; ++i) {
+        const int r = tid / CP + RP * i, cc = tid % CP;
+        if (r < rows) {
+          const int m = r0 + r;
+          size_t dst = (size_t)m;
+          bool sel = true;
+          if (ch.stride != 1) {
+            const int per = ch.H * ch.W;
+            const int b = m / per, q = m - b * per;
+            const int y = q / ch.W, xx = q - y * ch.W;
+            const int yo = y / ch.stride, xo = xx / ch.stride;
+            sel = yo * ch.stride == y && xo * ch.stride == xx;
+            dst = ((size_t)b * ch.Ho + (size_t)yo) * ch.Wo + (size_t)xo;
+          }
+          if (sel) {
+            float v[8];
+            lds_read32(lds_addr(stage2 + r * kStage2 + cc * 32), v);
+            if (ch.relu2) {
+#pragma unroll
+              for (int k = 0; k < 8; ++k) v[k] = fmaxf(v[k], 0.f);
+            }
+            *reinterpret_cast<uint4 *>(ch.out2 + dst * N2 + cc * 8) = ts_pack8(v);
+          }
+        }
+      }
+      if (ch.stride != 1) stores2_prev = 0;
+      else if (N2 == 64) stores2_prev = __builtin_amdgcn_readfirstlane(wave * 8 < rows ? 1 : 0);
+      else stores2_prev = __builtin_amdgcn_readfirstlane((wave * 4 < rows ? 1 : 0) + (wave * 4 + 32 < rows ? 1 : 0));
     }
     if constexpr (EPI == 2) {
 #pragma unroll
@@ -736,6 +865,15 @@
                                                                 int M, int N, int relu, int units_total, int parts, int chunks,
                                                                 TsSrc2 src2) {
   tsgemm_ws_body<0, KS, false, KS2>(x, w, bias, nullptr, out, M, N, relu, units_total, parts, chunks, TsPacked{}, src2);
+}
+
+template <int KS, int KS2, int N2>
+__global__ __launch_bounds__(kTsThreads) void tsgemm_ws_chain_kernel(const __half *__restrict__ x, const __half *__restrict__ w,
+                                                                     const __half *__restrict__ bias,
+                                                                     const __half *__restrict__ res, __half *__restrict__ out,
+                                                                     int M, int relu, int units_total, int parts, TsSrc2 src2,
+                                                                     TsChain ch) {
+  tsgemm_ws_body<0, KS, false, KS2, N2>(x, w, bias, KS2 > 0 ? nullptr : res, out, M, kTsBN, relu, units_total, parts, 1, TsPacked{}, src2, ch);
 }
 
 typedef int i32x4v __attribute__((ext_vector_type(4)));
@@ -1092,6 +1230,29 @@
   return launch_status();
 }
 
+struct ChainCall {
+  Gemm2Call g;
+  const void *res;
+  TsChain ch;
+};
+
+template <int KS, int KS2, int N2>
+int ws_chain_launch(const ChainCall &c) {
+  constexpr int lds = ws_lds(KS) + kWsRows * kTsBN * 2 + kWsRows * (N2 * 4 + 16);
+  if (!ensure_dynamic_lds<tsgemm_ws_chain_kernel<KS, KS2, N2>>(lds)) return BEVOPS_FAILURE;
+  const Gemm2Call &g = c.g;
+  const int units = (int)((g.m + 31) / 32);
+  int parts = ts_grid_x(1 << 30, 1);
+  if (parts > units) parts = units;
+  TsSrc2 src2{};
+  if (KS2 > 0)
+    src2 = TsSrc2{(const __half *)g.a2, (unsigned)((unsigned long long)g.B * g.H * g.W * g.k2 * 2), g.H, g.W, g.ho, g.wo, g.stride};
+  hipLaunchKernelGGL((tsgemm_ws_chain_kernel<KS, KS2, N2>), dim3((unsigned)parts), dim3(kTsThreads), lds, g.st,
+                     (const __half *)g.a1, (const __half *)g.w, (const __half *)g.bias, (const __half *)c.res, (__half *)g.out,
+                     (int)g.m, g.relu, units, parts, src2, c.ch);
+  return launch_status();
+}
+
 }
 
 bool tsgemm_ws2_in_domain(const Gemm2Call &g) { return g.n % kTsBN == 0 && g.k1 + g.k2 <= 256 && ts_use_ws(g.k1 + g.k2); }
@@ -1125,6 +1286,36 @@
   if (k % 64 != 0 || n % kTsBN != 0) return BEVOPS_NOT_SUPPORTED;
   const int rc = ts_f16_check(c, true);
   return rc != BEVOPS_SUCCESS ? rc : ts_launch_f16<0>(c, TsPacked{});
+}
+
+extern "C" int bevops_gemm_chain_f16(const void *a1, const void *a2, const void *weight, const void *bias,
+                                     const void *residual, void *out, long long M, int N, int K1, int K2, int a2_B, int a2_H,
+                                     int a2_W, int a2_stride, int relu, const void *weight2, const void *bias2, void *out2,
+                                     int N2, int relu2, int out_B, int out_H, int out_W, int out2_stride, void *stream) {
+  if (!a1 || !weight || !out || !weight2 || !out2 || M <= 0 || N <= 0 || K1 <= 0 || K2 < 0 || N2 <= 0 || out_B <= 0 ||
+      out_H <= 0 || out_W <= 0 || out2_stride <= 0 || (a2 != nullptr) != (K2 > 0))
+    return BEVOPS_BAD_PARAM;
+  const bool built = N == kTsBN && K1 == 64 && ((K2 == 0 && (N2 == 64 || N2 == 128)) || (K2 == 64 && N2 == 64));
+  if (!built || out2_stride > 2 || (a2 && residual) || !ts_use_ws(K1 + K2)) return BEVOPS_NOT_SUPPORTED;
+  ChainCall c{};
+  c.g = Gemm2Call{a1, a2, weight, bias, out, M, N, K1, K2, a2_B, a2_H, a2_W, a2_stride, 0, 0, relu, static_cast<hipStream_t>(stream)};
+  if (a2) {
+    const int rc = gemm2_check(c.g);
+    if (rc != BEVOPS_SUCCESS) return rc;
+  } else {
+    if (misaligned(a1, 15u) || misaligned(weight, 15u) || misaligned(out, 15u) || (bias && misaligned(bias, 15u)))
+      return BEVOPS_BAD_PARAM;
+    if (M > 0x7fffffffLL || gemm_over_limit((unsigned long long)M, K1, 2)) return BEVOPS_NOT_SUPPORTED;
+  }
+  if (M != (long long)out_B * out_H * out_W) return BEVOPS_BAD_PARAM;
+  if (misaligned(weight2, 15u) || misaligned(out2, 15u) || (bias2 && misaligned(bias2, 15u)) ||
+      (residual && misaligned(residual, 15u)))
+    return BEVOPS_BAD_PARAM;
+  c.res = residual;
+  c.ch = TsChain{(const __half *)weight2, (const __half *)bias2, (__half *)out2, relu2, out_H, out_W,
+                 (out_H - 1) / out2_stride + 1, (out_W - 1) / out2_stride + 1, out2_stride};
+  if (K2 == 64) return ws_chain_launch<2, 1, 64>(c);
+  return N2 == 64 ? ws_chain_launch<1, 0, 64>(c) : ws_chain_launch<1, 0, 128>(c);
 }
 
 extern "C" int bevops_tsgemm_f16_grouped(const void *x, const void *weight, const void *bias, void *out,
diff --git a/bevformer_tensorrt_amd/functions/__init__.py b/bevformer_tensorrt_amd/functions/__init__.py
--- a/bevformer_tensorrt_amd/functions/__init__.py
+++ b/bevformer_tensorrt_amd/functions/__init__.py
@@ -15,7 +15,7 @@
                                           feat_embed_nhwc)
 from .spatial_cross_attention import (spatial_cross_attention_sample, spatial_cross_attention_projected,
                                       spatial_cross_attention_plan)
-from .linear import (linear_bias_act, layer_norm, quantize_rows, dequantize_rows, linear_int8, tsgemm, tsgemm_ln, tsgemm_grouped, tile_gemm, tile_gemm_dst, gemm2, small_gemm, small_gemm_dst,
+from .linear import (linear_bias_act, layer_norm, quantize_rows, dequantize_rows, linear_int8, tsgemm, tsgemm_ln, tsgemm_grouped, tile_gemm, tile_gemm_dst, gemm2, gemm_chain, small_gemm, small_gemm_dst,
                      dense_auto, tsa_split, queue_mean2)
 from .int8_chain import linear_int8_chain, linear_int8_ln, conv_int8_chain_nhwc, modulated_deformable_conv2d_int8_nhwc
 from .conv import conv_nhwc, conv3x3_nhwc, conv3x3_auto, conv3x3_c64, conv_int8_nhwc, stem_conv_pool
@@ -71,7 +71,7 @@
     "BEVFORMER_IMAGE_PIPELINES", "scaled_size", "scale_lidar2img", "image_normalize_resize_pad",
     "DETECT2D_IMAGE_PIPELINES", "keep_ratio_size", "yolox_test_geometry", "centernet_test_geometry", "image_letterbox",
     "spatial_cross_attention_sample", "spatial_cross_attention_projected", "spatial_cross_attention_plan", "modulated_deformable_conv2d_nhwc", "bias_act_nhwc_", "linear_bias_act", "layer_norm", "rotate_hwc", "conv_offset_nhwc", "upsample_add_nhwc_", "feat_embed_nhwc",
-    "msda_pack_value", "multi_scale_deformable_attn_prepacked", "multi_scale_deformable_attn_local", "image_normalize_pad", "padded_size", "quantize_rows", "dequantize_rows", "linear_int8", "tsgemm", "tsgemm_ln", "tsgemm_grouped", "tile_gemm", "tile_gemm_dst", "gemm2", "small_gemm_dst", "small_gemm", "dense_auto", "tsa_split", "queue_mean2", "conv_nhwc", "conv3x3_nhwc", "conv3x3_auto", "conv3x3_c64", "conv_int8_nhwc", "bias_relu_maxpool_nhwc", "stem_conv_pool", "point_sampling", "self_attention_qkv", "refine_reference_points", "decode_boxes",
+    "msda_pack_value", "multi_scale_deformable_attn_prepacked", "multi_scale_deformable_attn_local", "image_normalize_pad", "padded_size", "quantize_rows", "dequantize_rows", "linear_int8", "tsgemm", "tsgemm_ln", "tsgemm_grouped", "tile_gemm", "tile_gemm_dst", "gemm2", "gemm_chain", "small_gemm_dst", "small_gemm", "dense_auto", "tsa_split", "queue_mean2", "conv_nhwc", "conv3x3_nhwc", "conv3x3_auto", "conv3x3_c64", "conv_int8_nhwc", "bias_relu_maxpool_nhwc", "stem_conv_pool", "point_sampling", "self_attention_qkv", "refine_reference_points", "decode_boxes",
     "linear_int8_chain", "linear_int8_ln", "conv_int8_chain_nhwc", "modulated_deformable_conv2d_int8_nhwc",
     "lss_depth_split", "upsample_bilinear_concat_nhwc", "lss_depth_split_q", "upsample_bilinear_nhwc_q",
     "conv_transpose2d_nhwc", "pack_deconv4x4s2", "deconv_packed_weight", "conv_transpose2d_q_nhwc", "quantize_deconv_weight",
diff --git a/bevformer_tensorrt_amd/functions/linear.py b/bevformer_tensorrt_amd/functions/linear.py
--- a/bevformer_tensorrt_amd/functions/linear.py
+++ b/bevformer_tensorrt_amd/functions/linear.py
@@ -210,11 +210,15 @@
     return outs
 
 
-def gemm2(a1, a2, weight, bias=None, stride=1, relu=False, out=None):
+def gemm2(a1, a2, weight, bias=None, stride=1, relu=False, out=None, chain=None):
     assert a1.is_cuda and a1.dtype == torch.float16 and a2.dtype == torch.float16 and weight.dtype == torch.float16
     if a2.dim() != 4 or not a2.is_contiguous(memory_format=torch.channels_last):
         raise ValueError("a2 must be a 4-d tensor in channels-last memory")
     B, K2, H, W = a2.shape
+    if chain is not None:
+        geom = (B, (H - 1) // stride + 1, (W - 1) // stride + 1)
+        return gemm_chain(a1, weight, bias, chain[0], chain[1], geom, a2=a2, a2_stride=stride, relu=relu, relu2=True,
+                          out2_stride=chain[2], out=out)
     K1, N = a1.shape[-1], weight.shape[0]
     if weight.shape[1] != K1 + K2:
         raise ValueError(f"weight {tuple(weight.shape)} does not match [N, {K1} + {K2}]")
@@ -235,6 +239,51 @@
     _call("bevops_gemm2_f16", a1.device, x1.data_ptr(), a2.data_ptr(), weight.data_ptr(), _ptr(bias), out.data_ptr(), M, N,
           K1, K2, B, H, W, int(stride), int(bool(relu)))
     return out
+
+
+def gemm_chain(a1, weight, bias, weight2, bias2, out_geom, a2=None, a2_stride=1, residual=None, relu=True, relu2=True,
+               out2_stride=1, out=None, out2=None):
+    assert a1.is_cuda and a1.dtype == torch.float16 and weight.dtype == torch.float16 and weight2.dtype == torch.float16
+    K1, N, N2 = a1.shape[-1], weight.shape[0], weight2.shape[0]
+    K2, geo = 0, (1, 1, 1)
+    if a2 is not None:
+        if a2.dtype != torch.float16 or a2.dim() != 4 or not a2.is_contiguous(memory_format=torch.channels_last):
+            raise ValueError("a2 must be a 4-d fp16 tensor in channels-last memory")
+        K2, geo = a2.shape[1], (a2.shape[0], a2.shape[2], a2.shape[3])
+    if weight.shape[1] != K1 + K2 or weight2.shape[1] != N:
+        raise ValueError(f"weights {tuple(weight.shape)}, {tuple(weight2.shape)} do not match [N, {K1} + {K2}], [N2, N]")
+    x1 = a1.reshape(-1, K1)
+    x1 = x1 if x1.is_contiguous() else x1.contiguous()
+    M = x1.shape[0]
+    weight = weight if weight.is_contiguous() else weight.contiguous()
+    weight2 = weight2 if weight2.is_contiguous() else weight2.contiguous()
+    if bias is not None and (bias.dtype != torch.float16 or not bias.is_contiguous()):
+        bias = bias.to(torch.float16).contiguous()
+    r2 = None
+    if residual is not None:
+        if residual.dtype != a1.dtype or residual.numel() != M * N:
+            raise ValueError("residual must be fp16 with M*N elements")
+        r2 = residual.reshape(M, N)
+        r2 = r2 if r2.is_contiguous() else r2.contiguous()
+    if out is None:
+        out = torch.empty((M, N), dtype=a1.dtype, device=a1.device)
+    else:
+        assert out.is_contiguous() and out.numel() == M * N and out.dtype == a1.dtype
+    if bias2 is not None and (bias2.dtype != torch.float16 or not bias2.is_contiguous()):
+        bias2 = bias2.to(torch.float16).contiguous()
+    B, H, W = (int(v) for v in out_geom)
+    s = int(out2_stride)
+    M2 = B * ((H - 1) // s + 1) * ((W - 1) // s + 1) if s > 0 else 0
+    if out2 is None:
+        out2 = torch.empty((M2, N2), dtype=a1.dtype, device=a1.device)
+    else:
+        assert out2.is_contiguous() and out2.numel() == M2 * N2 and out2.dtype == a1.dtype
+    if M == 0:
+        return out, out2
+    _call("bevops_gemm_chain_f16", a1.device, x1.data_ptr(), _ptr(a2), weight.data_ptr(), _ptr(bias), _ptr(r2), out.data_ptr(),
+          M, N, K1, K2, geo[0], geo[1], geo[2], int(a2_stride), int(bool(relu)), weight2.data_ptr(), _ptr(bias2),
+          out2.data_ptr(), N2, int(bool(relu2)), B, H, W, s)
+    return out, out2
 
 
 def small_gemm_dst(x, weight, bias, widths, residuals=None, relu=False, outs=None):
diff --git a/bevformer_tensorrt_amd/utils/lib.py b/bevformer_tensorrt_amd/utils/lib.py
--- a/bevformer_tensorrt_amd/utils/lib.py
+++ b/bevformer_tensorrt_amd/utils/lib.py
@@ -116,6 +116,8 @@
     "bevops_tile_gemm_f16": (c_int, [c_void_p] * 5 + [ctypes.c_longlong, c_int, c_int, c_int, c_void_p]),
     "bevops_tile_gemm_f16_dst": (c_int, [c_void_p] * 4 + [c_int, ctypes.c_longlong, c_int, c_int, c_int, c_void_p]),
     "bevops_gemm2_f16": (c_int, [c_void_p] * 5 + [ctypes.c_longlong] + [c_int] * 8 + [c_void_p]),
+    "bevops_gemm_chain_f16": (c_int, [c_void_p] * 6 + [ctypes.c_longlong] + [c_int] * 8 + [c_void_p] * 3 + [c_int] * 6
+                              + [c_void_p]),
     "bevops_small_gemm_f16_dst": (c_int, [c_void_p] * 4 + [c_int, ctypes.c_longlong, c_int, c_int, c_int, c_void_p]),
     "bevops_conv_tile_f16": (c_int, [c_void_p] * 5 + [c_int] * 8 + [c_void_p]),
     "bevops_conv3x3_c64_f16": (c_int, [c_void_p] * 4 + [c_int] * 6 + [c_void_p]),
diff --git a/include/bevops.h b/include/bevops.h
--- a/include/bevops.h
+++ b/include/bevops.h
@@ -178,6 +178,10 @@
                          void *out, long long M, int N, int K, int relu, void *stream);
 int bevops_gemm2_f16(const void *a1, const void *a2, const void *weight, const void *bias, void *out, long long M, int N,
                      int K1, int K2, int a2_B, int a2_H, int a2_W, int a2_stride, int relu, void *stream);
+int bevops_gemm_chain_f16(const void *a1, const void *a2, const void *weight, const void *bias, const void *residual,
+                          void *out, long long M, int N, int K1, int K2, int a2_B, int a2_H, int a2_W, int a2_stride,
+                          int relu, const void *weight2, const void *bias2, void *out2, int N2, int relu2, int out_B,
+                          int out_H, int out_W, int out2_stride, void *stream);
 typedef struct bevops_gemm_dst {
   int col_begin, col_end;
   void *out;
```
